# David-OConnor/molchanica

Measured on AMD Instinct MI355X. Metric: MD atom-updates/sec (and steps/sec), 1M-atom solvated box, higher is better.
Workload: dtype f32

## Files before the change

include/mdx.h:

```cpp
#ifndef MDX_H
#define MDX_H

#include <stddef.h>
#include <stdint.h>

#ifdef __cplusplus
extern "C" {
#endif

#define MDX_OK       0
#define MDX_EPARAM  (-1)
#define MDX_EDEVICE (-2)
#define MDX_ENAN    (-3)
#define MDX_EOOM    (-4)

#define MDX_OVR_BONDED_DISABLED           0x1u
#define MDX_OVR_COULOMB_DISABLED          0x2u
#define MDX_OVR_LJ_DISABLED               0x4u
#define MDX_OVR_LONG_RANGE_RECIP_DISABLED 0x8u

#define MDX_ATOM_STATIC      0x1u
#define MDX_ATOM_BONDED_ONLY 0x2u
#define MDX_ATOM_GHOST       0x4u

// ... 111 lines not shown
    uint64_t prune_passes;
    uint32_t n_owned, n_ghost;
    uint64_t repartitions;
    uint64_t local_rebuilds;
    double   repartition_ms_sum;
    double   fused_ms_sum;  uint64_t fused_launches;
    uint64_t energy_evaluations, energies_from_step_loop;
    uint64_t rebuild_fallbacks;
} mdx_stats;

typedef struct mdx_handle mdx_handle;

int mdx_device_count(void);

const char* mdx_last_error(void);

void mdx_config_default(mdx_config* cfg);

int mdx_create(const mdx_system* sys, const mdx_config* cfg, int device, mdx_handle** out);
void mdx_destroy(mdx_handle* h);

int mdx_step(mdx_handle* h, float dt, const float* ext_forces, uint32_t n_steps);

int      mdx_set_position_restraints(mdx_handle* h, uint32_t n, const uint32_t* idx, const float* ref, const float* k,
                                     const float* flat_bottom);
uint32_t mdx_position_restraints_read(mdx_handle* h, uint32_t capacity, uint32_t* idx, float* ref, float* k, float* flat_bottom);
int      mdx_restraint_energy(mdx_handle* h, double* energy, double* virial);

int mdx_energy(mdx_handle* h, mdx_energies* out);

int mdx_single_point(const mdx_system* sys, const mdx_config* cfg, int device,
                     mdx_energies* out, float* forces_or_null);
void mdx_single_point_release(void);

int mdx_download(mdx_handle* h, int which, float* dst );
int mdx_upload(mdx_handle* h, int which, const float* src );
int mdx_upload_range(mdx_handle* h, int which, uint32_t first, uint32_t count, const float* src );

int mdx_set_box(mdx_handle* h, const float lo[3], const float hi[3]);
int mdx_rebuild_spatial_caches(mdx_handle* h);

uint64_t mdx_step_count(const mdx_handle* h);

int mdx_neighbor_list(mdx_handle* h, uint32_t* offsets , uint32_t* idx );

enum { MDX_HC_FLEXIBLE = 0, MDX_HC_SHAKE = 1, MDX_HC_LINEAR = 2 };
int mdx_set_hydrogen_constraint(mdx_handle* h, int kind, uint32_t lincs_order, uint32_t lincs_iter, float shake_tolerance);
const char* mdx_constraint_description(mdx_handle* h);

int mdx_profile(mdx_handle* h, int enable);
int mdx_get_stats(mdx_handle* h, mdx_stats* out);
int mdx_pair_launch_info(const mdx_handle* h, uint32_t out[24]);
int mdx_pair_body_info(const mdx_handle* h, uint32_t out[4]);
int mdx_get_skin(const mdx_handle* h, float* skin, int* tuning);

#define MDX_THERMOSTAT_NONE      0
#define MDX_THERMOSTAT_BERENDSEN 1
#define MDX_THERMOSTAT_CSVR      2

#define MDX_INTEGRATOR_VERLET_VELOCITY 0
#define MDX_INTEGRATOR_LEAPFROG        1
#define MDX_INTEGRATOR_LANGEVIN_MIDDLE 2
int mdx_set_integrator(mdx_handle* h, int kind, float gamma_per_ps, float temperature, uint64_t seed);

int mdx_set_alchemical_softcore(mdx_handle* h, float alpha, float sigma_min);
int mdx_configure_alchemical_window(mdx_handle* h, uint32_t mol_index, double lambda);

#define MDX_MAX_FOREIGN_LAMBDAS 32
int      mdx_set_foreign_lambdas(mdx_handle* h, uint32_t n, const double* lambdas);
int      mdx_foreign_energies(mdx_handle* h, double* du , uint32_t n);
uint32_t mdx_snapshot_foreign_count(const mdx_handle* h, uint32_t k);
int      mdx_snapshot_read_foreign(mdx_handle* h, uint32_t k, double* du, uint32_t n);

#define MDX_BAROSTAT_NONE      0
#define MDX_BAROSTAT_BERENDSEN 1
#define MDX_BAR_PER_KCAL_MOL_A3 69476.95

int mdx_minimize_energy(mdx_handle* h, uint32_t max_iters, const float* ext_forces_or_null, float f_tol,
                        mdx_energies* final_or_null, uint32_t* iters_done_or_null);
int mdx_initialize_velocities(mdx_handle* h, float temperature, int zero_com_drift, uint64_t seed);
int mdx_shrink_cell_towards(mdx_handle* h, const float target_lo[3], const float target_hi[3], float shrink_per_step,
                            int* shrank_out);
int mdx_get_box(const mdx_handle* h, float lo[3], float hi[3]);
int mdx_set_barostat(mdx_handle* h, int kind, float pressure_target_bar, float tau_ps, float compressibility_per_bar,
                     uint32_t every_n_steps);
int mdx_set_thermostat(mdx_handle* h, int kind, float temp_target, float tau_ps, uint32_t every_n_steps,
                       uint64_t seed);
int mdx_set_zero_com_drift(mdx_handle* h, int enable);
int mdx_set_energy_cadence(mdx_handle* h, uint32_t every_n_steps);
int      mdx_set_snapshot_cadence(mdx_handle* h, uint32_t every_n, int with_velocities);
uint32_t mdx_snapshot_count(const mdx_handle* h);
int      mdx_snapshot_read(mdx_handle* h, uint32_t k, double* time_ps, uint64_t* step, mdx_energies* e,
                           float* pos , float* vel_or_null );
int      mdx_flush_snapshot_queues(mdx_handle* h);
#define MDX_SNAP_HANDLERS 8
enum { MDX_SNAP_MEMORY = 0, MDX_SNAP_DCD = 1, MDX_SNAP_NSTXOUT = 2, MDX_SNAP_NSTVOUT = 3, MDX_SNAP_NSTFOUT = 4, MDX_SNAP_NSTENERGY = 5,
       MDX_SNAP_NSTCALCENERGY = 6, MDX_SNAP_NSTXOUT_COMPRESSED = 7 };
int      mdx_set_snapshot_handlers(mdx_handle* h, const uint32_t every_n[MDX_SNAP_HANDLERS] );
uint32_t mdx_snapshot_handler_mask(const mdx_handle* h, uint32_t k);
int      mdx_snapshot_read_forces(mdx_handle* h, uint32_t k, float* frc );

#define MDX_HB_STANDARD 0
#define MDX_HB_WATER_O  1
#define MDX_HB_WATER_H0 2
#define MDX_HB_WATER_H1 3
typedef struct mdx_hbond {
// ... 132 lines not shown
```

molchanica_amd/csrc/mdx_api.hip:

```cpp
#include "mdx_comm.h"
#include <algorithm>
#include <atomic>
#include <chrono>
#include <cfloat>
#include <cmath>
#include <cstring>
#include <dlfcn.h>
#include <mutex>
#include <unordered_map>

static thread_local std::string g_last_error;
void mdx_set_error(const std::string& s) { g_last_error = s; }

static inline unsigned div_up(unsigned a, unsigned b) { return (a + b - 1) / b; }
static bool cut_on(float rc) { return rc > 0.f && std::isfinite(rc); }
static uint32_t f2u(float f) { uint32_t u; std::memcpy(&u, &f, 4); return u; }
static float u2f(uint32_t u) { float f; std::memcpy(&f, &u, 4); return f; }

#define FAIL(code, msg) do { mdx_set_error(msg); return (code); } while (0)

template <typename T>
static int upload_vec(T** dptr, const std::vector<T>& v, hipStream_t st) {
    if (*dptr) { (void)hipFree(*dptr); *dptr = nullptr; }
    HIP_TRY(hipMalloc((void**)dptr, std::max<size_t>(sizeof(T) * v.size(), 16)));
// ... 57 lines not shown
    MDX_TRY(chk(s->pairs14_idx, s->n_pairs14, 2, "pairs14"));
    if (s->n_bonds && (!s->bond_k || !s->bond_r0)) FAIL(MDX_EPARAM, "missing bond parameters");
    if (s->n_angles && (!s->angle_k || !s->angle_theta0)) FAIL(MDX_EPARAM, "missing angle parameters");
    if (s->n_dihedrals && (!s->dihedral_v || !s->dihedral_phase || !s->dihedral_n))
        FAIL(MDX_EPARAM, "missing dihedral parameters");
    if (s->excl_offsets) {
        if (s->excl_offsets[0] != 0) FAIL(MDX_EPARAM, "excl_offsets[0] must be 0");
        for (uint32_t i = 0; i < N; ++i)
            if (s->excl_offsets[i + 1] < s->excl_offsets[i]) FAIL(MDX_EPARAM, "excl_offsets not monotone");
        if (s->excl_offsets[N] && !s->excl_idx) FAIL(MDX_EPARAM, "missing excl_idx");
        for (uint32_t k = 0; k < s->excl_offsets[N]; ++k)
            if (s->excl_idx[k] >= N) FAIL(MDX_EPARAM, "exclusion index out of range");
    }
    if (!(c->skin >= 0.f) || !std::isfinite(c->skin)) FAIL(MDX_EPARAM, "skin must be finite and >= 0");
    if (!(c->coulomb_k >= 0.f)) FAIL(MDX_EPARAM, "coulomb_k must be >= 0");
    if (c->coulomb_mode < 0 || c->coulomb_mode > 2) FAIL(MDX_EPARAM, "unknown coulomb_mode");
    if (c->combining_rule < 0 || c->combining_rule > 1) FAIL(MDX_EPARAM, "unknown combining_rule");
    if (c->coulomb_mode == MDX_COULOMB_EWALD && !(c->ewald_alpha > 0.f))
        FAIL(MDX_EPARAM, "ewald_alpha must be > 0 for MDX_COULOMB_EWALD");
    return MDX_OK;
}

static void decode_periodic(int32_t v, int per[3]) {
    if (v & 0x10) { per[0] = v & 1; per[1] = (v >> 1) & 1; per[2] = (v >> 2) & 1; }
    else per[0] = per[1] = per[2] = (v != 0);
}

static int check_box(const int per[3], const float* lo, const float* hi, const mdx_config* c) {
    if (!(per[0] || per[1] || per[2])) return MDX_OK;
    if (!cut_on(c->lj_cutoff) || !cut_on(c->coulomb_cutoff))
        FAIL(MDX_EPARAM, "a periodic system needs finite LJ and Coulomb cut-offs");
    const float rl = std::max(c->lj_cutoff, c->coulomb_cutoff) + c->skin;
    for (int d = 0; d < 3; ++d) {
        if (!per[d]) continue;
        const float L = hi[d] - lo[d];
        if (!(L > 0.f) || !std::isfinite(L)) FAIL(MDX_EPARAM, "box extent must be positive");
        if (L < 2.0f * rl)
            FAIL(MDX_EPARAM, "box edge shorter than 2*(cutoff+skin): minimum image is not unique");
    }
    return MDX_OK;
}

int mdx_check_box(const mdx_handle* h, const float* lo, const float* hi) { return check_box(h->per, lo, hi, &h->cfg); }

static void free_device(mdx_handle* h) {
    DeviceState& d = h->d;
    void* ptrs[] = {d.o_qs, d.o_lj, d.o_invm, d.o_mass, d.o_q, d.o_lj_raw, d.excl_off, d.excl_idx, d.pos_orig,
                    d.vel_orig, d.ext_orig, d.posq, d.posq_alt, d.lj, d.vel, d.force, d.ref, d.orig_of, d.slot_of, d.gid, d.lflag,
                    d.slot_flags, d.cell_of,
                    d.cell_count, d.cell_start, d.cell_cursor, d.sorted_orig, d.sorted_tmp, d.col_tiles, d.tile_start,
                    d.tile_col, d.scan_tmp, d.cl_lo, d.cl_hi, d.cl_kind, d.list_counts, d.entry_cnt, d.entry_off,
                    d.mchunk_cnt, d.mchunk_off, d.entries, d.entries_in, d.inner_nch, d.list_cursors, d.masks, d.role_off_o, d.role_rec_o, d.role_cnt_s,
                    d.role_off_s, d.role_rec_s, d.role_prm, d.ctl, d.energy,
                    d.flags_dev, d.bonded_part, d.bbox_red, d.pair_count, d.inner_count, d.pme_force, d.wstep_s, d.path, d.dprune, d.force_b, d.force_c, d.cons_o, d.cons_s, d.cons_tmp, d.cons_mask, d.cons_cnt, d.cons_off, d.cons_vir, d.vsite_o, d.vsite_s, d.gsite_o, d.gsite_s, d.gsite_tmp, d.pme_q, d.pme_f,
                    d.pme_theta, d.pme_q2, d.pme_f2, d.scratch4, d.tile_bnd, d.tile_scan, d.tile_order, d.tile_lpt, d.rb_ctl, d.scan_chain, d.grp, d.grp_mat, d.fl_hot, d.fl_slab, d.star_o, d.star_s, d.ewald_tab,
                    d.ps_cls, d.ps_p14, d.ps_stage, d.ps_slab, d.ps_rows, d.ps_fslab, d.ps_fout, d.ps_rigid, d.ps_flex, d.ps_flex_tab, d.ps_search};
    for (void* p : ptrs) if (p) (void)hipFree(p);
    d = DeviceState{};
}

extern "C" void mdx_destroy(mdx_handle* h) {
    if (!h) return;
    (void)hipSetDevice(h->device);
    if (h->stream) (void)hipStreamSynchronize(h->stream);
    mdx_dd_destroy(h);
    for (auto& e : h->ev_pending) { (void)hipEventDestroy(e.a); (void)hipEventDestroy(e.b); }
    for (auto& e : h->ev_pool) (void)hipEventDestroy(e);
    mdx_pme_destroy(h);
    free_device(h);
    if (h->h_ctl) (void)hipHostFree(h->h_ctl);
    if (h->h_rb) (void)hipHostFree(h->h_rb);
    if (h->stream) (void)hipStreamDestroy(h->stream);
    delete h;
}

static int create_impl(const mdx_system* s, const mdx_config* c, int device, mdx_handle* h) {
    const uint32_t N = s->n_atoms;
    h->N = N; h->cfg = *c; h->device = device;
    if (h->cfg.chunk_steps == 0) h->cfg.chunk_steps = N < 131072u ? 48u : 16u;
    if (h->cfg.chunk_steps > MDX_MAX_CHUNK) h->cfg.chunk_steps = MDX_MAX_CHUNK;
    decode_periodic(s->periodic, h->per);
    h->periodic = h->per[0] || h->per[1] || h->per[2];
    for (int d = 0; d < 3; ++d) h->posre_per[d] = h->per[d];
    for (int d = 0; d < 3; ++d) { h->box_lo[d] = s->box_lo[d]; h->box_hi[d] = s->box_hi[d]; }
    MDX_TRY(check_box(h->per, h->box_lo, h->box_hi, c));
    h->n_local = N; h->cap_local = N;
    const bool all_cut = cut_on(c->lj_cutoff) && cut_on(c->coulomb_cutoff);
    if (c->skin == 0.f && all_cut && h->periodic) {
        float s0 = 2.0f;
        for (int d = 0; d < 3; ++d)
            if (h->per[d]) s0 = std::min(s0, 0.5f * (h->box_hi[d] - h->box_lo[d]) - std::max(c->lj_cutoff, c->coulomb_cutoff) - 0.01f);
        if (s0 >= 0.5f) { h->cfg.skin = s0; h->skin_tune.on = true; h->skin_tune.base_skin = s0; MDX_TRY(check_box(h->per, h->box_lo, h->box_hi, &h->cfg)); }
    }
    h->r_list = all_cut ? std::max(c->lj_cutoff, c->coulomb_cutoff) + h->cfg.skin : INFINITY;

    int ndev = 0;
    if (hipGetDeviceCount(&ndev) != hipSuccess || ndev == 0) FAIL(MDX_EDEVICE, "no HIP device available");
    if (device < 0 || device >= ndev) FAIL(MDX_EDEVICE, "device index out of range");
    HIP_TRY(hipSetDevice(device));
    h->pme_cus_per_xcd = mdx_pme_cu_split(h, c);
    if (h->pme_cus_per_xcd) MDX_TRY(mdx_stream_create_masked(&h->stream, h->pme_cus_per_xcd, true));
    else HIP_TRY(hipStreamCreateWithFlags(&h->stream, hipStreamNonBlocking));
    hipStream_t st = h->stream;
    DeviceState& d = h->d;

    const bool lj_off = (c->overrides & MDX_OVR_LJ_DISABLED) != 0;
    const bool coul_off = (c->overrides & MDX_OVR_COULOMB_DISABLED) != 0;
    const bool geom = c->combining_rule == MDX_COMBINE_GEOMETRIC;
    const float sqrt_ke = std::sqrt(c->coulomb_k);
    std::vector<float> qs(N), invm(N), mass(N), q(N);
    std::vector<float2> lj(N), ljraw(N);
    h->flags.assign(N, 0);
    h->n_mobile = 0; h->total_mass = 0.0;
    for (uint32_t i = 0; i < N; ++i) {
        const uint8_t fl = s->flags ? s->flags[i] : 0;
        h->flags[i] = fl;
        const bool nb_off = (fl & MDX_ATOM_BONDED_ONLY) != 0;
        const bool fixed = (fl & (MDX_ATOM_STATIC | MDX_ATOM_GHOST)) != 0;
        const float sg = s->lj_sigma[s->lj_type[i]], ep = s->lj_eps[s->lj_type[i]];
        q[i] = (nb_off || coul_off) ? 0.f : s->charge[i];
        qs[i] = q[i] * sqrt_ke;
        const float ep_eff = (nb_off || lj_off) ? 0.f : ep;
        lj[i] = make_float2(geom ? std::sqrt(sg) : 0.5f * sg, std::sqrt(24.0f * ep_eff));
        ljraw[i] = make_float2(sg, ep_eff);
        mass[i] = s->mass[i];
        invm[i] = fixed ? 0.f : MDX_ACC_CONV / s->mass[i];
        if (!fixed) { h->n_mobile++; }
        if (!(fl & MDX_ATOM_GHOST)) h->total_mass += s->mass[i];
    }
    h->h_mass = mass; h->h_lj = lj;
    {
        uint32_t n_lj_only = 0, n_q_only = 0;
        for (uint32_t i = 0; i < N; ++i) {
            const bool has_lj = lj[i].y != 0.f, has_q = qs[i] != 0.f;
            n_lj_only += has_lj && !has_q; n_q_only += has_q && !has_lj;
        }
        const char* const e = std::getenv("MDX_KIND_CLUSTERS");
        h->kind_split = e ? e[0] != '0' : (n_lj_only >= N / 20u && n_q_only >= N / 20u && N >= 200000u);
    }
    mdx_refresh_uni_lj(h);
    h->mol_start.assign(s->mol_start ? s->mol_start : nullptr, s->mol_start ? s->mol_start + s->n_mols : nullptr);
    h->total_charge = 0.0; h->sum_q2 = 0.0;
    h->q_abs_max = 0.0;
    for (uint32_t i = 0; i < N; ++i) { h->total_charge += q[i]; h->sum_q2 += (double)q[i] * q[i]; h->q_abs_max = std::max(h->q_abs_max, (double)std::fabs(q[i])); }
    const bool pme_on = c->coulomb_mode == MDX_COULOMB_EWALD && !(c->overrides & MDX_OVR_LONG_RANGE_RECIP_DISABLED) &&
                        !coul_off;
    MDX_TRY(upload_vec(&d.o_qs, qs, st)); MDX_TRY(upload_vec(&d.o_lj, lj, st));
    MDX_TRY(upload_vec(&d.o_invm, invm, st)); MDX_TRY(upload_vec(&d.o_mass, mass, st));
    MDX_TRY(upload_vec(&d.o_q, q, st)); MDX_TRY(upload_vec(&d.o_lj_raw, ljraw, st));

    std::vector<std::vector<uint32_t>> ex(N);
    {
        if (s->excl_offsets)
            for (uint32_t i = 0; i < N; ++i)
                for (uint32_t k = s->excl_offsets[i]; k < s->excl_offsets[i + 1]; ++k) {
                    const uint32_t j = s->excl_idx[k];
                    if (j == i) continue;
                    ex[i].push_back(j); ex[j].push_back(i);
                }
        for (uint32_t p = 0; p < s->n_pairs14; ++p) {
            const uint32_t a = s->pairs14_idx[2 * p], b = s->pairs14_idx[2 * p + 1];
            if (a == b) FAIL(MDX_EPARAM, "1-4 pair of an atom with itself");
            ex[a].push_back(b); ex[b].push_back(a);
        }
        std::vector<uint32_t> off(N + 1, 0), idx;
        for (uint32_t i = 0; i < N; ++i) {
            std::sort(ex[i].begin(), ex[i].end());
            ex[i].erase(std::unique(ex[i].begin(), ex[i].end()), ex[i].end());
            if (ex[i].size() > 255) FAIL(MDX_EPARAM, "more than 255 exclusions on one atom");
            off[i + 1] = off[i] + (uint32_t)ex[i].size();
            idx.insert(idx.end(), ex[i].begin(), ex[i].end());
        }
        MDX_TRY(upload_vec(&d.excl_off, off, st)); MDX_TRY(upload_vec(&d.excl_idx, idx, st));
    }

    h->n_bonds = s->n_bonds; h->n_angles = s->n_angles; h->n_dih = s->n_dihedrals; h->n_p14 = s->n_pairs14;
    {
        std::vector<uint32_t> cnt(N + 1, 0);
        auto count_term = [&](const uint32_t* idx, uint32_t n, int w) {
            for (size_t k = 0; k < (size_t)n * w; ++k) cnt[idx[k] + 1]++;
        };
        count_term(s->bond_idx, s->n_bonds, 2); count_term(s->angle_idx, s->n_angles, 3);
        count_term(s->dihedral_idx, s->n_dihedrals, 4); count_term(s->pairs14_idx, s->n_pairs14, 2);
        auto recip_excluded = [&](uint32_t i, uint32_t j) { return q[i] != 0.f && q[j] != 0.f; };
        if (pme_on)
            for (uint32_t i = 0; i < N; ++i)
                for (uint32_t j : ex[i]) cnt[i + 1] += recip_excluded(i, j) ? 1u : 0u;
        for (uint32_t i = 0; i < N; ++i) cnt[i + 1] += cnt[i];
        const uint32_t R = cnt[N];
        std::vector<RoleRec> recs(R);
        std::vector<uint32_t> cur(cnt.begin(), cnt.end() - 1);
        std::vector<float4> prm_tab;
// ... 1017 lines not shown

extern "C" int mdx_rebuild_spatial_caches(mdx_handle* h) {
    if (!h) FAIL(MDX_EPARAM, "null handle");
    HIP_TRY(hipSetDevice(h->device));
    h->list_valid = false;
    MDX_TRY(mdx_rebuild(h));
    return MDX_OK;
}

extern "C" int mdx_neighbor_list(mdx_handle* h, uint32_t* offsets, uint32_t* idx) {
    if (!h || !offsets) FAIL(MDX_EPARAM, "null argument");
    HIP_TRY(hipSetDevice(h->device));
    if (!h->list_valid) MDX_TRY(mdx_rebuild(h));
    return mdx_extract_neighbors(h, offsets, idx);
}

extern "C" int mdx_profile(mdx_handle* h, int enable) {
    if (!h) FAIL(MDX_EPARAM, "null handle");
    HIP_TRY(hipSetDevice(h->device));
    HIP_TRY(hipStreamSynchronize(h->stream));
    mdx_prof_collect(h);
    h->profile = enable != 0; h->profile_level = enable;
    if (enable) {
        h->stats.nb_ms_sum = h->stats.bonded_ms_sum = h->stats.integ_ms_sum = 0.0;
        h->stats.rebuild_ms_sum = h->stats.wall_ms_sum = 0.0;
        h->stats.nb_launches = h->stats.bonded_launches = h->stats.integ_launches = 0;
        if (h->dd) for (int k = 0; k < MDX_DIAG_PHASES; ++k) { h->dd->phase_ms[k] = 0.0; h->dd->phase_n[k] = 0; }
    }
    return MDX_OK;
}

extern "C" int mdx_get_skin(const mdx_handle* h, float* skin, int* tuning) {
    if (!h) FAIL(MDX_EPARAM, "null handle");
    if (skin) *skin = h->cfg.skin;
    if (tuning) *tuning = (h->skin_tune.on && h->skin_tune.phase < 4) ? 1 : 0;
    return MDX_OK;
}

extern "C" int mdx_pair_launch_info(const mdx_handle* h, uint32_t out[24]) {
    if (!h || !out) FAIL(MDX_EPARAM, "null argument");
    for (int k = 0; k < 8; ++k) { out[k] = h->pair_info_step[k]; out[8 + k] = h->pair_info_any[k]; }
    out[16] = h->inner_rebuilds; out[17] = h->inner_from_rebuild ? 1u : 0u; out[18] = h->water_step_launches; out[19] = h->water_step_mixed_launches;
    out[20] = (uint32_t)h->onepass_launches; out[21] = (uint32_t)h->onepass_violations; out[22] = h->pair_info_tail[0]; out[23] = h->pair_info_tail[1];
    return MDX_OK;
}

extern "C" int mdx_pair_body_info(const mdx_handle* h, uint32_t out[4]) {
    if (!h || !out) FAIL(MDX_EPARAM, "null argument");
    out[0] = h->uni_lj ? 1u : 0u; out[1] = h->pair_body_step; out[2] = h->pair_body_any;
    std::memcpy(&out[3], &h->uni_c, 4);
    return MDX_OK;
}

extern "C" int mdx_get_stats(mdx_handle* h, mdx_stats* out) {
    if (!h || !out) FAIL(MDX_EPARAM, "null argument");
    HIP_TRY(hipSetDevice(h->device));
    HIP_TRY(hipStreamSynchronize(h->stream));
    mdx_prof_collect(h);
    h->stats.step_count = h->step_count; h->stats.rebuild_count = h->rebuild_count;
    h->stats.n_inner_cluster_pairs = 0; h->stats.prune_passes = 0;
    if (h->d.inner_count) {
        unsigned long long c[MDX_EPART + 1];
        HIP_TRY(hipSetDevice(h->device));
        HIP_TRY(hipMemcpyAsync(c, h->d.inner_count, sizeof(c), hipMemcpyDeviceToHost, h->stream));
        HIP_TRY(hipStreamSynchronize(h->stream));
        unsigned long long tot = 0;
        for (int k = 0; k < MDX_EPART; ++k) tot += c[k];
        h->stats.prune_passes = c[MDX_EPART];
        h->stats.n_inner_cluster_pairs = c[MDX_EPART] ? tot / c[MDX_EPART] : 0;
    }
    h->stats.n_owned = h->dd ? h->dd->n_owned : h->n_local;
    h->stats.n_ghost = h->dd ? h->dd->n_local - h->dd->n_owned : 0;
    h->stats.repartitions = h->dd ? h->dd->repartitions : 0;
    h->stats.local_rebuilds = h->dd ? h->dd->local_rebuilds : 0;
    h->stats.repartition_ms_sum = h->dd ? h->dd->repartition_ms : 0.0;
    *out = h->stats;
    return MDX_OK;
}

__global__ void pack_pos_kernel(uint32_t n, const uint32_t* __restrict__ atom_idx, const uint32_t* __restrict__ slot_of,
                                const float4* __restrict__ posq, float4* __restrict__ out,
                                const uint32_t* __restrict__ flag_word) {
    uint32_t i = blockIdx.x * blockDim.x + threadIdx.x;
    if (i >= n) return;
    const uint32_t g = atom_idx[i];
    if (g == MDX_INVALID) {
        out[i] = make_float4(flag_word ? __uint_as_float(*flag_word) : 0.f, 0.f, 0.f, 0.f);
        return;
    }
    const uint32_t s = slot_of[g];
    out[i] = (s == MDX_INVALID) ? make_float4(0.f, 0.f, 0.f, 0.f) : posq[s];
}
__global__ void unpack_pos_kernel(uint32_t n, const uint32_t* __restrict__ atom_idx, const uint32_t* __restrict__ slot_of,
                                  float4* __restrict__ posq, const float4* __restrict__ in,
                                  const float4* __restrict__ shift, uint32_t* __restrict__ flag_word,
                                  float4* __restrict__ ref, uint32_t* __restrict__ prune_out, float path_thr,
                                  float gx, float gy, float gz, float* __restrict__ path_arr) {
    uint32_t i = blockIdx.x * blockDim.x + threadIdx.x;
    if (i >= n) return;
    const uint32_t g = atom_idx[i];
    if (g == MDX_INVALID) {
        if (flag_word) atomicMax(flag_word, __float_as_uint(in[i].x));
        return;
    }
    const uint32_t s = slot_of[g];
    if (s == MDX_INVALID) return;
// ... 267 lines not shown
```

molchanica_amd/csrc/mdx_extras.hip:

```cpp
#include "mdx_comm.h"
#include <algorithm>
#include <cmath>
#include <cstring>

#define FAIL(code, msg) do { mdx_set_error(msg); return (code); } while (0)
static inline unsigned div_up(unsigned a, unsigned b) { return (a + b - 1) / b; }

static double rng_u01(uint64_t* s) { return ((double)(mdx_splitmix64(s) >> 11) + 0.5) * (1.0 / 9007199254740992.0); }
static double rng_gauss(uint64_t* s) {
#pragma clang fp contract(off)
    const double u1 = rng_u01(s), u2 = rng_u01(s);
    return std::sqrt(-2.0 * std::log(u1)) * std::cos(6.283185307179586 * u2);
}
static double rng_gamma_int(uint64_t* s, long ia) {
    const double d = (double)ia - 1.0 / 3.0, c = 1.0 / std::sqrt(9.0 * d);
    for (;;) {
        const double x = rng_gauss(s), t = 1.0 + c * x;
        if (t <= 0.0) continue;
        const double v = t * t * t, u = rng_u01(s);
        if (std::log(u) < 0.5 * x * x + d - d * v + d * std::log(v)) return d * v;
    }
}
static double rng_sum_noises(uint64_t* s, long nn) {
    if (nn <= 0) return 0.0;
// ... 374 lines not shown
    h->e_cache_valid = false;
    return MDX_OK;
}

extern "C" int mdx_set_thermostat(mdx_handle* h, int kind, float temp_target, float tau_ps, uint32_t every_n_steps,
                                  uint64_t seed) {
    if (!h) FAIL(MDX_EPARAM, "null handle");
    if (kind < 0 || kind > 2) FAIL(MDX_EPARAM, "unknown thermostat kind");
    if (kind && (!(temp_target >= 0.f) || !(tau_ps > 0.f) || every_n_steps == 0))
        FAIL(MDX_EPARAM, "thermostat needs temp_target >= 0, tau > 0 and a coupling interval >= 1 step");
    h->tstat_kind = kind; h->tstat_temp = temp_target; h->tstat_tau = tau_ps;
    h->tstat_every = every_n_steps ? every_n_steps : 10; h->rng_state = seed;
    return MDX_OK;
}

extern "C" int mdx_set_integrator(mdx_handle* h, int kind, float gamma_per_ps, float temperature, uint64_t seed) {
    if (!h) FAIL(MDX_EPARAM, "null handle");
    if (kind < 0 || kind > 2) FAIL(MDX_EPARAM, "unknown integrator kind");
    if (kind == MDX_INTEGRATOR_LANGEVIN_MIDDLE && (!(gamma_per_ps >= 0.f) || !(temperature >= 0.f) || !std::isfinite(gamma_per_ps)))
        FAIL(MDX_EPARAM, "Langevin middle needs gamma >= 0 and temperature >= 0");
    if (kind && h->n_local != h->N && !h->dd) FAIL(MDX_EPARAM, "only velocity Verlet is supported on a decomposed handle");
    h->integrator = kind; h->lang_gamma = gamma_per_ps; h->lang_temp = temperature; h->lang_seed = seed;
    return MDX_OK;
}

extern "C" int mdx_set_alchemical_softcore(mdx_handle* h, float alpha, float sigma_min) {
    if (!h) FAIL(MDX_EPARAM, "null handle");
    if (!(alpha >= 0.f) || !std::isfinite(alpha)) FAIL(MDX_EPARAM, "soft-core alpha must be >= 0 (0 = linear coupling)");
    if (!(sigma_min > 0.f) || !std::isfinite(sigma_min)) FAIL(MDX_EPARAM, "soft-core sigma_min must be > 0");
    h->sc_alpha = alpha; h->sc_sigma_min = sigma_min;
    h->forces_valid = false;
    return MDX_OK;
}

extern "C" int mdx_configure_alchemical_window(mdx_handle* h, uint32_t mol_index, double lambda) {
    if (!h) FAIL(MDX_EPARAM, "null handle");
    HIP_TRY(hipSetDevice(h->device));
    const bool on = lambda >= 0.0;
    if (on) {
        if (!(lambda <= 1.0)) FAIL(MDX_EPARAM, "lambda must lie in [0, 1] (negative switches the window off)");
        if (h->mol_start.empty() || mol_index >= h->mol_start.size()) FAIL(MDX_EPARAM, "molecule index out of range (mol_start missing?)");
        if (!h->dd && h->n_local != h->N) FAIL(MDX_EPARAM, "alchemical windows need the library's own decomposition (mdx_comm_init) on a narrowed handle");
    }
    const uint32_t lo = on ? h->mol_start[mol_index] : 0;
    const uint32_t hi = on ? (mol_index + 1 < h->mol_start.size() ? h->mol_start[mol_index + 1] : h->N) : 0;
    for (uint32_t i = 0; i < h->N; ++i) {
        const float m = std::fabs(h->h_lj[i].y);
        h->h_lj[i].y = (i >= lo && i < hi) ? -m : m;
    }
    HIP_TRY(hipMemcpyAsync(h->d.o_lj, h->h_lj.data(), sizeof(float2) * h->N, hipMemcpyHostToDevice, h->stream));
    HIP_TRY(hipStreamSynchronize(h->stream));
    MDX_TRY(mdx_unsort_state(h));
    h->alch_on = on; h->alch_lambda = on ? lambda : 0.0; h->alch_lo = lo; h->alch_hi = hi;
    mdx_refresh_uni_lj(h);
    h->pme_canvas_clean = false; h->pme_canvas2_clean = false;
    h->list_valid = false; h->forces_valid = false;
    return MDX_OK;
}

extern "C" int mdx_get_box(const mdx_handle* h, float lo[3], float hi[3]) {
    if (!h || !lo || !hi) FAIL(MDX_EPARAM, "null argument");
    for (int d = 0; d < 3; ++d) { lo[d] = h->box_lo[d]; hi[d] = h->box_hi[d]; }
    return MDX_OK;
}

extern "C" int mdx_set_barostat(mdx_handle* h, int kind, float pressure_target_bar, float tau_ps,
                                float compressibility_per_bar, uint32_t every_n_steps) {
    if (!h) FAIL(MDX_EPARAM, "null handle");
    if (kind < 0 || kind > 1) FAIL(MDX_EPARAM, "unknown barostat kind");
    if (kind) {
        if (!h->dd && (!h->periodic || !(h->per[0] && h->per[1] && h->per[2]))) FAIL(MDX_EPARAM, "the barostat needs a fully periodic box");
        if (!h->dd && h->n_local != h->N) FAIL(MDX_EPARAM, "the barostat needs the library's own decomposition (mdx_comm_init) on a narrowed handle");
        if (!(tau_ps > 0.f) || every_n_steps == 0 || !std::isfinite(pressure_target_bar))
            FAIL(MDX_EPARAM, "barostat needs a finite target, tau > 0 and a coupling interval >= 1 step");
    }
    h->baro_kind = kind; h->baro_p0 = pressure_target_bar; h->baro_tau = tau_ps;
    h->baro_beta = compressibility_per_bar > 0.f ? compressibility_per_bar : 4.5e-5f;
    h->baro_every = every_n_steps ? every_n_steps : 25;
    return MDX_OK;
}

extern "C" int mdx_set_zero_com_drift(mdx_handle* h, int enable) {
    if (!h) FAIL(MDX_EPARAM, "null handle");
    h->zero_com = enable != 0;
    return MDX_OK;
}

extern "C" int mdx_set_snapshot_cadence(mdx_handle* h, uint32_t every_n, int with_velocities) {
    if (!h) FAIL(MDX_EPARAM, "null handle");
    h->snap_every = every_n; h->snap_vel = with_velocities != 0;
    return MDX_OK;
}

extern "C" uint32_t mdx_snapshot_count(const mdx_handle* h) { return h ? (uint32_t)h->snapshots.size() : 0u; }
extern "C" int mdx_snapshot_read_between_mols(mdx_handle* h, uint32_t k, float* out, uint32_t n) {
    if (!h || !out) FAIL(MDX_EPARAM, "null argument");
    if (k >= h->snapshots.size()) FAIL(MDX_EPARAM, "snapshot index out of range");
    const auto& sn = h->snapshots[k];
    if (sn.between.empty()) FAIL(MDX_EPARAM, "the snapshot was taken without energy groups (mdx_set_energy_groups)");
    if ((size_t)n * n != sn.between.size()) FAIL(MDX_EPARAM, "n must be the number of groups the snapshot was taken with");
    std::memcpy(out, sn.between.data(), sizeof(float) * sn.between.size());
    return MDX_OK;
}
extern "C" double mdx_time_ps(const mdx_handle* h) { return h ? h->time_ps : 0.0; }

extern "C" int mdx_set_snapshot_handlers(mdx_handle* h, const uint32_t every_n[MDX_SNAP_HANDLERS]) {
// ... 248 lines not shown
```

molchanica_amd/csrc/mdx_grid.hip:

```cpp
#include "mdx_internal.h"
#include <atomic>
#include <chrono>
#include <algorithm>
#include <cfloat>
#include <cmath>

#define WAVE_LDS_SYNC()                                      \
    do {                                                     \
        __builtin_amdgcn_fence(__ATOMIC_SEQ_CST, "workgroup"); \
        __builtin_amdgcn_wave_barrier();                     \
    } while (0)

static inline unsigned div_up(unsigned a, unsigned b) { return (a + b - 1) / b; }

constexpr int SCAN_THREADS = 256;
constexpr int SCAN_ITEMS = 8;
constexpr int SCAN_TILE = SCAN_THREADS * SCAN_ITEMS;

__device__ __forceinline__ uint32_t block_exclusive_scan_256(uint32_t v, uint32_t* s_wave, uint32_t* total) {
    const int lane = threadIdx.x & 63, wave = threadIdx.x >> 6;
    uint32_t inc = v;
#pragma unroll
    for (int d = 1; d < 64; d <<= 1) {
        uint32_t t = __shfl_up(inc, d);
// ... 836 lines not shown
        unsigned long long m = 0ull;
        uint32_t jcs[8], codes13 = 0;
#pragma unroll
        for (int e = 0; e < 8; ++e) {
            uint32_t idx = c * 8 + e;
            jcs[e] = (idx < nmc) ? (fl[idx] & 0x7FFFFFFu) : MDX_INVALID;
            if (a.half && idx < nmc && (fl[idx] >> 27) == 13u) codes13 |= 1u << e;
            if (idx < nmc) m |= 0xFFull << (8 * e);
        }
        if (myo == MDX_INVALID) {
            m = 0ull;
        } else {
#pragma unroll
            for (int e = 0; e < 8; ++e)
                if (jcs[e] == (myslot >> 3)) {
                    const unsigned long long gone = ((codes13 >> e) & 1u) ? ((2ull << (myslot & 7)) - 1ull)
                                                                          : (1ull << (myslot & 7));
                    m &= ~(gone << (8 * e));
                }
#pragma unroll
            for (int q = 0; q < LB_SPC; ++q) {
                const uint32_t sp = spc[q];
                if (sp == MDX_INVALID) continue;
#pragma unroll
                for (int e = 0; e < 8; ++e)
                    if (jcs[e] == (sp >> 3)) m &= ~(1ull << (8 * e + (sp & 7)));
            }
            for (uint32_t k = eb + LB_SPC; k < ee; ++k) {
                uint32_t sp = a.slot_of[a.excl_idx[k]];
                if (sp == MDX_INVALID) continue;
#pragma unroll
                for (int e = 0; e < 8; ++e)
                    if (jcs[e] == (sp >> 3)) m &= ~(1ull << (8 * e + (sp & 7)));
            }
        }
        if (a.mask_layout == 2) {
            const int ii = lane & 7, jj = lane >> 3;
            unsigned long long mq = 0ull;
#pragma unroll
            for (int ci = 0; ci < 8; ++ci) {
                const unsigned long long mp = __shfl(m, ci * 8 + ii);
#pragma unroll
                for (int e = 0; e < 8; ++e) mq |= ((mp >> (8 * e + jj)) & 1ull) << (8 * e + ci);
            }
            m = mq;
        }
        a.masks[(size_t)(mbase + c) * 64 + lane] = m;
    }
}

#ifndef PRUNE_TRIES
#define PRUNE_TRIES 1
#endif
struct PruneInner { uint2* entries_in; uint32_t* inner_nch; float rin2; WptRule rule; };
template <bool INNER>
__global__ __launch_bounds__(256) void prune_list_kernel(uint32_t T, float r2, float shx, float shy, float shz,
                                                         const float4* __restrict__ posq, ListCounts* __restrict__ counts,
                                                         const uint32_t* __restrict__ entry_off, uint2* __restrict__ entries,
                                                         uint32_t null_cluster, unsigned long long* __restrict__ pair_count,
                                                         const uint32_t* __restrict__ rb_ctl, uint32_t* __restrict__ tile_int,
                                                         const uint8_t* __restrict__ cl_kind, PruneInner pin) {
    __shared__ float4 s_j[4][64];
    const int lane = threadIdx.x & 63, wave = __builtin_amdgcn_readfirstlane(threadIdx.x >> 6);
    uint32_t first_ghost_cluster = 0xFFFFFFFFu;
    if (rb_ctl) {
        T = __builtin_amdgcn_readfirstlane(rb_ctl[0]); null_cluster = T * MDX_CL_PER_TILE;
        first_ghost_cluster = __builtin_amdgcn_readfirstlane(rb_ctl[1]) * MDX_CL_PER_TILE;
    }
    const bool inner_on = INNER && mdx_wpt_rule(pin.rule, T) == 1;
    bool ghost_hit = false;
    const uint32_t per_xcd = gridDim.x >> 3;
    const uint32_t t = MDX_XCD_SWIZZLE ? ((blockIdx.x & 7u) * per_xcd + (blockIdx.x >> 3)) * 4 + wave : blockIdx.x * 4 + wave;
    if (t >= T) return;
    const int ii = lane & 7, jj = lane >> 3;
    float xi[8], yi[8], zi[8];
#pragma unroll
    for (int ci = 0; ci < 8; ++ci) {
        const float4 p = posq[(size_t)t * MDX_TILE + ci * MDX_CLUSTER + ii];
        xi[ci] = p.x; yi[ci] = p.y; zi[ci] = p.z;
    }
    constexpr int NTRY = INNER ? 0 : PRUNE_TRIES;
    constexpr int TI[6] = {0, 7, 3, 0, 7, 4}, TJ[6] = {0, 7, 4, 7, 0, 3};
    float4 rep[NTRY ? NTRY : 1];
#pragma unroll
    for (int k = 0; k < NTRY; ++k) rep[k] = posq[(size_t)t * MDX_TILE + (lane & 7) * MDX_CLUSTER + TI[k]];
    uint32_t ilj = 0xFFu, iq = 0xFFu;
    if (cl_kind) {
        const uint32_t k = lane < MDX_CL_PER_TILE ? cl_kind[(size_t)t * MDX_CL_PER_TILE + lane] : 0u;
        ilj = (uint32_t)__ballot((k & 1u) != 0u) & 0xFFu; iq = (uint32_t)__ballot((k & 2u) != 0u) & 0xFFu;
    }
    const ListCounts cnt = counts[t];
    const uint32_t e0 = entry_off[t], nmc = cnt.n_masked >> 3, nchunks = (cnt.n_masked + cnt.n_plain) >> 3;
    uint32_t kept = 0, wcur = 0;
    uint32_t wcur_in = 0;
    uint2 ent_n = make_uint2(null_cluster, 13u), ent_nn = make_uint2(null_cluster, 13u);
    float4 pj_n = make_float4(0.f, 0.f, 0.f, 0.f);
    if (nchunks) { ent_n = entries[e0 + (lane >> 3)]; pj_n = posq[(size_t)ent_n.x * MDX_CLUSTER + (lane & 7)]; }
    if (nchunks > 1) ent_nn = entries[e0 + 8 + (lane >> 3)];
    for (uint32_t c = 0; c < nchunks; ++c) {
        const uint2 ent = ent_n;
        float4 pj = pj_n;
        if (c + 1 < nchunks) {
            ent_n = ent_nn;
            pj_n = posq[(size_t)ent_n.x * MDX_CLUSTER + (lane & 7)];
            if (c + 2 < nchunks) ent_nn = entries[e0 + (c + 2) * 8 + (lane >> 3)];
        }
        const uint32_t code = ent.y & 31u;
        pj.x += (float)((int)(code % 3u) - 1) * shx;
        pj.y += (float)((int)((code / 3u) % 3u) - 1) * shy;
        pj.z += (float)((int)(code / 9u) - 1) * shz;
        s_j[wave][lane] = pj;
        __builtin_amdgcn_fence(__ATOMIC_SEQ_CST, "workgroup"); __builtin_amdgcn_wave_barrier();
        uint32_t newy = ent.y;
        if (cl_kind) {
            const uint32_t kj = ent.x < null_cluster ? cl_kind[ent.x] : 0u;
            newy = (ent.y & 0xFFu) | (ent.y & ((((kj & 1u) ? ilj : 0u) | ((kj & 2u) ? iq : 0u)) << 8));
        }
        const uint32_t y_in = newy;
        uint32_t newy_in = newy & 0xFFu;
        unsigned long long acc = 0ull;
#pragma unroll
        for (int k = 0; k < NTRY; ++k) {
            const float4 q = s_j[wave][(lane & ~7) + TJ[k]];
            const float dx = rep[k].x - q.x, dy = rep[k].y - q.y, dz = rep[k].z - q.z;
            acc |= __ballot(dx * dx + dy * dy + dz * dz < r2);
        }
#pragma unroll 2
        for (int e = 0; e < 8; ++e) {
            const float4 q = s_j[wave][e * 8 + jj];
            const uint32_t y = __builtin_amdgcn_readlane(y_in, e * 8);
            const uint32_t sure = (uint32_t)(acc >> (e * 8)) & 0xFFu;
            uint32_t any = sure, anyin = 0u;
#pragma unroll
            for (int ci = 0; ci < 8; ++ci) {
                if (!(((y >> 8) & ~sure) & (1u << ci))) continue;
                const float dx = xi[ci] - q.x, dy = yi[ci] - q.y, dz = zi[ci] - q.z;
                const float d2 = dx * dx + dy * dy + dz * dz;
                const bool hit = __ballot(d2 < r2) != 0ull;
                any |= (hit ? 1u : 0u) << ci;
                if (INNER && hit) anyin |= (__ballot(d2 < pin.rin2) != 0ull ? 1u : 0u) << ci;
            }
            const uint32_t im = (y >> 8) & any;
            kept += __popc(im & 0xFFu);
            if ((lane >> 3) == e) newy = (y & 0xFFu) | ((im & 0xFFu) << 8);
            if (INNER && (lane >> 3) == e) newy_in = (y & 0xFFu) | ((((y >> 8) & anyin) & 0xFFu) << 8);
        }
        __builtin_amdgcn_fence(__ATOMIC_SEQ_CST, "workgroup"); __builtin_amdgcn_wave_barrier();
        ghost_hit |= ((newy >> 8) & 0xFFu) != 0u && ent.x >= first_ghost_cluster && ent.x < null_cluster;
        if (c < nmc) {
            if ((lane & 7) == 0 && newy != ent.y) entries[e0 + c * 8 + (lane >> 3)].y = newy;
            if (inner_on && (lane & 7) == 0) pin.entries_in[e0 + c * 8 + (lane >> 3)] = make_uint2(ent.x, newy_in);
        } else {
            const bool alive = (lane & 7) == 0 && ((newy >> 8) & 0xFFu) != 0u;
            const unsigned long long bal = __ballot(alive);
            if (alive) {
                const uint32_t rank = __popcll(bal & ((1ull << lane) - 1ull));
                entries[e0 + cnt.n_masked + wcur + rank] = make_uint2(ent.x, newy);
            }
            wcur += __popcll(bal);
            if (inner_on) {
                const bool alive_in = (lane & 7) == 0 && ((newy_in >> 8) & 0xFFu) != 0u;
                const unsigned long long bin = __ballot(alive_in);
                if (alive_in) pin.entries_in[e0 + cnt.n_masked + wcur_in + __popcll(bin & ((1ull << lane) - 1ull))] = make_uint2(ent.x, newy_in);
                wcur_in += __popcll(bin);
            }
        }
    }
    const uint32_t np_pad = (wcur + 7u) & ~7u;
    if (lane < (int)(np_pad - wcur)) entries[e0 + cnt.n_masked + wcur + lane] = make_uint2(null_cluster, 13u);
    if (inner_on) {
        const uint32_t nin_pad = (wcur_in + 7u) & ~7u;
        if (lane < (int)(nin_pad - wcur_in)) pin.entries_in[e0 + cnt.n_masked + wcur_in + lane] = make_uint2(null_cluster, 13u);
        if (lane < 8) pin.inner_nch[(size_t)t * 8 + lane] = nmc + (nin_pad >> 3);
    }
    const bool any_ghost = __any(ghost_hit);
    if (lane == 0) {
        counts[t].n_plain = np_pad;
        if (kept) atomicAdd(pc_slot(pair_count, t, 1), (unsigned long long)kept);
        if (tile_int) tile_int[t] = (!any_ghost && t * MDX_CL_PER_TILE < first_ghost_cluster) ? 1u : 0u;
    }
}

template <int W>
__global__ __launch_bounds__(W * 64) void prune_list_mw_kernel(uint32_t T, float r2, float shx, float shy, float shz,
                                                               const float4* __restrict__ posq, ListCounts* __restrict__ counts,
                                                               const uint32_t* __restrict__ entry_off, uint2* __restrict__ entries,
                                                               uint32_t null_cluster, unsigned long long* __restrict__ pair_count,
                                                               const uint32_t* __restrict__ rb_ctl, uint32_t* __restrict__ tile_int,
                                                               const uint8_t* __restrict__ cl_kind) {
    __shared__ float4 s_j[W][64];
    __shared__ uint32_t s_ghost;
    const int lane = threadIdx.x & 63, wave = __builtin_amdgcn_readfirstlane(threadIdx.x >> 6);
    uint32_t first_ghost_cluster = 0xFFFFFFFFu;
    if (rb_ctl) {
        T = __builtin_amdgcn_readfirstlane(rb_ctl[0]); null_cluster = T * MDX_CL_PER_TILE;
        first_ghost_cluster = __builtin_amdgcn_readfirstlane(rb_ctl[1]) * MDX_CL_PER_TILE;
    }
    const uint32_t t = blockIdx.x;
    if (t >= T) return;
    if (threadIdx.x == 0) s_ghost = 0u;
    if (tile_int) __syncthreads();
    bool ghost_hit = false;
    const int ii = lane & 7, jj = lane >> 3;
    float xi[8], yi[8], zi[8];
#pragma unroll
    for (int ci = 0; ci < 8; ++ci) {
        const float4 p = posq[(size_t)t * MDX_TILE + ci * MDX_CLUSTER + ii];
        xi[ci] = p.x; yi[ci] = p.y; zi[ci] = p.z;
    }
    const float4 rep = posq[(size_t)t * MDX_TILE + (lane & 7) * MDX_CLUSTER];
    uint32_t ilj = 0xFFu, iq = 0xFFu;
    if (cl_kind) {
        const uint32_t k = lane < MDX_CL_PER_TILE ? cl_kind[(size_t)t * MDX_CL_PER_TILE + lane] : 0u;
        ilj = (uint32_t)__ballot((k & 1u) != 0u) & 0xFFu; iq = (uint32_t)__ballot((k & 2u) != 0u) & 0xFFu;
    }
    const ListCounts cnt = counts[t];
    const uint32_t e0 = entry_off[t], nchunks = (cnt.n_masked + cnt.n_plain) >> 3;
    uint32_t kept = 0;
    uint2 ent_n = make_uint2(null_cluster, 13u);
    float4 pj_n = make_float4(0.f, 0.f, 0.f, 0.f);
    if ((uint32_t)wave < nchunks) { ent_n = entries[e0 + wave * 8 + (lane >> 3)]; pj_n = posq[(size_t)ent_n.x * MDX_CLUSTER + (lane & 7)]; }
    for (uint32_t c = wave; c < nchunks; c += W) {
        const uint2 ent = ent_n;
        float4 pj = pj_n;
        if (c + W < nchunks) {
            ent_n = entries[e0 + (c + W) * 8 + (lane >> 3)];
// ... 483 lines not shown
            return major * LPT_BUCKETS + LPT_BUCKETS - 1u - min(nch, LPT_BUCKETS - 1u);
        };
        for (uint32_t t = threadIdx.x; t < T; t += blockDim.x) atomicAdd(&s_hist[bucket(t)], 1u);
        __syncthreads();
        {
            const uint32_t b0 = 2u * threadIdx.x, h0 = b0 < NB ? s_hist[b0] : 0u, h1 = b0 + 1u < NB ? s_hist[b0 + 1u] : 0u;
            uint32_t tot;
            const uint32_t ex = block_exclusive_scan_1024(h0 + h1, s_scan, &tot);
            if (b0 < NB) s_cur[b0] = ex;
            if (b0 + 1u < NB) s_cur[b0 + 1u] = ex + h0;
            __syncthreads();
            if (pass == 1 && threadIdx.x == 0) s_nint = s_cur[LPT_BUCKETS];
        }
        __syncthreads();
        for (uint32_t t = threadIdx.x; t < T; t += blockDim.x) order[atomicAdd(&s_cur[bucket(t)], 1u)] = t;
        __syncthreads();
    }
    if (threadIdx.x < 64) {
        const unsigned long long c = a.cursors[(size_t)threadIdx.x * 16];
        uint32_t e = (uint32_t)c, m = (uint32_t)(c >> 32);
        unsigned long long pa = a.pair_count[(size_t)threadIdx.x * PC_STRIDE], pb = a.pair_count[(size_t)threadIdx.x * PC_STRIDE + 1];
#pragma unroll
        for (int k = 32; k > 0; k >>= 1) { e += __shfl_xor(e, k); m += __shfl_xor(m, k); pa += __shfl_xor(pa, k); pb += __shfl_xor(pb, k); }
        if (threadIdx.x == 0) {
            a.pair_count[PC_TOTAL] = pa; a.pair_count[PC_TOTAL + 1] = pb;
            a.rb_ctl[RB_N_INT] = s_nint;
            a.host[0] = T; a.host[1] = a.rb_ctl[RB_T_OWN]; a.host[2] = a.rb_ctl[RB_NONFINITE]; a.host[3] = s_nint;
            for (int k = 0; k < 4; ++k) a.host[4 + k] = a.flags[k];
            a.host[8] = e; a.host[9] = m;
            a.host[10] = (uint32_t)pa; a.host[11] = (uint32_t)(pa >> 32); a.host[12] = (uint32_t)pb; a.host[13] = (uint32_t)(pb >> 32);
            a.rb_ctl[RB_NONFINITE] = 0u;
            __threadfence_system();
            a.host[31] = a.seq;
        }
    }
}


static int spin_on_readback(mdx_handle* h, uint32_t seq) {
    static const bool spin_ok = [] { const char* e = std::getenv("MDX_CHUNK_SPIN"); return !(e && e[0] == '0'); }();
    if (!spin_ok) { HIP_TRY(hipStreamSynchronize(h->stream)); return MDX_OK; }
    volatile uint32_t* seq_word = (volatile uint32_t*)h->h_rb + 31;
    const auto t0 = std::chrono::steady_clock::now();
    for (uint32_t spins = 0; *seq_word != seq; ++spins) {
        if ((spins & 0xFFFu) == 0xFFFu && std::chrono::steady_clock::now() - t0 > std::chrono::milliseconds(50)) {
            HIP_TRY(hipStreamSynchronize(h->stream));
            break;
        }
    }
    std::atomic_thread_fence(std::memory_order_acquire);
    return MDX_OK;
}

struct RebuildResult { uint32_t T = 0, E = 0, MC = 0, n_interior = 0; unsigned long long npairs = 0; bool ordered = false, classified = false, inner_built = false; };

struct TileOrderPlan { bool lpt, grouped, split; };
static TileOrderPlan tile_order_plan(const mdx_handle* h, uint32_t T) {
    static const int lpt_env = [] { const char* e = std::getenv("MDX_TILE_LPT"); return e ? (e[0] == '0' ? 0 : (e[0] == '2' ? 2 : 1)) : -1; }();
    const bool decomposed = h->dd || h->n_local != h->N;
    TileOrderPlan p;
    p.lpt = (lpt_env >= 0 ? lpt_env >= 1 : (decomposed || T >= 512u)) && mdx_nb_variant(h) >= 2;
    p.grouped = lpt_env >= 0 ? lpt_env == 2 : !decomposed;
    p.split = h->want_tile_split && mdx_nb_variant(h) >= 2;
    return p;
}

static int rebuild_fast(mdx_handle* h, RebuildResult* res, bool* fell_back) {
    DeviceState& d = h->d;
    hipStream_t st = h->stream;
    const uint32_t N = h->n_local;
    const GridParams g = h->grid;
    *fell_back = false;
    if (!d.rb_ctl) { ALLOC(d.rb_ctl, RB_WORDS); HIP_TRY(hipMemsetAsync(d.rb_ctl, 0, sizeof(uint32_t) * RB_WORDS, st)); }
    if (!d.pair_count) ALLOC(d.pair_count, PC_TOTAL + 2);
    if (!d.list_cursors) ALLOC(d.list_cursors, LB_REGIONS * 32 + 2);
    if (!h->h_rb) { HIP_TRY(hipHostMalloc((void**)&h->h_rb, sizeof(uint32_t) * 32, hipHostMallocDefault)); h->h_rb[31] = 0u; }
    if (!h->cell_count_clean) { HIP_TRY(hipMemsetAsync(d.cell_count, 0, sizeof(uint32_t) * ((size_t)h->ncells + 1), st)); h->cell_count_clean = true; }
    if (!h->slot_of_clean) { HIP_TRY(hipMemsetAsync(d.slot_of, 0xFF, sizeof(uint32_t) * (size_t)h->N, st)); h->slot_of_clean = true; }
    const uint32_t T_bound = N / MDX_TILE + h->ncol + 1;
    if (T_bound + 1 > h->cap_tiles) { *fell_back = true; return MDX_OK; }
    const TileOrderPlan plan = tile_order_plan(h, T_bound);
    const bool prune = !std::isinf(h->r_list) && mdx_nb_variant(h) >= 2;
    static const bool exact_prune = [] { const char* e = std::getenv("MDX_EXACT_PRUNE"); return !(e && e[0] == '0'); }();
    const bool classify_here = plan.split && plan.lpt && g.npop > 1 && prune && exact_prune;
    if (plan.lpt && (!d.tile_lpt || d.cap_tile_lpt < T_bound)) { d.cap_tile_lpt = h->cap_tiles + 1; ALLOC(d.tile_lpt, d.cap_tile_lpt); }
    if (classify_here && (!d.tile_bnd || h->cap_tile_split < T_bound + 1)) {
        h->cap_tile_split = h->cap_tiles + 1;
        ALLOC(d.tile_bnd, h->cap_tile_split); ALLOC(d.tile_scan, h->cap_tile_split); ALLOC(d.tile_order, h->cap_tile_split);
    }

    if (h->in_slot_space)
        hipLaunchKernelGGL(rb_prep_kernel<true>, dim3(div_up(N, 256)), dim3(256), 0, st, N, g, d.gid, d.slot_of, d.posq, d.vel, d.pos_orig,
                           d.vel_orig, d.lflag, d.cell_of, d.sorted_orig, d.cell_count, d.rb_ctl);
    else
        hipLaunchKernelGGL(rb_prep_kernel<false>, dim3(div_up(N, 256)), dim3(256), 0, st, N, g, d.gid, d.slot_of, d.posq, d.vel, d.pos_orig,
                           d.vel_orig, d.lflag, d.cell_of, d.sorted_orig, d.cell_count, d.rb_ctl);
    h->in_slot_space = false;
    {
        GridScanArgs ga{};
        ga.ncells = h->ncells; ga.ncol = h->ncol; ga.nzb = g.nzb;
        ga.first_ghost_col = g.npop > 1 ? (uint32_t)(g.ncx * g.ncy) : 0xFFFFFFFFu;
        ga.cell_count = d.cell_count; ga.cell_start = d.cell_start; ga.tile_start = d.tile_start; ga.tile_col = d.tile_col;
        ga.rb_ctl = d.rb_ctl; ga.flags = d.flags_dev; ga.pair_count = d.pair_count; ga.list_cursors = d.list_cursors;
        MDX_TRY(scan_chain_of(h, &ga.chain));
        hipLaunchKernelGGL(rb_gridscan_kernel, dim3(div_up(h->ncells + 1, SCAN1_WINDOW)), dim3(SCAN1_THREADS), 0, st, ga);
    }
    hipLaunchKernelGGL(rb_scatter_kernel, dim3(div_up(N, 256)), dim3(256), 0, st, N, d.cell_of, d.sorted_orig, d.cell_start, d.sorted_tmp);
    hipLaunchKernelGGL(cell_rank_kernel, dim3(div_up(N, 256)), dim3(256), 0, st, N, d.cell_of, d.cell_start, d.pos_orig, d.sorted_tmp, d.sorted_orig);
    {
        AssignArgs aa{};
        aa.rb_ctl = d.rb_ctl; aa.nzb = g.nzb; aa.tile_col = d.tile_col; aa.tile_start = d.tile_start; aa.cell_start = d.cell_start;
        aa.sorted_orig = d.sorted_orig; aa.pos_orig = d.pos_orig; aa.vel_orig = d.vel_orig; aa.gid = d.gid; aa.lflag = d.lflag;
        aa.o_qs = d.o_qs; aa.o_lj = d.o_lj; aa.o_invm = d.o_invm; aa.orig_of = d.orig_of; aa.slot_of = d.slot_of;
        aa.cl_kind = d.cl_kind; aa.kind_split = h->kind_split ? 1 : 0;
        aa.posq = d.posq; aa.lj = d.lj; aa.vel = d.vel; aa.ref = d.ref; aa.force = d.force; aa.slot_flags = d.slot_flags; aa.path = d.path; aa.dprune = d.dprune;
        aa.cl_lo = d.cl_lo; aa.cl_hi = d.cl_hi;
        aa.role_off_o = h->n_roles ? d.role_off_o : nullptr; aa.role_cnt_s = h->n_roles ? d.role_cnt_s : nullptr;
        hipLaunchKernelGGL(rb_assign_kernel, dim3(div_up(T_bound + 1, 4)), dim3(256), 0, st, aa);
    }
    h->in_slot_space = true;
    const uint32_t S_bound = (T_bound + 1) * MDX_TILE;
    if (h->n_roles) MDX_TRY(scan_u32_dev_n(h, d.role_cnt_s, d.role_off_s, S_bound + 1, d.scan_tmp, d.rb_ctl + RB_SCAN_N));

    ListArgs a{};
    a.T = T_bound; a.T_dev = d.rb_ctl + RB_T; a.g = g;
    a.r_build = std::isinf(h->r_list) ? h->r_list : h->r_list * (1.0f + 1e-5f) + 1e-4f;
    a.tile_col = d.tile_col; a.tile_start = d.tile_start; a.cl_lo = d.cl_lo; a.cl_hi = d.cl_hi;
    a.orig_of = d.orig_of; a.slot_of = d.slot_of; a.gid = d.gid; a.slot_flags = d.slot_flags;
    a.excl_off = d.excl_off; a.excl_idx = d.excl_idx;
    a.counts = d.list_counts; a.entry_cnt = d.entry_cnt; a.mchunk_cnt = d.mchunk_cnt;
    a.entry_off = d.entry_off; a.mchunk_off = d.mchunk_off; a.entries = d.entries; a.masks = d.masks;
    a.err = d.flags_dev; a.null_cluster = T_bound * MDX_CL_PER_TILE;
    a.mask_layout = mdx_nb_variant(h) >= 2 ? 2 : 1;
    a.half = mdx_nb_half(h) ? 1 : 0;
    a.cell_start = d.cell_start; a.posq = d.posq; a.pair_count = d.pair_count;
    a.cursors = reinterpret_cast<unsigned long long*>(d.list_cursors);
    a.n_regions = 1;
    while (a.n_regions < (uint32_t)LB_REGIONS && a.n_regions * 128u <= T_bound) a.n_regions <<= 1;
    a.region_cap_e = (uint32_t)(std::min<uint64_t>(h->cap_entries, 0xFFFFFFFFull) / a.n_regions) & ~7u;
    a.region_cap_m = h->cap_mchunks / a.n_regions;
    a.list_grid = (div_up(T_bound, LB_WAVES) + 7u) & ~7u;
    uint32_t rf_blocks = 0;
    if (h->n_roles) {
        a.rf_S = S_bound; a.rf_role_off_o = d.role_off_o; a.rf_rec_o = d.role_rec_o; a.rf_role_off_s = d.role_off_s;
        a.rf_rec_s = d.role_rec_s; a.rf_lflag = d.lflag;
        rf_blocks = div_up(S_bound, LB_WAVES * 64);
    }
    if (g.npop > 1) hipLaunchKernelGGL((build_list_kernel<LB_SINGLE, LB_PLAIN_DD>), dim3(a.list_grid + rf_blocks), dim3(LB_WAVES * 64), 0, st, a);
    else hipLaunchKernelGGL(build_list_kernel<LB_SINGLE>, dim3(a.list_grid + rf_blocks), dim3(LB_WAVES * 64), 0, st, a);
    static const int inner_mode = [] { const char* e = std::getenv("MDX_REBUILD_INNER"); return e ? (e[0] == '0' ? 0 : (e[0] == '2' ? 2 : 1)) : 1; }();
    const bool inner_env = inner_mode == 2 || (inner_mode == 1 && !mdx_has_constraints(h) && h->n_vsites == 0);
    const float inner_skin_next = h->inner_skin_auto > 0.f ? h->inner_skin_auto : c_inner_skin(h->cfg);
    const bool dual_next = !h->dual_auto_off && mdx_nb_half(h) && prune && inner_skin_next > 0.f && inner_skin_next < h->cfg.skin &&
                           (h->n_vsites == 0 || h->vsites_convex);
    const bool inner_here = inner_env && dual_next && exact_prune && !h->dd && h->n_local == h->N && g.npop == 1 && !h->alch_on &&
                            d.entries_in && d.inner_nch;
    bool inner_launched = false;
    if (prune && exact_prune) {
        const float rb = a.r_build;
        const float shx = h->per[0] ? h->box_hi[0] - h->box_lo[0] : 0.f, shy = h->per[1] ? h->box_hi[1] - h->box_lo[1] : 0.f,
                    shz = h->per[2] ? h->box_hi[2] - h->box_lo[2] : 0.f;
        uint32_t* const tint = classify_here ? d.tile_bnd : nullptr;
        const uint8_t* const kinds = h->kind_split ? d.cl_kind : nullptr;
        static const uint32_t mw_below = [] { const char* e = std::getenv("MDX_PRUNE_MW_BELOW"); return e ? (uint32_t)std::atoi(e) : 12000u; }();
        if (T_bound < mw_below)
            hipLaunchKernelGGL(prune_list_mw_kernel<8>, dim3(T_bound), dim3(512), 0, st, T_bound, rb * rb, shx, shy, shz, d.posq, d.list_counts,
                               d.entry_off, d.entries, a.null_cluster, d.pair_count, (const uint32_t*)d.rb_ctl, tint, kinds);
        else if (inner_here) {
            PruneInner pin{};
            pin.entries_in = d.entries_in; pin.inner_nch = d.inner_nch; pin.rule = mdx_wpt_rule_of(h);
            const float rin = std::max(std::isfinite(h->cfg.lj_cutoff) && h->cfg.lj_cutoff > 0.f ? h->cfg.lj_cutoff : 0.f,
                                       std::isfinite(h->cfg.coulomb_cutoff) && h->cfg.coulomb_cutoff > 0.f ? h->cfg.coulomb_cutoff : 0.f) + inner_skin_next;
            pin.rin2 = rin * rin;
            hipLaunchKernelGGL(prune_list_kernel<true>, dim3((div_up(T_bound, 4) + 7u) & ~7u), dim3(256), 0, st, T_bound, rb * rb, shx, shy, shz,
                               d.posq, d.list_counts, d.entry_off, d.entries, a.null_cluster, d.pair_count, (const uint32_t*)d.rb_ctl, tint, kinds, pin);
            inner_launched = true;
        } else
            hipLaunchKernelGGL(prune_list_kernel<false>, dim3((div_up(T_bound, 4) + 7u) & ~7u), dim3(256), 0, st, T_bound, rb * rb, shx, shy, shz,
                               d.posq, d.list_counts, d.entry_off, d.entries, a.null_cluster, d.pair_count, (const uint32_t*)d.rb_ctl, tint, kinds,
                               PruneInner{});
    }
    MDX_TRY(mdx_remap_constraints(h));
    const uint32_t seq = ++h->rb_seq;
    {
        FinishArgs fa{};
        fa.rb_ctl = d.rb_ctl; fa.counts = d.list_counts;
        fa.tile_lpt = plan.lpt ? d.tile_lpt : nullptr; fa.lpt_grouped = plan.grouped ? 1u : 0u; fa.rule = mdx_wpt_rule_of(h);
        fa.tile_int = classify_here ? d.tile_bnd : nullptr; fa.tile_order = classify_here ? d.tile_order : nullptr;
        fa.cursors = reinterpret_cast<const unsigned long long*>(d.list_cursors); fa.pair_count = d.pair_count; fa.flags = d.flags_dev;
        fa.host = (volatile uint32_t*)h->h_rb; fa.seq = seq;
        hipLaunchKernelGGL(rb_finish_kernel, dim3(1), dim3(1024), 0, st, fa);
    }
    HIP_TRY(hipGetLastError());
    MDX_TRY(spin_on_readback(h, seq));
    const uint32_t T = h->h_rb[0];
    uint32_t flags[4];
    for (int k = 0; k < 4; ++k) flags[k] = h->h_rb[4 + k];
    if (h->h_rb[2]) { h->cell_count_clean = false; mdx_set_error("non-finite position at neighbour rebuild"); return MDX_ENAN; }
    if (T > T_bound) { mdx_set_error("internal: tile count beyond its bound"); return MDX_EDEVICE; }
    h->T = T; h->S = (T + 1) * MDX_TILE;
    if (flags[0] & 1u) { mdx_set_error("exclusion table overflow while building the pair list"); return MDX_EPARAM; }
    if (flags[0] & (16u | 32u)) {
        if (std::getenv("MDX_LIST_DEBUG")) fprintf(stderr, "[mdx] fused list rebuild fell back: flags %u, T %u, cap_e %llu cap_m %u regions %u\n",
                                                   flags[0], T, (unsigned long long)h->cap_entries, h->cap_mchunks, a.n_regions);
        *fell_back = true;
        return MDX_OK;
    }
    if (flags[0] & 8u) { mdx_set_error("a constrained / virtual-site atom is missing from the local atom set"); return MDX_EPARAM; }
    if (flags[0] & 2u) { mdx_set_error("exclusion table overflow while building the pair list"); return MDX_EPARAM; }
    if (flags[0] & 4u) { mdx_set_error("a bonded partner of an owned atom is missing from the local atom set (halo too thin)"); return MDX_EPARAM; }
    res->T = T; res->E = h->h_rb[8]; res->MC = h->h_rb[9];
    const unsigned long long built = (unsigned long long)h->h_rb[10] | ((unsigned long long)h->h_rb[11] << 32);
    const unsigned long long kept = (unsigned long long)h->h_rb[12] | ((unsigned long long)h->h_rb[13] << 32);
    res->npairs = (prune && exact_prune) ? kept : built;
    h->E = res->E; h->MC = res->MC;
    res->ordered = true;
    res->inner_built = inner_launched && mdx_wpt_rule(mdx_wpt_rule_of(h), T) == 1;
    h->force_zeroed = true;
    h->tile_lpt_on = plan.lpt; h->tile_lpt_grouped = plan.grouped;
    h->tile_split = false; h->n_interior = 0;
    if (classify_here) { h->tile_split = true; h->n_interior = h->h_rb[3]; res->classified = true; }
    return MDX_OK;
}


int mdx_rebuild(mdx_handle* h) {
    MdxRange range_rebuild("mdx list rebuild");
    h->vsites_fresh = false;
    hipEvent_t e0 = nullptr, e1 = nullptr;
    if (h->profile) {
        for (hipEvent_t* e : {&e0, &e1}) {
            if (!h->ev_pool.empty()) { *e = h->ev_pool.back(); h->ev_pool.pop_back(); }
            else HIP_TRY(hipEventCreate(e));
        }
        HIP_TRY(hipEventRecord(e0, h->stream));
    }
    DeviceState& d = h->d;
    static const bool fused_env = [] { const char* e = std::getenv("MDX_REBUILD_FUSED"); return !(e && e[0] == '0'); }();
    static const bool two_pass_env0 = [] { const char* e = std::getenv("MDX_LIST_TWO_PASS"); return e && e[0] == '1'; }();
    bool fast = fused_env && !two_pass_env0 && d.entries && d.masks && h->cap_entries && h->cap_mchunks && h->T > 0 && h->n_local > 0;
    for (int k = 0; k < 3; ++k) if (!h->per[k] && !h->have_local_bounds) fast = false;
    if (!fast) MDX_TRY(mdx_unsort_state(h));
    const bool was_in_slot_space = h->in_slot_space;
    MDX_TRY(setup_grid(h));
    if (fast && (size_t)h->ncells + 1 > ((size_t)1 << 21)) { fast = false; MDX_TRY(mdx_unsort_state(h)); }
    if (fast && was_in_slot_space && !h->in_slot_space) fast = false;
    const uint32_t N = h->n_local;
    const GridParams g = h->grid;
    hipStream_t st = h->stream;
    RebuildResult res;
    bool fast_done = false;
    if (fast) {
        bool fell_back = false;
        MDX_TRY(rebuild_fast(h, &res, &fell_back));
        fast_done = !fell_back;
        if (fell_back) { MDX_TRY(mdx_unsort_state(h)); h->stats.rebuild_fallbacks++; }
    }
    uint32_t E = res.E, MC = res.MC;
    unsigned long long npairs = res.npairs;
    const bool prune = !std::isinf(h->r_list) && mdx_nb_variant(h) >= 2;
    if (!fast_done) {
    h->cell_count_clean = false;
    {
        const uint32_t n_max = std::max<uint32_t>(h->N, h->ncells + 1);
        hipLaunchKernelGGL(rebuild_clear_kernel, dim3(div_up(n_max, 256)), dim3(256), 0, st, d.slot_of, h->N, d.cell_count,
                           d.cell_cursor, h->ncells + 1, d.flags_dev);
    }
    hipLaunchKernelGGL(bin_atoms_kernel, dim3(div_up(N, 256)), dim3(256), 0, st, d.pos_orig, N, g, d.lflag, d.cell_of,
                       d.cell_count, d.flags_dev + 1);
// ... 143 lines not shown
    };
    MDX_TRY(read_counts());
    if (speculative) {
        if (flags[0] & 1u) { mdx_set_error("exclusion table overflow while building the pair list"); return MDX_EPARAM; }
        if (flags[0] & (16u | 32u)) {
            const uint32_t keep = flags[0] & ~(16u | 32u);
            HIP_TRY(hipMemcpyAsync(d.flags_dev, &keep, sizeof(uint32_t), hipMemcpyHostToDevice, st));
            HIP_TRY(hipStreamSynchronize(st));
            speculative = false;
            grow_for_regions = (flags[0] & 32u) != 0;
            if (std::getenv("MDX_LIST_DEBUG")) fprintf(stderr, "[mdx] single-pass list build fell back: flags %u, T %u, E %u MC %u, cap_e %llu cap_m %u regions %u\n",
                                                       flags[0], T, E, MC, (unsigned long long)h->cap_entries, h->cap_mchunks, a.n_regions);
            MDX_TRY(two_pass());
            launch_prune();
            MDX_TRY(read_counts());
        } else {
            h->E = E; h->MC = MC;
        }
    }
    if (prune && exact_prune) npairs = npairs_pruned;
    if (flags[0] & 8u) { mdx_set_error("a constrained / virtual-site atom is missing from the local atom set"); return MDX_EPARAM; }
    if (flags[0] & 3u) { mdx_set_error("exclusion table overflow while building the pair list"); return MDX_EPARAM; }
    if (flags[0] & 4u) {
        mdx_set_error("a bonded partner of an owned atom is missing from the local atom set (halo too thin)");
        return MDX_EPARAM;
    }

    res.T = T;
    }
    const uint32_t T = h->T, S = h->S, NC = (T + 1) * MDX_CL_PER_TILE;
    {
        const TileOrderPlan plan = tile_order_plan(h, T);
        if (!res.classified) {
            h->tile_split = false; h->n_interior = 0;
            if (plan.split) MDX_TRY(mdx_classify_tiles(h, plan.lpt));
        }
        if (!res.ordered) {
            h->tile_lpt_on = false;
            if (plan.lpt) MDX_TRY(mdx_order_tiles_by_length(h, plan.grouped));
        }
    }
    h->list_valid = true;
    h->forces_valid = false;
    h->rebuild_count++; h->steps_since_rebuild = 0;
    mdx_dd_note_rebuild(h);
    h->inner_skin = h->inner_skin_auto > 0.f ? h->inner_skin_auto : c_inner_skin(h->cfg);
    h->dual_on = !h->dual_auto_off && mdx_nb_half(h) && prune && h->inner_skin > 0.f && h->inner_skin < h->cfg.skin &&
                 (h->n_vsites == 0 || h->vsites_convex);
    h->prune_pending = !(res.inner_built && h->dual_on);
    h->inner_from_rebuild = !h->prune_pending;
    if (h->inner_from_rebuild) ++h->inner_rebuilds;
    h->tail_w = 0; h->tail_tiles = 0;
    if (h->dual_on && h->tile_lpt_on && h->tile_lpt_grouped && !h->alch_on) mdx_tail_plan(h, T, &h->tail_w, &h->tail_tiles);
    if (!d.inner_count) { ALLOC(d.inner_count, MDX_EPART + 8); HIP_TRY(hipMemsetAsync(d.inner_count, 0, sizeof(unsigned long long) * (MDX_EPART + 8), st)); }
    uint64_t nmask = (uint64_t)MC * 8;
    h->stats.n_atoms = N; h->stats.n_slots = S; h->stats.n_tiles = T; h->stats.n_clusters = NC;
    h->stats.n_list_entries = E; h->stats.n_masked_entries = nmask;
    h->stats.n_cluster_pairs = (mdx_nb_variant(h) >= 2) ? npairs : (uint64_t)E * 8;
    if (h->profile) {
        float ms = 0.f;
        HIP_TRY(hipEventRecord(e1, st)); HIP_TRY(hipEventSynchronize(e1));
        HIP_TRY(hipEventElapsedTime(&ms, e0, e1));
        h->stats.rebuild_ms_sum += ms;
        h->ev_pool.push_back(e0); h->ev_pool.push_back(e1);
    }
    return MDX_OK;
}

__global__ __launch_bounds__(1024) void lpt_order_kernel(uint32_t T, const ListCounts* __restrict__ counts, const uint32_t* __restrict__ is_int,
                                                         uint32_t* __restrict__ order, uint32_t group_tiles) {
    constexpr uint32_t NB = 8 * LPT_BUCKETS;
    __shared__ uint32_t s_hist[NB], s_cur[NB];
    for (uint32_t b = threadIdx.x; b < NB; b += blockDim.x) s_hist[b] = 0;
    __syncthreads();
    auto bucket = [&](uint32_t t) {
        const uint32_t nch = (counts[t].n_masked + counts[t].n_plain) >> 3;
        const uint32_t major = group_tiles ? min(t / group_tiles, 7u) : ((is_int && !is_int[t]) ? 1u : 0u);
        return major * LPT_BUCKETS + LPT_BUCKETS - 1u - min(nch, LPT_BUCKETS - 1u);
    };
    for (uint32_t t = threadIdx.x; t < T; t += blockDim.x) atomicAdd(&s_hist[bucket(t)], 1u);
    __syncthreads();
    if (threadIdx.x == 0) {
        uint32_t run = 0;
        for (uint32_t b = 0; b < NB; ++b) { s_cur[b] = run; run += s_hist[b]; }
    }
    __syncthreads();
    for (uint32_t t = threadIdx.x; t < T; t += blockDim.x) order[atomicAdd(&s_cur[bucket(t)], 1u)] = t;
}

__global__ __launch_bounds__(256) void tile_class_kernel(uint32_t T, const uint8_t* __restrict__ slot_flags,
                                                         const ListCounts* __restrict__ counts, const uint32_t* __restrict__ entry_off,
                                                         const uint2* __restrict__ entries, uint32_t* __restrict__ tile_bnd) {
    const uint32_t t = blockIdx.x * 4 + (threadIdx.x >> 6);
    const int lane = threadIdx.x & 63;
    if (t >= T) return;
    const uint8_t f = slot_flags[t * MDX_TILE + lane];
    bool ghost = (f & 1u) && !(f & 2u);
    const ListCounts c = counts[t];
    const uint32_t e0 = entry_off[t], n = c.n_masked + c.n_plain;
    for (uint32_t k = lane; k < n; k += 64) {
        const uint2 e = entries[e0 + k];
        if (((e.y >> 8) & 0xFFu) == 0u) continue;
        const unsigned long long fl = *reinterpret_cast<const unsigned long long*>(slot_flags + (size_t)e.x * MDX_CLUSTER);
        ghost |= ((fl & 0x0101010101010101ull) & ~((fl >> 1) & 0x0101010101010101ull)) != 0ull;
    }
    const bool any = __any(ghost);
// ... 113 lines not shown
```

molchanica_amd/csrc/mdx_hostutil.cpp:

```cpp
#include <cstdint>
#include <cstddef>
#include <cstring>
#if defined(__x86_64__) || defined(__i386__)
#define MDX_HOST_X86 1
#include <immintrin.h>
#endif

static uint64_t fp_mix_scalar(uint64_t h, const void* p, size_t bytes) {
    const unsigned char* b = (const unsigned char*)p;
    const uint64_t K = 0x9E3779B97F4A7C15ull;
    uint64_t x0 = h ^ 0x243F6A8885A308D3ull, x1 = h ^ 0x13198A2E03707344ull, x2 = h ^ 0xA4093822299F31D0ull, x3 = h ^ 0x082EFA98EC4E6C89ull;
    auto rotl = [](uint64_t v, int r) { return (v << r) | (v >> (64 - r)); };
    size_t k = 0;
    for (; k + 32 <= bytes; k += 32) {
        uint64_t w[4]; std::memcpy(w, b + k, 32);
        x0 = rotl(x0 ^ w[0], 29) * K; x1 = rotl(x1 ^ w[1], 31) * K; x2 = rotl(x2 ^ w[2], 33) * K; x3 = rotl(x3 ^ w[3], 37) * K;
    }
    for (; k + 8 <= bytes; k += 8) { uint64_t w; std::memcpy(&w, b + k, 8); x0 = rotl(x0 ^ w, 29) * K; }
    uint64_t w = 0; std::memcpy(&w, b + k, bytes - k);
    x1 = rotl(x1 ^ w ^ (uint64_t)bytes, 31) * K;
    h = (x0 ^ rotl(x1, 17) ^ rotl(x2, 31) ^ rotl(x3, 47)) * 0xBF58476D1CE4E5B9ull;
    return h ^ (h >> 31);
}
#ifdef MDX_HOST_X86
__attribute__((target("avx2"))) static uint64_t fp_mix_avx2(uint64_t h, const void* p, size_t bytes) {
    const unsigned char* b = (const unsigned char*)p;
    const __m256i key[4] = {_mm256_set_epi64x(0x243F6A8885A308D3ll, 0x13198A2E03707344ll, (long long)0xA4093822299F31D0ull, 0x082EFA98EC4E6C89ll),
                            _mm256_set_epi64x(0x452821E638D01377ll, (long long)0xBE5466CF34E90C6Cull, (long long)0xC0AC29B7C97C50DDull, 0x3F84D5B5B5470917ll),
                            _mm256_set_epi64x((long long)0x9216D5D98979FB1Bull, (long long)0xD1310BA698DFB5ACull, 0x2FFD72DBD01ADFB7ll, (long long)0xB8E1AFED6A267E96ull),
                            _mm256_set_epi64x((long long)0xBA7C9045F12C7F99ull, 0x24A19947B3916CF7ll, 0x0801F2E2858EFC16ll, 0x636920D871574E69ll)};
    __m256i acc[4];
    for (int i = 0; i < 4; ++i) acc[i] = _mm256_xor_si256(key[i], _mm256_set1_epi64x((long long)h));
    size_t k = 0;
    __m256i walk = _mm256_setzero_si256();
    const __m256i stride = _mm256_set_epi64x((long long)0x9E3779B97F4A7C15ull, (long long)0xC2B2AE3D27D4EB4Full, 0x165667B19E3779F9ll, (long long)0x85EBCA77C2B2AE63ull);
    for (; k + 128 <= bytes; k += 128) {
        walk = _mm256_add_epi64(walk, stride);
        for (int i = 0; i < 4; ++i) {
            const __m256i d = _mm256_loadu_si256((const __m256i*)(b + k + 32 * i));
            const __m256i dk = _mm256_xor_si256(d, _mm256_add_epi64(key[i], walk));
            acc[i] = _mm256_add_epi64(acc[i], _mm256_mul_epu32(dk, _mm256_shuffle_epi32(dk, 0x31)));
            acc[i] = _mm256_add_epi64(acc[i], _mm256_shuffle_epi32(d, 0x4E));
        }
    }
    uint64_t lanes[16];
    for (int i = 0; i < 4; ++i) _mm256_storeu_si256((__m256i*)(lanes + 4 * i), acc[i]);
    uint64_t x = h ^ (uint64_t)bytes;
    for (int i = 0; i < 16; ++i) { x = (x ^ lanes[i]) * 0x9E3779B97F4A7C15ull; x ^= x >> 29; }
    return fp_mix_scalar(x, b + k, bytes - k);
}
#endif
bool mdx_uniform_lj(const float* lj, size_t n, bool geometric, bool alch_on, float* c_out) {
    if (c_out) *c_out = 0.f;
    if (!lj || geometric || alch_on) return false;
    bool have = false;
    uint32_t hbits = 0;
    for (size_t i = 0; i < n; ++i) {
        if (lj[2 * i + 1] == 0.f) continue;
        uint32_t b; std::memcpy(&b, &lj[2 * i], 4);
        if (!have) { have = true; hbits = b; }
        else if (b != hbits) return false;
    }
    if (!have) return false;
    float h; std::memcpy(&h, &hbits, 4);
    volatile float sig = h + h;
    const float s = sig;
    volatile float c = s * s;
    if (c_out) *c_out = c;
    return true;
}

uint64_t mdx_fp_mix(uint64_t h, const void* p, size_t bytes) {
    if (!p) return (h ^ 0x9E3779B97F4A7C15ull) * 0xBF58476D1CE4E5B9ull;
#ifdef MDX_HOST_X86
    static const bool avx2 = __builtin_cpu_supports("avx2");
    if (avx2 && bytes >= 512) return fp_mix_avx2(h, p, bytes);
#endif
    return fp_mix_scalar(h, p, bytes);
}
```

molchanica_amd/csrc/mdx_internal.h:

```cpp
#pragma once
#include <hip/hip_runtime.h>
#include <stdint.h>
#include <chrono>
#include <cstdlib>
#include <cstring>
#include <string>
#include <vector>
#include "../../include/mdx.h"

#define MDX_TILE 64
#define MDX_CLUSTER 8
#define MDX_CL_PER_TILE 8
#define MDX_ACC_CONV 418.4f
#define MDX_KB 0.0019872041
#define MDX_INVALID 0xFFFFFFFFu
#define MDX_DUMMY_BASE 1.0e6f
#define MDX_DUMMY_STEP 64.0f
#define MDX_MAX_CHUNK 64
#define MDX_MAX_GROUPS 255

#define MDX_ESTRIDE 5
#define MDX_EPART 256
enum { EN_BOND = 0, EN_ANGLE, EN_DIHEDRAL, EN_LJ, EN_COUL, EN_LJ14, EN_COUL14, EN_KIN, EN_RECIP, EN_VIRIAL, EN_POSRE, EN_POSRE_VIR, EN_COUNT };

// ... 113 lines not shown
    float4* ref = nullptr;
    float* path = nullptr; float* dprune = nullptr;
    float4* force_b = nullptr;
    float4* force_c = nullptr;
    float4* posq_alt = nullptr;
    uint32_t* orig_of = nullptr;
    uint32_t* slot_of = nullptr;
    uint32_t* gid = nullptr;
    uint8_t*  lflag = nullptr;
    uint8_t*  slot_flags = nullptr;
    uint32_t* cell_of = nullptr;
    uint32_t* cell_count = nullptr;
    uint32_t* cell_start = nullptr;
    uint32_t* cell_cursor = nullptr;
    uint32_t* sorted_orig = nullptr;
    uint32_t* sorted_tmp = nullptr;
    uint32_t* col_tiles = nullptr;
    uint32_t* tile_start = nullptr;
    uint32_t* tile_col = nullptr;
    uint32_t* scan_tmp = nullptr;
    float4* cl_lo = nullptr; float4* cl_hi = nullptr;
    uint8_t* cl_kind = nullptr;
    ListCounts* list_counts = nullptr;
    uint32_t* entry_cnt = nullptr;
    uint32_t* entry_off = nullptr;
    uint32_t* mchunk_cnt = nullptr;
    uint32_t* mchunk_off = nullptr;
    uint2*    entries = nullptr;
    uint2*    entries_in = nullptr;
    uint32_t* list_cursors = nullptr;
    uint32_t* inner_nch = nullptr;
    unsigned long long* masks = nullptr;
    uint32_t* role_off_o = nullptr; RoleRec* role_rec_o = nullptr;
    uint32_t* role_cnt_s = nullptr; uint32_t* role_off_s = nullptr;
    RoleRec*  role_rec_s = nullptr;
    float4*   role_prm = nullptr;
    float* pme_q = nullptr; float2* pme_f = nullptr; float* pme_theta = nullptr;
    float* pme_q2 = nullptr; float2* pme_f2 = nullptr;
    float4* pme_force = nullptr;
    ConsGroup* cons_o = nullptr; ConsGroup* cons_s = nullptr;
    ConsGroup* cons_tmp = nullptr; unsigned long long* cons_mask = nullptr; uint32_t* cons_cnt = nullptr; uint32_t* cons_off = nullptr;
    uint32_t cons_cap_tiles = 0; const uint32_t* cons_n_dev = nullptr;
    float* cons_vir = nullptr;
    ConsStar5* star_o = nullptr; ConsStar5* star_s = nullptr;
    VSite* vsite_o = nullptr; VSite* vsite_s = nullptr;
    uint8_t* wstep_s = nullptr; uint32_t cap_wstep = 0;
    GroupSite* gsite_o = nullptr; GroupSite* gsite_s = nullptr; GroupSite* gsite_tmp = nullptr;
    StepCtl* ctl = nullptr;
    double*  energy = nullptr;
    uint32_t* flags_dev = nullptr;
    double*  bonded_part = nullptr; size_t cap_bonded_part = 0;
    unsigned long long* pair_count = nullptr;
    unsigned long long* inner_count = nullptr;
    float*   bbox_red = nullptr;
    uint32_t* tile_bnd = nullptr;
    uint32_t* tile_scan = nullptr;
    uint32_t* tile_order = nullptr;
    uint32_t* tile_lpt = nullptr;
    uint32_t cap_tile_lpt = 0;
    float4*  scratch4 = nullptr;
    uint32_t* rb_ctl = nullptr;
    unsigned long long* scan_chain = nullptr;
    uint8_t* grp = nullptr; double* grp_mat = nullptr;
    uint8_t* fl_hot = nullptr; uint32_t fl_hot_cap = 0; double* fl_slab = nullptr;
    float4* ewald_tab = nullptr;
    uint8_t* ps_cls = nullptr; void* ps_p14 = nullptr; float* ps_stage = nullptr; double* ps_slab = nullptr; double* ps_rows = nullptr;
    double* ps_fslab = nullptr; float* ps_fout = nullptr; float* ps_rigid = nullptr;
    void* ps_flex = nullptr; void* ps_flex_tab = nullptr;
    void* ps_search = nullptr;
};

struct MdxDecomp;
struct mdx_handle;
bool mdx_dd_brick_bounds(const mdx_handle* h, int d, float* lo, float* hi);
bool mdx_dd_half_shell(const mdx_handle* h);

struct mdx_handle {
    int device = 0;
    MdxDecomp* dd = nullptr;
    hipStream_t stream = nullptr;
    uint32_t N = 0;
    mdx_config cfg{};
    bool periodic = false;
    int per[3] = {0, 0, 0};
    uint32_t n_local = 0, cap_local = 0;
    uint32_t cap_scratch4 = 0;
    float local_lo[3]{}, local_hi[3]{};
    bool have_local_bounds = false;
    float box_lo[3]{}, box_hi[3]{};
    uint32_t n_bonds = 0, n_angles = 0, n_dih = 0, n_p14 = 0;
    uint32_t n_roles = 0;
    uint32_t n_roles_excl = 0;
    uint32_t n_roles_dih = 0;
    uint32_t n_posre = 0, n_prm_base = 0;
    int posre_per[3] = {0, 0, 0};
    std::vector<uint32_t> posre_idx; std::vector<float> posre_ref, posre_k, posre_b;
    double posre_e = 0.0, posre_w = 0.0;
    bool excl_inside_rigid = false;
    uint32_t n_groups = 0, n_cons = 0, n_vsites = 0;
    uint32_t n_star5 = 0; std::vector<ConsStar5> h_star5;
    bool cons_all_rigid3 = false;
    bool vsites_in_groups = false;
    uint32_t water_step_launches = 0, water_step_mixed_launches = 0;
    uint32_t n_wstep_groups = 0;
    bool wstep_all = false;
    bool wstep_sites_all = false;
// ... 41 lines not shown
    float inner_skin_auto = 0.f; bool dual_auto_off = false; uint32_t dual_win_steps = 0, dual_win_prunes = 0;
    bool prune_pending = true;
    uint32_t inner_rebuilds = 0;
    bool inner_from_rebuild = false;
    bool path_split = false;
    OnePassNow onepass;
    bool onepass_refused = false;
    uint64_t onepass_launches = 0, onepass_violations = 0;
    bool prune_latch = false;
    bool moved_outside = true;
    void (*wait_hook)(void*) = nullptr; void* wait_hook_arg = nullptr;
    bool kind_split = false;
    uint32_t n_interior = 0;
    bool tile_split = false;
    bool tile_lpt_on = false;
    bool tile_lpt_grouped = false;
    bool want_tile_split = false; uint32_t cap_tile_split = 0;
    int nb_step = -1;
    uint32_t energy_every = 0; bool e_pending = false, e_cache_valid = false; uint64_t e_cache_step = 0; mdx_energies e_cache{};
    bool nb_post_rebuild = false;
    uint32_t steps_since_rebuild = 0, stretch_samples = 0; float stretch_mean = 0.f, stretch_dev = 0.f;
    struct SkinTune {
        bool on = false; int phase = 0;
        float base_skin = 2.f, best_skin = 2.f, trial = 2.f; double base_rate = 0.0, best_rate = 0.0;
        uint32_t win_steps = 0, win_rebuilds = 0, skip_rebuilds = 0, warm_steps = 0;
        float dt_tuned = 0.f;
        std::chrono::steady_clock::time_point t0;
    } skin_tune;
    int chunk_s = -1;
    bool list_valid = false;
    bool forces_valid = false;
    bool in_slot_space = false;
    bool have_ext = false;
    uint64_t step_count = 0, rebuild_count = 0;
    bool profile = false; int profile_level = 0; bool prof_open = false;
    struct EvPair { hipEvent_t a, b; int kind; int tag; hipStream_t st; };
    int prof_tag = -1;
    uint32_t prof_seq = 0; bool prof_sampled = false;
    std::vector<EvPair> ev_pending;
    std::vector<hipEvent_t> ev_pool;
    mdx_stats stats{};
    int tstat_kind = 0; float tstat_temp = 300.f, tstat_tau = 1.f; uint32_t tstat_every = 10;
    int integrator = 0; float lang_gamma = 1.f, lang_temp = 300.f; uint64_t lang_seed = 0, lang_step = 0;
    int baro_kind = 0; float baro_p0 = 1.f, baro_tau = 5.f, baro_beta = 4.5e-5f; uint32_t baro_every = 25;
    double last_pressure = 0.0, last_mu = 1.0;
    bool force_zeroed = false;
    bool cons_full_kick = false;
    bool bonded_fused = false;
    uint32_t tail_w = 0, tail_tiles = 0;
    uint32_t pair_info_tail[2] = {};
    uint32_t pair_info_step[8] = {}, pair_info_any[8] = {};
    bool uni_lj = false; float uni_c = 0.f;
    uint32_t pair_body_step = 0, pair_body_any = 0;
    bool bonded_deferred = false;
    uint64_t rng_state = 0;
    bool zero_com = false;
    uint32_t snap_every = 0; bool snap_vel = false;
    uint32_t snap_handlers[MDX_SNAP_HANDLERS] = {};
    double time_ps = 0.0;
    struct Snapshot { double time; uint64_t step; mdx_energies e; std::vector<float> pos, vel, frc; std::vector<mdx_hbond> hbonds; std::vector<float> between; uint32_t handler_mask = 0;
                      std::vector<double> foreign; };
    uint32_t water_first = 0, n_waters = 0, water_sites = 0;
    std::vector<uint8_t> hb_heavy; float hb_dmax = 2.5f, hb_angle_min = 120.f;
    std::vector<uint32_t> hb_donor_of;
    std::vector<uint32_t> h_bond_pairs;
    std::vector<uint32_t> h_dih_idx; std::vector<float> h_dih_v, h_dih_phase; std::vector<int32_t> h_dih_n;
    std::vector<Snapshot> snapshots;
    DeviceState d;
    StepCtl* h_ctl = nullptr;
    uint32_t ctl_seq = 0;
    uint32_t* h_rb = nullptr;
    uint32_t rb_seq = 0;
    uint32_t scan_gen = 0;
    bool cell_count_clean = false;
    bool slot_of_clean = false;
};

struct FusedArgs {
    uint32_t S; float dt;
    const float4* posq_in; float4* posq_out; float4* vel; float4* force; float4* ref;
    float* path; const float* dprune;
    const uint32_t* role_off; const RoleRec* roles; const float4* prm; BondedParams p; uint32_t R;
    const uint32_t* gate_in; uint32_t* disp_out; uint32_t thr_bits; uint32_t* prune_out; float path_thr;
    uint32_t pipe_flags;
    const uint32_t* send_cnt; const uint32_t* send_rows;
    const float4* frc_in; float4* send_buf;
    uint32_t n_flag; uint32_t flag_rows[32];
    PipeCtl* pc;
    uint32_t* gate_word;
};
bool mdx_dd_pipe_fill(mdx_handle* h, FusedArgs& a, uint32_t* gate_word);
void mdx_dd_note_rebuild(mdx_handle* h);

void mdx_set_error(const std::string& s);
#define HIP_TRY(expr)                                                                      \
    do {                                                                                   \
        hipError_t _e = (expr);                                                            \
        if (_e != hipSuccess) {                                                            \
            mdx_set_error(std::string(#expr) + ": " + hipGetErrorString(_e));              \
            return (_e == hipErrorOutOfMemory) ? MDX_EOOM : MDX_EDEVICE;                   \
        }                                                                                  \
    } while (0)
#define MDX_TRY(expr) do { int _r = (expr); if (_r != MDX_OK) return _r; } while (0)

int mdx_rebuild(mdx_handle* h);
int mdx_unsort_state(mdx_handle* h);
// ... 37 lines not shown
#ifndef MDX_NB_WAVES
#define MDX_NB_WAVES 1
#endif
struct WptRule { int env; uint32_t wpt8_below; int decomposed; };
__host__ __device__ static inline int mdx_wpt_rule(const WptRule& r, uint32_t T) {
    if (r.env) return r.env;
    if (T >= 12000u) return r.decomposed ? 2 : 1;
    if (T >= (r.decomposed ? 8000u : 3000u)) return 2;
    return T < r.wpt8_below ? 8 : 4;
}
static inline WptRule mdx_wpt_rule_of(const mdx_handle* h) {
    static const int env = [] { const char* e = std::getenv("MDX_WPT"); return (e && (e[0] == '1' || e[0] == '2' || e[0] == '4' || e[0] == '8')) ? e[0] - '0' : 0; }();
    WptRule r; r.env = env; r.wpt8_below = mdx_wpt8_below(h); r.decomposed = (h->dd || h->n_local != h->N) ? 1 : 0;
    return r;
}
static inline int mdx_nb_wpt_half(const mdx_handle* h, uint32_t T) { return mdx_wpt_rule(mdx_wpt_rule_of(h), T); }
#define MDX_WPT_TAIL_DEFAULT_W 4u
#define MDX_WPT_TAIL_DEFAULT_DEN 8u
static inline void mdx_tail_plan(const mdx_handle* h, uint32_t T, uint32_t* w_out, uint32_t* tiles_out) {
    struct TailEnv { int set; uint32_t w, den; };
    static const TailEnv env = [] {
        TailEnv r{0, 0u, 0u};
        const char* e = std::getenv("MDX_WPT_TAIL");
        if (!e || !e[0]) return r;
        r.set = 1;
        const uint32_t w = (uint32_t)std::atoi(e);
        const char* s = std::strchr(e, '/');
        const uint32_t den = s ? (uint32_t)std::atoi(s + 1) : 8u;
        if ((w == 2u || w == 4u) && den >= 1u) { r.w = w; r.den = den; }
        return r;
    }();
    *w_out = 0; *tiles_out = 0;
    if (h->dd || h->n_local != h->N || mdx_nb_wpt_half(h, T) != 1) return;
    if (const char* e = std::getenv("MDX_ONEPASS")) { if (e[0] == '2') return; }
    uint32_t w = 0, den = 0;
    if (env.set) { w = env.w; den = env.den; }
    else if (T >= 12000u && !h->pme_on) { w = MDX_WPT_TAIL_DEFAULT_W; den = MDX_WPT_TAIL_DEFAULT_DEN; }
    if (w < 2u) return;
    const uint32_t group = (T + 7u) >> 3;
    const uint32_t tiles = den == 1u ? group : group / den;
    if (!tiles) return;
    *w_out = w; *tiles_out = tiles;
}

bool mdx_uniform_lj(const float* lj, size_t n, bool geometric, bool alch_on, float* c_out);
static inline void mdx_refresh_uni_lj(mdx_handle* h) {
    static const bool off = [] { const char* e = std::getenv("MDX_UNI_LJ"); return e && e[0] == '0'; }();
    float c = 0.f;
    const bool ok = !off && mdx_uniform_lj(reinterpret_cast<const float*>(h->h_lj.data()), h->h_lj.size(),
                                           h->cfg.combining_rule == MDX_COMBINE_GEOMETRIC, h->alch_on, &c);
    h->uni_lj = ok; h->uni_c = ok ? c : 0.f;
}

int mdx_build_constraints(mdx_handle* h, const mdx_system* s);
int mdx_remap_constraints(mdx_handle* h);
int mdx_launch_constrain_positions(mdx_handle* h, float dt, const uint32_t* d_gate, uint32_t* d_disp_out, uint32_t thr,
                                   uint32_t* d_prune_out = nullptr, bool skip_wstep = false);
int mdx_launch_constrain_velocities(mdx_handle* h, const uint32_t* d_gate, uint32_t thr);
bool mdx_water_step_ok(const mdx_handle* h);
bool mdx_water_step_mixed(const mdx_handle* h);
int mdx_launch_water_step(mdx_handle* h, int mode, float dt, const uint32_t* d_gate, uint32_t* d_disp_out, uint32_t thr, uint32_t* d_prune_out);
int mdx_launch_vsite_construct(mdx_handle* h, const uint32_t* d_gate, uint32_t thr);
int mdx_launch_constraint_virial(mdx_handle* h);
int mdx_check_box(const mdx_handle* h, const float* lo, const float* hi);
int mdx_launch_vsite_spread(mdx_handle* h, const uint32_t* d_gate, uint32_t thr);

int mdx_pme_setup(mdx_handle* h);
int mdx_pme_cu_split(const mdx_handle* h, const mdx_config* c);
int mdx_stream_create_masked(hipStream_t* s, int cus_per_xcd, bool complement);
int mdx_stream_unmask(mdx_handle* h);
void mdx_pme_destroy(mdx_handle* h);
int mdx_launch_pme(mdx_handle* h, bool energy, const uint32_t* d_gate, uint32_t thr);
int mdx_pme_fork(mdx_handle* h);
int mdx_pme_join(mdx_handle* h, const uint32_t* d_gate, uint32_t thr);

int mdx_compute_forces(mdx_handle* h, bool energy, const uint32_t* gate, uint32_t thr);
int mdx_ensure_ready(mdx_handle* h);
int mdx_energy_impl(mdx_handle* h, mdx_energies* out);
int mdx_after_steps(mdx_handle* h, float dt, uint32_t done);
uint32_t mdx_steps_to_next_event(const mdx_handle* h);
bool mdx_energy_wanted_at(const mdx_handle* h, uint64_t step);
int mdx_finalize_energy_cache(mdx_handle* h);
int mdx_groups_evaluate(mdx_handle* h, float* out );
int mdx_foreign_evaluate(mdx_handle* h, double* du );
int mdx_launch_scale_velocities(mdx_handle* h, float lambda, const double* com_v_or_null);
int mdx_launch_momentum(mdx_handle* h);

static inline bool mdx_has_constraints(const mdx_handle* h) { return h->n_groups != 0 || h->n_star5 != 0; }
static inline double mdx_dof(const mdx_handle* h) {
    const double d = 3.0 * (double)h->n_mobile - (double)h->n_cons - 3.0;
    return d < 1.0 ? 1.0 : d;
}

#include "mdx_splitmix64.h"

void mdx_range_push(const char* name);
void mdx_range_pop();
struct MdxRange {
    explicit MdxRange(const char* name) { mdx_range_push(name); }
    ~MdxRange() { mdx_range_pop(); }
    MdxRange(const MdxRange&) = delete; MdxRange& operator=(const MdxRange&) = delete;
};

void mdx_prof_begin(mdx_handle* h, int kind, hipStream_t st = nullptr);
void mdx_prof_end(mdx_handle* h);
void mdx_prof_collect(mdx_handle* h, int first_stale_step = 1 << 30);
// ... 1 lines not shown
```

molchanica_amd/csrc/mdx_nonbonded.hip:

```cpp
#include "mdx_internal.h"
#include "mdx_bonded_dev.h"
#include "mdx_pair_dev.h"
#include <algorithm>
#include <cfloat>
#include <cstdlib>
#include <cstring>
#include <vector>

template <bool ENERGY, int COUL>
void launch_variant(mdx_handle* h, const NbArgs& a, bool geom, bool samecut);
#define NB_EXTERN(E, C) extern template void launch_variant<E, C>(mdx_handle*, const NbArgs&, bool, bool);
NB_EXTERN(false, CM_SHIFTED) NB_EXTERN(false, CM_RF) NB_EXTERN(false, CM_EWALD) NB_EXTERN(false, CM_SOFT)
NB_EXTERN(false, CM_EWALD_TAB)
NB_EXTERN(true, CM_SHIFTED) NB_EXTERN(true, CM_RF) NB_EXTERN(true, CM_EWALD) NB_EXTERN(true, CM_SOFT)
#undef NB_EXTERN

#ifdef NB_DRAIN_TRACE
uint4* g_mdx_drain = nullptr; size_t g_mdx_drain_cap = 0; uint32_t g_mdx_drain_n = 0; int g_mdx_drain_on = 0;
extern "C" int mdx_debug_drain_trace(mdx_handle* h, int on, uint32_t* out, uint32_t cap_waves) {
    HIP_TRY(hipStreamSynchronize(h->stream));
    g_mdx_drain_on = on;
    if (!out || !g_mdx_drain) return 0;
    const uint32_t n = std::min(g_mdx_drain_n, cap_waves);
    HIP_TRY(hipMemcpy(out, g_mdx_drain, sizeof(uint4) * 2 * (size_t)n, hipMemcpyDeviceToHost));
// ... 64 lines not shown
    HIP_TRY(hipMalloc((void**)&h->d.ewald_tab, sizeof(float4) * tab.size()));
    HIP_TRY(hipMemcpy(h->d.ewald_tab, tab.data(), sizeof(float4) * tab.size(), hipMemcpyHostToDevice));
    h->ewald_tab_n = (uint32_t)tab.size(); h->ewald_tab_scale = (float)scale; h->ewald_tab_shift = sh;
    return MDX_OK;
}

bool mdx_onepass_ok(const mdx_handle* h) {
    const char* e = std::getenv("MDX_ONEPASS");
    if (e && e[0] == '0') return false;
    const int wpt = mdx_nb_wpt_half(h, h->T);
    if (!(wpt == 8 || (wpt == 1 && e && e[0] == '2'))) return false;
    static const bool dbg = [] { const char* x = std::getenv("MDX_DEBUG_ONEPASS"); return x && x[0] == '1'; }();
    if (dbg) std::fprintf(stderr, "[mdx onepass] refused %d dd %d dual %d path_split %d force_b %d fuse_ok %d variant %d wpt %d (T %u)\n", (int)h->onepass_refused, h->dd != nullptr,
                          (int)h->dual_on, (int)h->path_split, h->d.force_b != nullptr, (int)mdx_bonded_integrate_ok(h), mdx_nb_variant(h), mdx_nb_wpt_half(h, h->T), h->T);
    if (h->onepass_refused || h->dd || !h->dual_on || !h->path_split || !h->d.force_b) return false;
    if (mdx_nb_variant(h) != 5 || h->integrator != MDX_INTEGRATOR_VERLET_VELOCITY || mdx_has_constraints(h) || h->n_vsites != 0 || h->pme_on ||
        h->have_ext || h->n_posre || h->n_local != h->N || h->alch_on || h->d.posq_alt == nullptr) return false;
    if (wpt == 1 && !mdx_bonded_integrate_ok(h)) return false;
    if (h->profile && h->profile_level < 2) return false;
    NbParams p; int mode = CM_SHIFTED; bool geom = false, samecut = false;
    mdx_fill_nb_params(h, p, &mode, &geom, &samecut);
    return !geom && mode != CM_SOFT;
}

int mdx_launch_nonbonded(mdx_handle* h, bool energy, const uint32_t* d_gate, uint32_t thr_bits, int part) {
    const mdx_config& c = h->cfg;
    NbArgs a{};
    a.T = h->T;
    if (part != 0) {
        if (!h->tile_split) FAIL_NB("internal: split pair-kernel launch without a tile classification");
        a.tile_order = h->d.tile_order;
        a.t_first = part == 1 ? 0u : h->n_interior;
        a.t_count = part == 1 ? h->n_interior : h->T - h->n_interior;
    }
    if (part == 0 && h->tile_lpt_on) { a.tile_order = h->d.tile_lpt; a.t_first = 0; a.t_count = h->T; }
    a.posq = h->d.posq; a.lj = h->d.lj; a.counts = h->d.list_counts; a.entry_off = h->d.entry_off;
    a.mchunk_off = h->d.mchunk_off; a.entries = h->d.entries; a.masks = h->d.masks;
    a.force = h->d.force; a.energy = h->d.energy; a.slot_flags = h->d.slot_flags; a.gate = d_gate; a.thr_bits = thr_bits;
    a.energy_all = mdx_dd_half_shell(h) ? 1u : 0u;
    {
        static const int xcd_env = [] { const char* e = std::getenv("MDX_XCD_INTERLEAVE"); return e ? (e[0] == '1' ? 1 : 0) : -1; }();
        a.xcd_interleave = xcd_env >= 0 ? (uint32_t)xcd_env : ((h->have_local_bounds && h->n_local != h->N) ? 1u : 0u);
        if (part == 0 && h->tile_lpt_on && !h->tile_lpt_grouped) a.xcd_interleave = 1u;
    }
    const bool step_call = h->nb_step >= 0 && d_gate != nullptr;
    a.inner = (h->dual_on && !h->alch_on && !energy && (step_call || (h->nb_post_rebuild && (h->prune_pending || h->inner_from_rebuild)))) ? 1u : 0u;
    if (a.inner) {
        if (part != 2) { h->prune_latch = h->prune_pending; h->prune_pending = false; }
        a.force_prune = h->prune_latch ? 1u : 0u;
        a.prune_flag = &h->d.ctl->prune[step_call ? h->nb_step + 1 : 0];
        a.prune_flag2 = (part == 2 && step_call) ? &h->d.ctl->prune_ghost[h->nb_step + 1] : nullptr;
        const float rin = std::max(cut_on(c.lj_cutoff) ? c.lj_cutoff : 0.f, cut_on(c.coulomb_cutoff) ? c.coulomb_cutoff : 0.f) + h->inner_skin;
        a.rin2 = rin * rin;
        a.entries_in = h->d.entries_in; a.inner_nch = h->d.inner_nch; a.ref = h->d.ref; a.inner_count = h->d.inner_count;
        a.path = h->path_split ? h->d.path : nullptr; a.dprune = h->path_split ? h->d.dprune : nullptr;
    }
    static const bool fuse_bonded = [] { const char* e = std::getenv("MDX_FUSE_BONDED"); return !(e && e[0] == '0'); }();
    h->bonded_fused = false;
    if (fuse_bonded && a.inner && part == 0 && mdx_bonded_wanted(h) && !h->n_posre && !h->bonded_deferred && (!h->profile || h->profile_level >= 2)) {
        a.b_S = h->S; a.b_role_off = h->d.role_off_s; a.b_roles = h->d.role_rec_s; a.b_prm = h->d.role_prm;
        mdx_fill_bonded_params(h, a.b_p);
    }
    if (h->onepass.fprev && a.inner && part == 0 && !energy) {
        const OnePassNow& o = h->onepass;
        a.posq = o.yin; a.force = o.fcur;
        a.st_fprev = o.fprev; a.st_yout = o.yout; a.st_fnext = o.fnext; a.st_vel = h->d.vel; a.st_dt = o.dt; a.st_last = o.last ? 1u : 0u; a.st_kick = o.first ? 0.5f : 1.0f;
        {
            static const float grant = [] { const char* e = std::getenv("MDX_ONEPASS_GRANT"); return e ? (float)std::atof(e) : 1.0f; }();
            a.st_grant = grant;
        }
        a.st_disp_out = o.disp_out; a.st_prune_out = o.prune_out; a.st_viol = o.viol;
        a.st_path_thr = 0.5f * h->inner_skin * (1.0f - 1.0e-4f);
        a.b_S = 0; a.b_role_off = nullptr;
        if (mdx_bonded_wanted(h)) {
            a.b_role_off = h->d.role_off_s; a.b_roles = h->d.role_rec_s; a.b_prm = h->d.role_prm;
            mdx_fill_bonded_params(h, a.b_p);
            if (mdx_nb_wpt_half(h, a.T) != 1) a.b_S = h->S;
        }
        h->force_zeroed = true;
        ++h->onepass_launches;
    }
    int mode = CM_SHIFTED; bool geom = false, samecut = false;
    mdx_fill_nb_params(h, a.p, &mode, &geom, &samecut);
    mdx_prof_begin(h, energy ? 3 : (part == 2 ? 4 : 0));
    if (part != 2) {
        if (mdx_nb_half(h) && !h->force_zeroed) HIP_TRY(hipMemsetAsync(h->d.force, 0, sizeof(float4) * (size_t)h->S, h->stream));
        h->force_zeroed = false;
    }
#define NB_DISPATCH(E)                                                              \
    switch (mode) {                                                                 \
    case CM_SHIFTED: launch_variant<E, CM_SHIFTED>(h, a, geom, samecut); break;     \
    case CM_SOFT: launch_variant<E, CM_SOFT>(h, a, geom, samecut); break;           \
    case CM_RF: launch_variant<E, CM_RF>(h, a, geom, samecut); break;               \
    default: launch_variant<E, CM_EWALD>(h, a, geom, samecut); break;               \
    }
    if (!energy && mode == CM_EWALD && a.p.etab && !h->alch_on && mdx_nb_variant(h) != 1) launch_variant<false, CM_EWALD_TAB>(h, a, geom, samecut);
    else if (energy) { NB_DISPATCH(true) } else { NB_DISPATCH(false) }
#undef NB_DISPATCH
    mdx_prof_end(h);
    HIP_TRY(hipGetLastError());
    return MDX_OK;
}
```

molchanica_amd/csrc/mdx_nonbonded_impl.h:

```cpp
#pragma once
#include "mdx_internal.h"
#include "mdx_bonded_dev.h"
#include "mdx_pair_dev.h"
#include <algorithm>
#include <cfloat>
#include <cstdlib>
#include <type_traits>

constexpr int NB_WAVES = MDX_NB_WAVES;
#ifdef NB_DRAIN_TRACE
extern uint4* g_mdx_drain; extern size_t g_mdx_drain_cap; extern uint32_t g_mdx_drain_n; extern int g_mdx_drain_on;
#endif
#ifndef NB_ASM_PAIR
#define NB_ASM_PAIR 0
#endif
#ifndef NB_HALF_FLUSH
#define NB_HALF_FLUSH 0
#endif

template <bool BIAS, bool R2OUT>
__device__ __forceinline__ void pair_eval_asm(float xi, float yi, float zi, float qi, float sgi, float epi, const float4 pj,
                                              const float2 lj, float rc2, float bias, float& fx, float& fy, float& fz,
                                              float& g0, float& g1, float& g2, float& r2_out) {
    float dx, dy, dz, r2, t1, t2, t3, t4;
// ... 90 lines not shown
    float fx = 0.f, fy = 0.f, fz = 0.f;
    double elj = 0.0, ecoul = 0.0, evir = 0.0;

    float4 nj = make_float4(0.f, 0.f, 0.f, 0.f);
    float2 nl = make_float2(0.f, 0.f);
    uint32_t ncode = 13;
    if (nchunks) {
        const uint2 ent = a.entries[e0 + (lane >> 3)];
        const uint32_t js = ent.x * MDX_CLUSTER + (lane & 7);
        nj = a.posq[js]; nl = a.lj[js]; ncode = ent.y & 31u;
    }
    for (uint32_t c = 0; c < nchunks; ++c) {
        {
            const int kx = (int)(ncode % 3u) - 1, ky = (int)((ncode / 3u) % 3u) - 1, kz = (int)(ncode / 9u) - 1;
            nj.x += (float)kx * a.p.shift[0];
            nj.y += (float)ky * a.p.shift[1];
            nj.z += (float)kz * a.p.shift[2];
            sx[lane] = nj;
            sl[lane] = nl;
        }
        WAVE_LDS_SYNC();
        if (c + 1 < nchunks) {
            const uint2 ent = a.entries[e0 + (c + 1) * 8 + (lane >> 3)];
            const uint32_t js = ent.x * MDX_CLUSTER + (lane & 7);
            nj = a.posq[js]; nl = a.lj[js]; ncode = ent.y & 31u;
        }
        if (c < nmc) {
            const unsigned long long m = a.masks[(size_t)(mbase + c) * 64 + lane];
            chunk_pairs<ENERGY, COUL, GEOM, SAMECUT, true>(sx, sl, m, pi.x, pi.y, pi.z, pi.w, li.x, li.y, a.p,
                                                           fx, fy, fz, elj, ecoul, evir);
        } else {
            chunk_pairs<ENERGY, COUL, GEOM, SAMECUT, false>(sx, sl, ~0ull, pi.x, pi.y, pi.z, pi.w, li.x, li.y,
                                                            a.p, fx, fy, fz, elj, ecoul, evir);
        }
        WAVE_LDS_SYNC();
    }
    a.force[islot] = make_float4(fx, fy, fz, 0.f);
    if (ENERGY) {
        if (!(a.slot_flags[islot] & 2u)) { elj = 0.0; ecoul = 0.0; evir = 0.0; }
#pragma unroll
        for (int m = 32; m > 0; m >>= 1) {
            elj += __shfl_xor(elj, m);
            ecoul += __shfl_xor(ecoul, m);
            evir += __shfl_xor(evir, m);
        }
        if (lane == 0) {
            double* q = a.energy + EN_COUNT + 8 + MDX_ESTRIDE * (blk & (MDX_EPART - 1));
            atomicAdd(q, 0.5 * elj); atomicAdd(q + 1, 0.5 * ecoul); atomicAdd(q + 2, 0.5 * evir);
        }
    }
}


template <bool ENERGY, int COUL, bool GEOM, bool SAMECUT, int WPT, bool HALF, bool ALCH, int DUAL, int BW, bool STEP = false, bool UNI = false>
__device__ __forceinline__ void nb_cluster_body(const NbArgs& a, const bool owned_prune, float4 (*s_xyzq)[64], float4 (*s_lj)[64],
                                                float (*s_red)[3][64], float (*s_ownj)[64], float4 (*s_g)[64],
                                                unsigned long long (*s_mask)[64], const float4* __restrict__ etab = nullptr) {
    const int lane = threadIdx.x & 63, wave = __builtin_amdgcn_readfirstlane(threadIdx.x >> 6);
    constexpr int SPLIT = BW < WPT ? WPT / BW : 1;
    static_assert(!UNI || (!ENERGY && !GEOM && !ALCH && !STEP), "the constant-sigma^2 body: force-only, Lorentz-Berthelot, no alchemical window");
    static_assert(SPLIT == 1 || HALF, "a tile split over workgroups returns its i-forces through atomics");
    constexpr int TPB = SPLIT > 1 ? 1 : BW / WPT;
    const uint32_t ntiles = a.tile_order ? a.t_count : a.T;
    const uint32_t nblocks = SPLIT > 1 ? ntiles * SPLIT : (ntiles + TPB - 1) / TPB;
    const uint32_t per_xcd = (nblocks + 7) >> 3;
    constexpr bool TAIL = WPT == 1 && HALF && DUAL != 0 && !STEP && BW == 1;
    const bool tail_on = TAIL && a.tail_w > 1u;
    const uint32_t blk = (a.xcd_interleave || tail_on) ? blockIdx.x : (blockIdx.x & 7u) * per_xcd + (blockIdx.x >> 3);
    if (!tail_on && blk >= nblocks) return;
    const int tib = SPLIT > 1 ? 0 : wave / WPT;
    int part = SPLIT > 1 ? (int)(blk % SPLIT) * BW + wave : wave % WPT;
    uint32_t tidx = SPLIT > 1 ? blk / SPLIT : blk * TPB + tib;
    uint32_t wv = WPT;
    if (tail_on) {
        const uint32_t xcd = blockIdx.x & 7u, u = blockIdx.x >> 3;
        tidx = xcd * a.tail_group + u;
        if (u >= a.tail_head) {
            const uint32_t v = u - a.tail_head;
            wv = a.tail_w;
            part = (int)(v & (wv - 1u));
            tidx = xcd * a.tail_group + a.tail_head + (v >> (wv == 4u ? 2 : 1));
        }
    }
    const bool t_ok = tidx < ntiles;
    if (WPT == 1 && !t_ok) return;
    const uint32_t t = t_ok ? (a.tile_order ? __builtin_amdgcn_readfirstlane(a.tile_order[a.t_first + tidx]) : tidx) : a.T;
    const int ii = lane & 7, jj = lane >> 3;

    float xi[8], yi[8], zi[8], qi[8], sgi[8], epi[8], fx[8], fy[8], fz[8];
    if constexpr (STEP) {
        static_assert(HALF && !ENERGY && !ALCH && DUAL != 0, "one launch per step: half list, dual list");
        const uint32_t s = t * MDX_TILE + lane;
        const float4 Y = a.posq[s], Fp = a.st_fprev[s];
        const float4 x = step_pos(Y, Fp);
        if (part == 0 && t_ok) {
            float4 v = a.st_vel[s];
            float d2w = 0.f, pw = 0.f;
            bool viol = false;
            if (v.w != 0.f) {
                const float w = Fp.w, kdt = a.st_kick * a.st_dt * v.w;
                const float4 Fm = a.st_fnext[s];
                const float kx = w * Fp.x, ky = w * Fp.y, kz = w * Fp.z;
                const float sx_ = fmaf(a.st_dt, v.x, kx), sy_ = fmaf(a.st_dt, v.y, ky), sz_ = fmaf(a.st_dt, v.z, kz);
                v.x = fmaf(kdt, Fp.x, v.x); v.y = fmaf(kdt, Fp.y, v.y); v.z = fmaf(kdt, Fp.z, v.z);
                float path;
                const float4 r = a.ref[s];
                const float dpr = __builtin_sqrtf((x.x - r.x) * (x.x - r.x) + (x.y - r.y) * (x.y - r.y) + (x.z - r.z) * (x.z - r.z));
                if (DUAL == 2) {
                    path = 0.f;
                    a.dprune[s] = dpr;
                } else path = a.path[s] + __builtin_sqrtf(sx_ * sx_ + sy_ * sy_ + sz_ * sz_);
                a.path[s] = path;
                {
                    float dt2 = dpr * dpr;
// ... 45 lines not shown
            fx[ci] = 0.f; fy[ci] = 0.f; fz[ci] = 0.f;
        }
        WAVE_LDS_SYNC();
    } else {
#pragma unroll
    for (int ci = 0; ci < 8; ++ci) {
        const uint32_t s = t * MDX_TILE + ci * MDX_CLUSTER + ii;
        const float4 pi = a.posq[s];
        const float2 li = UNI ? make_float2(0.f, reinterpret_cast<const float*>(a.lj)[2 * s + 1]) : a.lj[s];
        xi[ci] = pi.x; yi[ci] = pi.y; zi[ci] = pi.z; qi[ci] = pi.w; sgi[ci] = li.x; epi[ci] = li.y;
        fx[ci] = 0.f; fy[ci] = 0.f; fz[ci] = 0.f;
    }
    }
    ListCounts cnt = a.counts[t_ok ? t : 0];
    if (!t_ok) { cnt.n_masked = 0; cnt.n_plain = 0; }
    const uint32_t e0 = a.entry_off[t_ok ? t : 0];
    const uint2* __restrict__ const entries = DUAL == 1 ? a.entries_in : a.entries;
    const uint32_t nmc = cnt.n_masked >> 3;
    const uint32_t nchunks = DUAL == 1 ? (t_ok ? a.inner_nch[t * 8 + part] : 0u) : (cnt.n_masked + cnt.n_plain) >> 3;
    const uint32_t mbase = a.mchunk_off[t_ok ? t : 0];
    float4* sx = s_xyzq[wave];
    float4* const sl = s_lj[wave];
    const float* __restrict__ const lj_eps = reinterpret_cast<const float*>(a.lj) + 1;
    double elj = 0.0, ecoul = 0.0, evir = 0.0, ecross = 0.0, edudl = 0.0;
    uint32_t own_bits = 0xFFu;
    if (ENERGY && !a.energy_all) {
        own_bits = 0;
#pragma unroll
        for (int ci = 0; ci < 8; ++ci)
            own_bits |= ((a.slot_flags[t * MDX_TILE + ci * MDX_CLUSTER + ii] >> 1) & 1u) << ci;
    }

    float4 nj = make_float4(0.f, 0.f, 0.f, 0.f), nf = nj;
    float2 nl = make_float2(0.f, 0.f);
    uint32_t ny = 13, njc = 0;
    float nown = 0.f;
    unsigned long long nmq = ~0ull;
    uint2 ent_n = make_uint2(0u, 13u);
    if ((uint32_t)part < nchunks) {
        const uint2 ent = entries[e0 + part * 8 + (lane >> 3)];
        if ((uint32_t)part < nmc) nmq = a.masks[(size_t)(mbase + part) * 64 + lane];
        if ((uint32_t)part + wv < nchunks) ent_n = entries[e0 + (part + wv) * 8 + (lane >> 3)];
        const uint32_t js = ent.x * MDX_CLUSTER + (lane & 7);
        nj = a.posq[js]; ny = ent.y; njc = ent.x;
        if (UNI) nl.y = lj_eps[2 * js]; else nl = a.lj[js];
        if (STEP) nf = a.st_fprev[js];
        if (ENERGY && HALF) nown = a.energy_all ? 1.0f : (float)((a.slot_flags[js] >> 1) & 1u);
    }
    float* const fbase = reinterpret_cast<float*>(a.force);
    const bool jsel_x = ii == 0 || ii == 7, jsel_y = ii == 1 || ii == 6;
    const uint32_t jlane_off = (uint32_t)(jj * 4 + ii) * 4u;
    float4* const sg = s_g[HALF ? wave : 0];
    constexpr bool prune = DUAL == 2;
    uint32_t kept = 0;
#ifdef NB_HALF_STATS
    uint32_t dbg_jh = 0, dbg_ih = 0, dbg_q = 0, dbg_pairs = 0;
#endif
    const uint32_t c_first = nmc + (TAIL ? (((uint32_t)part + wv - (nmc & (wv - 1u))) & (wv - 1u)) : ((uint32_t)part + WPT - nmc % WPT) % WPT);
    uint32_t wcur = 0;
    if (HALF && NB_HALF_FLUSH) __builtin_amdgcn_s_waitcnt(0x0F70);
    const float rc2_s = __builtin_bit_cast(float, __builtin_amdgcn_readfirstlane(__builtin_bit_cast(int, a.p.rc2_lj)));
    auto chunk_pass = [&](auto masked_tag, const uint32_t c_begin, const uint32_t c_end) __attribute__((always_inline)) {
    constexpr bool MASKED_CHUNK = decltype(masked_tag)::value;
    for (uint32_t c = c_begin; c < c_end; c += wv) {
        const uint32_t cur_y = ny, cur_jc = njc;
        constexpr bool masked = MASKED_CHUNK;
        if (masked) s_mask[wave][lane] = nmq;
        if (ENERGY && HALF) s_ownj[wave][lane] = nown;
        if (HALF && NB_HALF_FLUSH) {
            const bool live = ((ny >> 8) & 0xFFu) != 0u;
            sg[lane] = make_float4(0.f, 0.f, 0.f, __uint_as_float(live ? njc * MDX_CLUSTER + (uint32_t)ii : t * MDX_TILE + lane));
        }
        {
            const uint32_t code = ny & 31u;
            const int kx = (int)(code % 3u) - 1, ky = (int)((code / 3u) % 3u) - 1, kz = (int)(code / 9u) - 1;
            if (STEP) nj = step_pos(nj, nf);
            nj.x += (float)kx * a.p.shift[0];
            nj.y += (float)ky * a.p.shift[1];
            nj.z += (float)kz * a.p.shift[2];
            sx[lane] = nj;
            if (UNI) sl[lane].x = nl.y; else *reinterpret_cast<float2*>(&sl[lane]) = nl;
        }
        WAVE_LDS_SYNC();
        if (c + wv < nmc) nmq = a.masks[(size_t)(mbase + c + wv) * 64 + lane];
        if (c + wv < nchunks) {
            const uint32_t js = ent_n.x * MDX_CLUSTER + (lane & 7);
            nj = a.posq[js]; ny = ent_n.y; njc = ent_n.x;
            if (UNI) nl.y = lj_eps[2 * js]; else nl = a.lj[js];
            if (STEP) nf = a.st_fprev[js];
            if (ENERGY && HALF) nown = a.energy_all ? 1.0f : (float)((a.slot_flags[js] >> 1) & 1u);
            if (c + 2 * wv < nchunks) ent_n = entries[e0 + (c + 2 * wv) * 8 + (lane >> 3)];
        }
        float celj = 0.f, cecoul = 0.f, cevir = 0.f, cecross = 0.f, cedudl = 0.f;
        uint32_t newy = cur_y & 0xFFu;
#pragma unroll 1
        for (int e = 0; e < 8; ++e) {
            const float4 pj = sx[e * 8 + jj];
            const float2 lj = UNI ? make_float2(0.f, sl[e * 8 + jj].x) : *reinterpret_cast<const float2*>(&sl[e * 8 + jj]);
            const uint32_t im = (__builtin_amdgcn_readlane(cur_y, e * 8) >> 8) & 0xFFu;
            if (im == 0) continue;
            uint32_t newm = 0;
            const int x8 = MASKED_CHUNK ? (int)(~(uint32_t)reinterpret_cast<const uint8_t*>(&s_mask[wave][lane])[e]) : 0;
            float g[3] = {-0.f, -0.f, -0.f};
            float wj = 0.f;
            if (ENERGY && HALF) wj = 0.5f * s_ownj[wave][e * 8 + jj];
#pragma unroll
            for (int ci = 0; ci < 8; ++ci) {
                if (im & (1u << ci)) {
                    float e1 = 0.f, e2 = 0.f, e3 = 0.f, e4 = 0.f, e5 = 0.f;
                    const float bias = MASKED_CHUNK ? __int_as_float((x8 << (31 - ci)) >> 31) : 0.f;
                    float r2v = 0.f;
                    constexpr bool ASM_PAIR = NB_ASM_PAIR && !ENERGY && COUL == CM_SHIFTED && !GEOM && SAMECUT && HALF && !ALCH && !UNI;
                    if constexpr (ASM_PAIR)
                        pair_eval_asm<MASKED_CHUNK, prune>(xi[ci], yi[ci], zi[ci], qi[ci], sgi[ci], epi[ci], pj, lj, rc2_s, bias, fx[ci], fy[ci], fz[ci],
                                                           g[0], g[1], g[2], r2v);
                    else
                    pair_eval<ENERGY, COUL, GEOM, SAMECUT, true, HALF, ALCH, MASKED_CHUNK, UNI>(xi[ci], yi[ci], zi[ci], qi[ci], sgi[ci], epi[ci],
                                                                             pj, lj, true, a.p, fx[ci], fy[ci],
                                                                             fz[ci], e1, e2, g, ENERGY ? &e3 : nullptr,
                                                                             (ENERGY && ALCH) ? &e4 : nullptr, bias,
                                                                             prune ? &r2v : nullptr, (ENERGY && ALCH) ? &e5 : nullptr, etab);
                    if (prune) {
                        const unsigned long long bb = __ballot(r2v < a.rin2);
                        if (bb != 0ull) newm |= 1u << ci;
#ifdef NB_HALF_STATS
                        if (bb != 0ull) {
                            const unsigned long long ilo = 0x0F0F0F0F0F0F0F0Full;
                            dbg_jh += ((uint32_t)bb != 0u) + ((bb >> 32) != 0ull);
                            dbg_ih += ((bb & ilo) != 0ull) + ((bb & ~ilo) != 0ull);
                            dbg_q += (((uint32_t)bb & 0x0F0F0F0Fu) != 0u) + (((uint32_t)bb & 0xF0F0F0F0u) != 0u) +
                                     (((uint32_t)(bb >> 32) & 0x0F0F0F0Fu) != 0u) + (((uint32_t)(bb >> 32) & 0xF0F0F0F0u) != 0u);
                            dbg_pairs += __popcll(bb);
                        }
#endif
                    }
                    if (ENERGY && HALF) {
                        const float w = wj + (((own_bits >> ci) & 1u) ? 0.5f : 0.f);
                        celj += w * e1; cecoul += w * e2; cevir += w * e3; cecross += w * e4; cedudl += w * e5;
                    } else if (ENERGY && ((own_bits >> ci) & 1u)) { celj += e1; cecoul += e2; cevir += e3; cecross += e4; cedudl += e5; }
                }
            }
            if (prune) {
                kept += __popc(newm);
                if (jj == e) newy |= newm << 8;
            }
            if (HALF && NB_HALF_FLUSH) {
#pragma unroll
                for (int d = 0; d < 3; ++d) {
                    g[d] = dpp_xadd<0xB1>(g[d]);
                    g[d] = dpp_xadd<0x4E>(g[d]);
                    g[d] = dpp_xadd<0x141>(g[d]);
                }
                if (ii < 3) reinterpret_cast<float*>(sg)[(e * 8 + jj) * 4 + ii] = ii == 0 ? g[0] : (ii == 1 ? g[1] : g[2]);
            } else if (HALF) {
                const float v = jforce_reduce8(g, jsel_x, jsel_y);
                typedef __attribute__((address_space(1))) char gchar;
                gchar* frow = (gchar*)(fbase + (size_t)__builtin_amdgcn_readlane(cur_jc, e * 8) * (MDX_CLUSTER * 4));
                asm("" : "+s"(frow));
                if (ii < 3) {
                    uint32_t off = jlane_off;
                    asm("" : "+v"(off));
#ifdef NB_EXP_NOATOMIC
                    if (v == 1.2345e30f)
#endif
                    unsafeAtomicAdd((float*)(frow + off), v);
                }
            }
        }
        if (ENERGY) { elj += (double)celj; ecoul += (double)cecoul; evir += (double)cevir; ecross += (double)cecross; edudl += (double)cedudl; }
        if (prune) {
            if (masked) {
                if (ii == 0) a.entries_in[e0 + c * 8 + jj] = make_uint2(cur_jc, newy);
            } else {
                const bool alive = ii == 0 && (newy >> 8) != 0u;
                const unsigned long long bal = __ballot(alive);
                if (alive) {
                    const uint32_t k = wcur + (uint32_t)__popcll(bal & ((1ull << lane) - 1ull));
                    a.entries_in[e0 + (c_first + (k >> 3) * wv) * 8 + (k & 7u)] = make_uint2(cur_jc, newy);
                }
                wcur += (uint32_t)__popcll(bal);
            }
        }
        WAVE_LDS_SYNC();
        if (HALF && NB_HALF_FLUSH) {
            __builtin_amdgcn_s_waitcnt(0x0F70);
            const float* const sgf = reinterpret_cast<const float*>(sg);
#pragma unroll
            for (int k = 0; k < 3; ++k) {
                const uint32_t fidx = (uint32_t)(k * 64 + lane), atom = (fidx * 171u) >> 9, comp = fidx - 3u * atom;
                const uint32_t slot = __float_as_uint(sgf[atom * 4 + 3]);
                unsafeAtomicAdd(fbase + (size_t)slot * 4 + comp, sgf[atom * 4 + comp]);
            }
        }
    }
    };
#ifndef NB_SPLIT_MASKED
#define NB_SPLIT_MASKED 1
#endif
    if (NB_SPLIT_MASKED) {
        const uint32_t c_mid = c_first < nchunks ? c_first : nchunks;
        chunk_pass(std::true_type{}, (uint32_t)part, c_mid);
        chunk_pass(std::false_type{}, c_mid, nchunks);
    } else chunk_pass(std::true_type{}, (uint32_t)part, nchunks);
    float ox = 0.f, oy = 0.f, oz = 0.f;
#pragma unroll
    for (int ci = 0; ci < 8; ++ci) {
        float x = fx[ci], y = fy[ci], z = fz[ci];
#pragma unroll
        for (int m = 8; m < 64; m <<= 1) {
            x += __shfl_xor(x, m); y += __shfl_xor(y, m); z += __shfl_xor(z, m);
        }
        if (jj == ci) { ox = x; oy = y; oz = z; }
    }
    float* const fi = fbase + (size_t)(t * MDX_TILE + lane) * 4;
    constexpr bool IFORCE_ROWS = HALF && NB_IFORCE_ROWS && !STEP;
    if (prune && t_ok) {
        const uint32_t nfull = (wcur + 7u) >> 3;
        if ((uint32_t)lane < nfull * 8u - wcur) {
            const uint32_t k = wcur + (uint32_t)lane;
            a.entries_in[e0 + (c_first + (k >> 3) * wv) * 8 + (k & 7u)] = make_uint2(a.T * MDX_CL_PER_TILE, 13u);
        }
        if (lane == 0) a.inner_nch[t * 8 + part] = nfull ? c_first + (nfull - 1u) * wv + 1u : nmc;
    }
    if (prune) {
        if (!STEP && part == 0 && t_ok && (owned_prune || !(a.slot_flags[t * MDX_TILE + lane] & 2u))) {
            const uint32_t s = t * MDX_TILE + lane;
            if (a.path) {
                const float4 x = a.posq[s], r = a.ref[s];
                const float dx = x.x - r.x, dy = x.y - r.y, dz = x.z - r.z;
                a.path[s] = 0.f; a.dprune[s] = __builtin_sqrtf(dx * dx + dy * dy + dz * dz);
            } else a.ref[s].w = 0.f;
        }
        if (lane == 0 && kept) atomicAdd(a.inner_count + ((blk * BW + wave) & (MDX_EPART - 1)), (unsigned long long)kept);
        if (lane == 0 && blk == 0 && wave == 0) atomicAdd(a.inner_count + MDX_EPART, 1ull);
#ifdef NB_HALF_STATS
        if (lane == 0) {
            atomicAdd(a.inner_count + MDX_EPART + 1, (unsigned long long)dbg_jh); atomicAdd(a.inner_count + MDX_EPART + 2, (unsigned long long)dbg_ih);
            atomicAdd(a.inner_count + MDX_EPART + 3, (unsigned long long)dbg_q); atomicAdd(a.inner_count + MDX_EPART + 4, (unsigned long long)kept);
            atomicAdd(a.inner_count + MDX_EPART + 5, (unsigned long long)dbg_pairs);
        }
#endif
    }
    if (WPT > 1) {
        s_red[wave][0][lane] = ox; s_red[wave][1][lane] = oy; s_red[wave][2][lane] = oz;
        __syncthreads();
        if ((SPLIT > 1 ? wave == 0 : part == 0) && t_ok) {
            const int w0 = SPLIT > 1 ? 0 : tib * WPT;
            ox = s_red[w0][0][lane]; oy = s_red[w0][1][lane]; oz = s_red[w0][2][lane];
#pragma unroll
            for (int w = 1; w < (SPLIT > 1 ? BW : WPT); ++w) { ox += s_red[w0 + w][0][lane]; oy += s_red[w0 + w][1][lane]; oz += s_red[w0 + w][2][lane]; }
            if (IFORCE_ROWS) iforce_add_rows(fbase + (size_t)t * (MDX_TILE * 4), sx, lane, ox, oy, oz);
            else if (HALF) { unsafeAtomicAdd(fi, ox); unsafeAtomicAdd(fi + 1, oy); unsafeAtomicAdd(fi + 2, oz); }
            else a.force[t * MDX_TILE + lane] = make_float4(ox, oy, oz, 0.f);
        }
    } else {
        if (IFORCE_ROWS) iforce_add_rows(fbase + (size_t)t * (MDX_TILE * 4), sx, lane, ox, oy, oz);
        else if (HALF) { unsafeAtomicAdd(fi, ox); unsafeAtomicAdd(fi + 1, oy); unsafeAtomicAdd(fi + 2, oz); }
        else a.force[t * MDX_TILE + lane] = make_float4(ox, oy, oz, 0.f);
    }
    if (ENERGY) {
#pragma unroll
        for (int m = 32; m > 0; m >>= 1) {
            elj += __shfl_xor(elj, m);
            ecoul += __shfl_xor(ecoul, m);
            evir += __shfl_xor(evir, m);
            if (ALCH) { ecross += __shfl_xor(ecross, m); edudl += __shfl_xor(edudl, m); }
        }
        if (lane == 0) {
            double* q = a.energy + EN_COUNT + 8 + MDX_ESTRIDE * ((blk * BW + wave) & (MDX_EPART - 1));
            atomicAdd(q, HALF ? elj : 0.5 * elj);
            atomicAdd(q + 1, HALF ? ecoul : 0.5 * ecoul);
            atomicAdd(q + 2, HALF ? evir : 0.5 * evir);
            if (ALCH) { atomicAdd(q + 3, HALF ? ecross : 0.5 * ecross); atomicAdd(q + 4, HALF ? edudl : 0.5 * edudl); }
        }
    }
}

template <bool STEP = false>
__device__ __forceinline__ void bonded_workgroup(const NbArgs& a, uint32_t wg, uint32_t wg_threads) {
    const uint32_t tid = wg * wg_threads + threadIdx.x;
    const uint32_t s = tid >> 2, q4 = tid & 3u;
    if (s >= a.b_S) return;
    const uint32_t rb = a.b_role_off[s], re = a.b_role_off[s + 1];
    if (re <= rb) return;
    const float4 self = STEP ? step_pos(a.posq[s], a.st_fprev[s]) : a.posq[s];
    float fx = 0.f, fy = 0.f, fz = 0.f;
    RoleEnergies en;
    for (uint32_t k = rb + q4; k < re; k += 4) {
        const RoleRec r = a.b_roles[k];
        if (STEP) role_eval_step<false>(r, a.b_prm, self, a.posq, a.st_fprev, a.b_p, fx, fy, fz, en);
        else role_eval<false>(r, a.b_prm, self, a.posq, a.b_p, fx, fy, fz, en);
    }
    fx = dpp_xadd<0xB1>(fx); fy = dpp_xadd<0xB1>(fy); fz = dpp_xadd<0xB1>(fz);
    fx = dpp_xadd<0x4E>(fx); fy = dpp_xadd<0x4E>(fy); fz = dpp_xadd<0x4E>(fz);
    if (q4 < 3) {
        float* const f = reinterpret_cast<float*>(a.force) + (size_t)s * 4;
        unsafeAtomicAdd(f + q4, q4 == 0 ? fx : (q4 == 1 ? fy : fz));
    }
}

#ifndef NB_STEP_WAVES3
#define NB_STEP_WAVES3 0
#endif
#ifndef NB_MERGED_NOINLINE
#define NB_MERGED_NOINLINE 0
#endif
template <bool ENERGY, int COUL, bool GEOM, bool SAMECUT, int WPT, bool HALF, bool ALCH, int DUAL, int BW>
__device__ __attribute__((noinline)) void nb_cluster_body_call(const NbArgs& a, const bool owned_prune, float4 (*s_xyzq)[64], float4 (*s_lj)[64],
                                                               float (*s_red)[3][64], float (*s_ownj)[64], float4 (*s_g)[64],
                                                               unsigned long long (*s_mask)[64], const float4* __restrict__ etab = nullptr) {
    nb_cluster_body<ENERGY, COUL, GEOM, SAMECUT, WPT, HALF, ALCH, DUAL, BW>(a, owned_prune, s_xyzq, s_lj, s_red, s_ownj, s_g, s_mask, etab);
}

template <bool ENERGY, int COUL, bool GEOM, bool SAMECUT, int WPT, bool HALF, bool ALCH = false, int DUAL = 0, bool FB = false, int SPLIT = 1, bool UNI = false>
__global__ __launch_bounds__((SPLIT > 1 ? WPT / SPLIT : (WPT > NB_WAVES ? WPT : NB_WAVES)) * 64, ((HALF && NB_HALF_FLUSH) || ENERGY || (DUAL == 5 && NB_STEP_WAVES3)) ? 3 : 4) void nb_cluster_kernel(NbArgs a) {
    if (a.gate && *a.gate > a.thr_bits) {
        if ((DUAL == 5 || DUAL == 6) && a.st_disp_out && blockIdx.x == 0 && threadIdx.x == 0) atomicMax(a.st_disp_out, *a.gate);
        return;
    }
    static_assert(DUAL != 5 || (WPT == 1 && !FB && SPLIT == 1), "one launch per step: the one-wave-per-tile class");
    static_assert(DUAL != 6 || (WPT == 8 && !FB), "one launch per step: the eight-waves-per-tile class");
    constexpr bool STEP = DUAL == 5 || DUAL == 6;
    static_assert(!UNI || (!ENERGY && !GEOM && !ALCH && !STEP && !FB && SPLIT == 1 && DUAL <= 3), "the constant-sigma^2 bodies that exist (launch_cluster)");
    static_assert(DUAL == 0 || (HALF && !ENERGY), "the dual list exists for the half-list force kernel");
    static_assert(!FB || DUAL != 0, "the bonded workgroups ride with the dual-list launches");
    constexpr int BW = SPLIT > 1 ? WPT / SPLIT : (WPT > NB_WAVES ? WPT : NB_WAVES);
    if ((DUAL == 4 || DUAL == 6 || FB) && blockIdx.x >= a.pair_grid) {
        if (DUAL == 1 || DUAL == 2) {
            const bool want_prune = (a.force_prune | *a.prune_flag) != 0u || (a.prune_flag2 && *a.prune_flag2 != 0u);
            if (want_prune != (DUAL == 2)) return;
        }
        bonded_workgroup<STEP>(a, blockIdx.x - a.pair_grid, BW * 64);
        return;
    }
    __shared__ float4 s_xyzq[BW][64];
    __shared__ float4 s_lj[BW][64];
    __shared__ float s_red[WPT > 1 ? BW : 1][3][64];
    __shared__ float s_ownj[(ENERGY && HALF) ? BW : 1][64];
    __shared__ float4 s_g[HALF ? BW : 1][64];
    __shared__ unsigned long long s_mask[BW][64];
    extern __shared__ float4 s_dyn_etab[];
    const float4* etab = nullptr;
    if (COUL == CM_EWALD_TAB && !ENERGY && !ALCH) {
        for (uint32_t k = threadIdx.x; k < a.p.etab_n; k += BW * 64) s_dyn_etab[k] = a.p.etab[k];
        __syncthreads();
        etab = reinterpret_cast<const float4*>(reinterpret_cast<const char*>(s_dyn_etab) - ((EWALD_TAB_CBITS >> a.p.etab_shift) << 4));
    }
#ifdef NB_DRAIN_TRACE
    const unsigned long long drain_t0 = wall_clock64();
#endif
    if (DUAL == 0) {
        nb_cluster_body<ENERGY, COUL, GEOM, SAMECUT, WPT, HALF, ALCH, 0, BW, false, UNI>(a, true, s_xyzq, s_lj, s_red, s_ownj, s_g, s_mask, etab);
    } else {
        const bool owned_prune = (a.force_prune | *a.prune_flag) != 0u;
        const bool want_prune = owned_prune || (a.prune_flag2 && *a.prune_flag2 != 0u);
        if (DUAL >= 3) {
#if NB_MERGED_NOINLINE
            static_assert(!UNI, "the experiment has the general bodies only");
            if (want_prune) nb_cluster_body_call<ENERGY, COUL, GEOM, SAMECUT, WPT, HALF, ALCH, 2, BW>(a, owned_prune, s_xyzq, s_lj, s_red, s_ownj, s_g, s_mask, etab);
            else nb_cluster_body_call<ENERGY, COUL, GEOM, SAMECUT, WPT, HALF, ALCH, 1, BW>(a, owned_prune, s_xyzq, s_lj, s_red, s_ownj, s_g, s_mask, etab);
#else
            if (want_prune) nb_cluster_body<ENERGY, COUL, GEOM, SAMECUT, WPT, HALF, ALCH, 2, BW, STEP, UNI>(a, owned_prune, s_xyzq, s_lj, s_red, s_ownj, s_g, s_mask, etab);
            else nb_cluster_body<ENERGY, COUL, GEOM, SAMECUT, WPT, HALF, ALCH, 1, BW, STEP, UNI>(a, owned_prune, s_xyzq, s_lj, s_red, s_ownj, s_g, s_mask, etab);
#endif
        } else {
            if (want_prune != (DUAL == 2)) return;
            nb_cluster_body<ENERGY, COUL, GEOM, SAMECUT, WPT, HALF, ALCH, DUAL == 2 ? 2 : 1, BW, false, UNI>(a, owned_prune, s_xyzq, s_lj, s_red, s_ownj, s_g, s_mask, etab);
        }
#ifdef NB_DRAIN_TRACE
        if (DUAL == 3 && a.drain) {
            __builtin_amdgcn_s_waitcnt(0);
            const unsigned long long t1 = wall_clock64();
            if ((threadIdx.x & 63u) == 0u) {
                uint4* const o = a.drain + 2 * ((size_t)blockIdx.x * BW + (threadIdx.x >> 6));
                o[0] = make_uint4((uint32_t)drain_t0, (uint32_t)(drain_t0 >> 32), (uint32_t)t1, (uint32_t)(t1 >> 32));
                o[1] = make_uint4(__builtin_amdgcn_s_getreg(4 | (31 << 11)), __builtin_amdgcn_s_getreg(20 | (31 << 11)), want_prune ? 1u : 0u, 1u);
            }
        }
#endif
    }
}

template <bool ENERGY, int COUL, bool G, bool S, int WPT, bool HALF, int DUAL>
static bool launch_cluster(bool uni, dim3 g, dim3 b, uint32_t lds, hipStream_t st, const NbArgs& a) {
    if constexpr (!ENERGY && !G && COUL != CM_SOFT) {
        if (uni) {
            hipLaunchKernelGGL((nb_cluster_kernel<false, COUL, false, S, WPT, HALF, false, DUAL, false, 1, true>), g, b, lds, st, a);
            return true;
        }
    }
    hipLaunchKernelGGL((nb_cluster_kernel<ENERGY, COUL, G, S, WPT, HALF, false, DUAL>), g, b, lds, st, a);
    return false;
}

template <bool ENERGY, int COUL>
void launch_variant(mdx_handle* h, const NbArgs& a_in, bool geom, bool samecut) {
    NbArgs a = a_in;
    const bool uni = h->uni_lj && !h->alch_on && !geom && a.p.uni_c != 0.f;
    bool uni_used = false;
    const int var = mdx_nb_variant(h);
    int wpt = 1;
    const bool half = var == 5;
    if (var == 2) wpt = (a.T < mdx_wpt8_below(h)) ? 8 : 4;
    if (half) wpt = mdx_nb_wpt_half(h, a.T);
    if (var == 4) wpt = 4;
    const uint32_t bw = std::max(wpt, NB_WAVES);
    const uint32_t tpb = (var == 1) ? NB_WAVES : bw / wpt;
    const uint32_t nblocks = ((a.tile_order ? a.t_count : a.T) + tpb - 1) / tpb;
    const uint32_t grid = ((nblocks + 7) / 8) * 8;
    if (nblocks == 0) return;
    dim3 g(grid), b(bw * 64);
    if (half && wpt == 1 && a.inner && !ENERGY && !a.st_fprev && h->tail_w > 1u && h->tile_lpt_on && a.tile_order == h->d.tile_lpt && !a.xcd_interleave) {
        a.tail_group = (a.T + 7u) >> 3;
        const uint32_t tail = std::min(h->tail_tiles, a.tail_group);
        a.tail_w = h->tail_w; a.tail_head = a.tail_group - tail;
        g = dim3(8u * (a.tail_head + a.tail_w * tail));
    }
    if (a.inner) {
        uint32_t n_tail = 0;
        for (uint32_t x = 0; a.tail_w && x < 8u; ++x) {
            const uint32_t in_range = a.T > x * a.tail_group ? std::min(a.T - x * a.tail_group, a.tail_group) : 0u;
            n_tail += in_range > a.tail_head ? in_range - a.tail_head : 0u;
        }
        h->pair_info_tail[0] = a.tail_w; h->pair_info_tail[1] = n_tail;
    }
#ifdef NB_DRAIN_TRACE
    if (a.inner && g_mdx_drain_on) {
        const size_t want = (size_t)g.x * bw * 2;
        if (want > g_mdx_drain_cap) {
            if (g_mdx_drain) (void)hipFree(g_mdx_drain);
            (void)hipMalloc((void**)&g_mdx_drain, sizeof(uint4) * want);
            g_mdx_drain_cap = want;
        }
        (void)hipMemsetAsync(g_mdx_drain, 0, sizeof(uint4) * want, h->stream);
        a.drain = g_mdx_drain; g_mdx_drain_n = (uint32_t)(g.x * bw);
    }
#endif
    static const uint32_t lds_pad_env = [] { const char* e = std::getenv("MDX_NB_LDS_PAD"); return e ? (uint32_t)std::atoi(e) : 0u; }();
    const uint32_t lds_pad = ((h->pme_on && h->pme_overlap && !ENERGY) ? lds_pad_env : 0u) +
                             ((COUL == CM_EWALD_TAB && !ENERGY) ? a.p.etab_n * (uint32_t)sizeof(float4) : 0u);
    static const bool dual_merged = [] { const char* e = std::getenv("MDX_DUAL_MERGED"); return !(e && e[0] == '0'); }();
    static const bool merge_all = [] { const char* e = std::getenv("MDX_DUAL_MERGED"); return !(e && (e[0] == '0' || e[0] == '1')); }();
    static const int split_env = [] { const char* e = std::getenv("MDX_TILE_SPLIT"); return e ? (e[0] == '0' ? 0 : 1) : -1; }();
    const bool split2 = split_env >= 0 ? split_env == 1 : (a.tile_order ? a.t_count : a.T) < 1024u;
    static const bool fb_all = [] { const char* e = std::getenv("MDX_FUSE_BONDED"); return e && e[0] == '2'; }();
    auto note = [&](int dual, int w, int split, int fb) {
        uint32_t* const o = a.inner ? h->pair_info_step : h->pair_info_any;
        o[0] = (uint32_t)w; o[1] = (uint32_t)dual; o[2] = half ? 1u : 0u; o[3] = (uint32_t)COUL; o[4] = ENERGY ? 1u : 0u;
        o[5] = (uint32_t)split; o[6] = (uint32_t)fb; o[7] = a.tile_order ? a.t_count : a.T;
    };
#define NB_STEP(G, S)                                                                                                 \
    do {                                                                                                               \
        if constexpr (!ENERGY && !G && COUL != CM_SOFT) {                                                              \
            if (wpt == 1 && half && a.inner) {                                                                         \
                hipLaunchKernelGGL((nb_cluster_kernel<false, COUL, false, S, 1, true, false, 5>), g, b, lds_pad, h->stream, a); \
                note(5, 1, 1, 0);                                                                                      \
            } else if (wpt == 8 && half && a.inner && split2) {             \
                NbArgs af = a;                                                                                         \
                const uint32_t nb2 = (a.tile_order ? a.t_count : a.T) * 2u;                                            \
                af.pair_grid = ((nb2 + 7) / 8) * 8;                                                                    \
                const dim3 gf(af.pair_grid + (a.b_S ? (uint32_t)(((size_t)a.b_S * 4 + 255) / 256) : 0u)), bf(256);     \
                hipLaunchKernelGGL((nb_cluster_kernel<false, COUL, false, S, 8, true, false, 6, false, 2>), gf, bf, lds_pad, h->stream, af); \
                note(6, 8, 2, 0);                                                                                      \
            } else if (wpt == 8 && half && a.inner) {                                                                  \
                NbArgs af = a; af.pair_grid = grid;                                                                    \
                const dim3 gf(grid + (a.b_S ? (uint32_t)(((size_t)a.b_S * 4 + bw * 64 - 1) / (bw * 64)) : 0u));        \
                hipLaunchKernelGGL((nb_cluster_kernel<false, COUL, false, S, 8, true, false, 6>), gf, b, lds_pad, h->stream, af); \
                note(6, 8, 1, 0);                                                                                      \
            } else h->onepass_refused = true;                                                                          \
        } else h->onepass_refused = true;                                                                              \
    } while (0)
#define NB_DUAL(G, S, D)                                                                                              \
    do {                                                                                                               \
        if (ENERGY) break;                                                                                             \
        if (fb_all && a.b_S && (wpt == 2 || wpt == 4)) {     \
            NbArgs af = a; af.pair_grid = grid;                                                                        \
            const dim3 gf(grid + (uint32_t)(((size_t)a.b_S * 4 + bw * 64 - 1) / (bw * 64)));                           \
            if (wpt == 2) hipLaunchKernelGGL((nb_cluster_kernel<false, COUL, G, S, 2, true, false, D, true>), gf, b, lds_pad, h->stream, af); \
            else hipLaunchKernelGGL((nb_cluster_kernel<false, COUL, G, S, 4, true, false, D, true>), gf, b, lds_pad, h->stream, af);          \
            h->bonded_fused = true; note(D, wpt, 1, 1);                                                                \
            break;                                                                                                     \
        }                                                                                                              \
        note(D, wpt == 8 || wpt == 2 || wpt == 1 ? wpt : 4, 1, 0);                                                     \
        if (wpt == 8) hipLaunchKernelGGL((nb_cluster_kernel<false, COUL, G, S, 8, true, false, D>), g, b, lds_pad, h->stream, a); \
        else if (wpt == 2) hipLaunchKernelGGL((nb_cluster_kernel<false, COUL, G, S, 2, true, false, D>), g, b, lds_pad, h->stream, a); \
        else if (wpt == 1) uni_used = launch_cluster<false, COUL, G, S, 1, true, D>(uni, g, b, lds_pad, h->stream, a);                 \
        else hipLaunchKernelGGL((nb_cluster_kernel<false, COUL, G, S, 4, true, false, D>), g, b, lds_pad, h->stream, a);               \
    } while (0)
#define NB_LAUNCH(G, S)                                                                                    \
    do {                                                                                                   \
        note(0, var == 1 ? 0 : ((h->alch_on && wpt != 8) ? 4 : wpt), 1, 0);    \
        if (h->alch_on && wpt == 8) hipLaunchKernelGGL((nb_cluster_kernel<ENERGY, COUL, G, S, 8, true, COUL != CM_EWALD_TAB>), g, b, lds_pad, h->stream, a); \
        else if (h->alch_on) hipLaunchKernelGGL((nb_cluster_kernel<ENERGY, COUL, G, S, 4, true, COUL != CM_EWALD_TAB>), g, b, lds_pad, h->stream, a); \
        else if (a.st_fprev) { NB_STEP(G, S); }                                                                    \
        else if (var == 1) hipLaunchKernelGGL((nb_tile_kernel<ENERGY, COUL, G, S>), g, b, lds_pad, h->stream, a);     \
        else if (half && a.inner && dual_merged && wpt == 8 && split2 && !ENERGY) {    \
            NbArgs af = a;                                                                                         \
            const uint32_t nb2 = (a.tile_order ? a.t_count : a.T) * 2u;                                            \
            af.pair_grid = ((nb2 + 7) / 8) * 8;                                                                    \
            const dim3 gf(af.pair_grid + (a.b_S ? (uint32_t)(((size_t)a.b_S * 4 + 255) / 256) : 0u)), bf(256);     \
            if (a.b_S) { hipLaunchKernelGGL((nb_cluster_kernel<false, COUL, G, S, 8, true, false, 4, false, 2>), gf, bf, lds_pad, h->stream, af); h->bonded_fused = true; note(4, 8, 2, 0); } \
            else { hipLaunchKernelGGL((nb_cluster_kernel<false, COUL, G, S, 8, true, false, 3, false, 2>), gf, bf, lds_pad, h->stream, af); note(3, 8, 2, 0); } \
        }                                                                                                          \
        else if (half && a.inner && dual_merged && wpt == 8 && a.b_S && !ENERGY) {                                 \
            NbArgs af = a; af.pair_grid = grid;                                                                    \
            const dim3 gf(grid + (uint32_t)(((size_t)a.b_S * 4 + bw * 64 - 1) / (bw * 64)));                       \
            hipLaunchKernelGGL((nb_cluster_kernel<false, COUL, G, S, 8, true, false, 4>), gf, b, lds_pad, h->stream, af); \
            h->bonded_fused = true; note(4, 8, 1, 0);                                                              \
        }                                                                                                          \
        else if (half && a.inner && dual_merged && (wpt == 8 || merge_all)) { NB_DUAL(G, S, 3); }                  \
        else if (half && a.inner) { if (!a.force_prune) NB_DUAL(G, S, 1); NB_DUAL(G, S, 2); }    \
        else if (half && wpt == 8) hipLaunchKernelGGL((nb_cluster_kernel<ENERGY, COUL, G, S, 8, true>), g, b, lds_pad, h->stream, a); \
        else if (half && wpt == 2) hipLaunchKernelGGL((nb_cluster_kernel<ENERGY, COUL, G, S, 2, true>), g, b, lds_pad, h->stream, a); \
        else if (half && wpt == 1) uni_used = launch_cluster<ENERGY, COUL, G, S, 1, true, 0>(uni, g, b, lds_pad, h->stream, a);    \
        else if (half) hipLaunchKernelGGL((nb_cluster_kernel<ENERGY, COUL, G, S, 4, true>), g, b, lds_pad, h->stream, a); \
        else if (wpt == 8) uni_used = launch_cluster<ENERGY, COUL, G, S, 8, false, 0>(uni, g, b, lds_pad, h->stream, a);           \
        else if (wpt == 4) uni_used = launch_cluster<ENERGY, COUL, G, S, 4, false, 0>(uni, g, b, lds_pad, h->stream, a);           \
        else hipLaunchKernelGGL((nb_cluster_kernel<ENERGY, COUL, G, S, 1, false>), g, b, lds_pad, h->stream, a);        \
    } while (0)
    if (geom) { if (samecut) NB_LAUNCH(true, true); else NB_LAUNCH(true, false); }
    else      { if (samecut) NB_LAUNCH(false, true); else NB_LAUNCH(false, false); }
#undef NB_LAUNCH
#undef NB_DUAL
#undef NB_STEP
    if (a.inner || (h->nb_step >= 0 && a.gate)) h->pair_body_step = uni_used ? 1u : 0u;
    h->pair_body_any = uni_used ? 1u : 0u;
}
```

molchanica_amd/csrc/mdx_pair_dev.h:

```cpp
#pragma once
#include "mdx_internal.h"

struct NbParams;
void mdx_fill_nb_params(const mdx_handle* h, NbParams& p, int* mode_out, bool* geom_out, bool* samecut_out);

#define WAVE_LDS_SYNC()                                        \
    do {                                                       \
        __builtin_amdgcn_fence(__ATOMIC_SEQ_CST, "workgroup"); \
        __builtin_amdgcn_wave_barrier();                       \
    } while (0)

template <int CTRL>
__device__ __forceinline__ float dpp_xadd(float v) {
    return v + __int_as_float(__builtin_amdgcn_update_dpp(0, __float_as_int(v), CTRL, 0xF, 0xF, true));
}

__device__ __forceinline__ float jforce_reduce8(const float g[3], const bool sel_x, const bool sel_y) {
    float q[3];
#pragma unroll
    for (int d = 0; d < 3; ++d) q[d] = dpp_xadd<0x4E>(dpp_xadd<0xB1>(g[d]));
    float v = dpp_xadd<0x141>(sel_x ? q[0] : (sel_y ? q[1] : q[2]));
    asm volatile("" : "+v"(v));
    return v;
}

#ifndef NB_IFORCE_ROWS
#define NB_IFORCE_ROWS 1
#endif

__device__ __forceinline__ void iforce_add_rows(float* __restrict__ rows, float4* strip, const int lane, const float ox, const float oy, const float oz) {
    strip[lane] = make_float4(ox, oy, oz, 0.f);
    WAVE_LDS_SYNC();
    const float* const w = reinterpret_cast<const float*>(strip);
#pragma unroll
    for (int k = 0; k < 4; ++k) {
        const float v = w[k * 64 + lane];
        if ((lane & 3) != 3) unsafeAtomicAdd(rows + k * 64 + lane, v);
    }
}

struct NbArgs {
    uint32_t T;
    const float4* posq; const float2* lj;
    const ListCounts* counts; const uint32_t* entry_off; const uint32_t* mchunk_off;
    const uint2* entries; const unsigned long long* masks;
    float4* force; double* energy;
    const uint8_t* slot_flags;
    NbParams p;
    const uint32_t* gate; uint32_t thr_bits;
    uint32_t inner;
    uint32_t force_prune;
    const uint32_t* prune_flag;
    float rin2;
    uint2* entries_in;
    uint32_t* inner_nch;
    float4* ref; unsigned long long* inner_count;
    float* path; float* dprune;
    uint32_t xcd_interleave;
    const uint32_t* tile_order; uint32_t t_first, t_count;
    const uint32_t* prune_flag2;
    uint32_t energy_all;
    uint32_t pair_grid, b_S;
    const uint32_t* b_role_off; const RoleRec* b_roles; const float4* b_prm;
    BondedParams b_p;
    const float4* st_fprev; float4* st_yout; float4* st_fnext; float4* st_vel;
    float st_dt, st_path_thr;
    uint32_t st_last;
    float st_grant;
    float st_kick;
    uint32_t* st_disp_out;
    uint32_t* st_prune_out;
    uint32_t* st_viol;
    uint32_t tail_w, tail_head, tail_group;
#ifdef NB_DRAIN_TRACE
    uint4* drain;
#endif
};

enum { CM_SHIFTED = 0, CM_RF = 1, CM_EWALD = 2, CM_SOFT = 3,
       CM_EWALD_TAB = 4 };

#define EWALD_TAB_C 4.0f
#define EWALD_TAB_CBITS 0x40800000u
#define EWALD_TAB_MAX 1024u

template <bool ENERGY, int COUL, bool GEOM, bool SAMECUT, bool BRANCHY, bool HALF = false, bool ALCH = false, bool NANMASK = false, bool UNI = false>
__device__ __forceinline__ void pair_eval(float xi, float yi, float zi, float qi, float sgi, float epi,
                                          const float4 pj, const float2 lj, bool allowed, const NbParams& p,
                                          float& fx, float& fy, float& fz, float& elj, float& ecoul,
                                          float* g = nullptr, float* evir = nullptr, float* ecross = nullptr,
                                          float r2bias = 0.f, float* r2_out = nullptr, float* edudl = nullptr,
                                          const float4* __restrict__ etab = nullptr) {
    static_assert(!NANMASK || BRANCHY, "the NaN-coded exclusion needs the early-out");
    static_assert(!UNI || (!ENERGY && !GEOM && !ALCH), "the constant-sigma^2 body: force-only, Lorentz-Berthelot, no alchemical window");
    const float dx = xi - pj.x, dy = yi - pj.y, dz = zi - pj.z;
    const float r2 = NANMASK ? __builtin_fmaf(dz, dz, __builtin_fmaf(dx, dx, __builtin_fmaf(dy, dy, r2bias)))
                             : dx * dx + dy * dy + dz * dz;
    if (NANMASK) allowed = true;
    if (r2_out) *r2_out = r2;
    const bool in_lj = (r2 < p.rc2_lj) && allowed;
    const bool in_c = SAMECUT ? in_lj : ((r2 < p.rc2_coul) && allowed);
    if (BRANCHY && !(in_lj || in_c)) return;
    const float sig = UNI ? 0.f : (GEOM ? sgi * lj.x : sgi + lj.x);
    const float eps_s = epi * lj.y;
    const float eps = ALCH ? fabsf(eps_s) : eps_s;
    const bool cross = ALCH && __float_as_int(eps_s) < 0;
    const float ascale = cross ? p.alch_scale : 1.0f;
    float rinv, r2e = r2, sg6 = 0.f;
    float4 en = make_float4(0.f, 0.f, 0.f, 0.f); float dxt = 0.f;
    constexpr bool tab = COUL == CM_EWALD_TAB && !ENERGY && !ALCH;
    if (tab) {
        const float x = __builtin_fmaf(r2, p.etab_scale, EWALD_TAB_C);
        const uint32_t sh = p.etab_shift, xm = __float_as_uint(x) & (0xFFFFFFFFu << sh);
        en = *reinterpret_cast<const float4*>(reinterpret_cast<const char*>(etab) + (xm >> (sh - 4u)));
        dxt = x - __uint_as_float(xm);
    }
    if (ALCH) {
        const float sgsc = (sig > 0.f && eps != 0.f) ? sig : p.sc_sigmin;
        const float sg2 = sgsc * sgsc;
        sg6 = sg2 * sg2 * sg2;
        const float rsc6 = __builtin_fmaf(cross ? p.sc_al : 0.f, sg6, r2 * r2 * r2);
        rinv = (cross && p.sc_al != 0.f) ? __builtin_amdgcn_exp2f(__builtin_amdgcn_logf(rsc6) * (-1.0f / 6.0f)) : __builtin_amdgcn_rsqf(r2);
        if (cross && p.sc_al != 0.f) r2e = __builtin_amdgcn_rcpf(rinv * rinv);
    } else rinv = __builtin_amdgcn_rsqf(r2);
    const float rinv2 = rinv * rinv;
    const float s2 = (UNI ? p.uni_c : sig * sig) * rinv2;
    const float s6 = s2 * s2 * s2;
    const float es6 = eps * s6;
#ifdef NB_EXP_NOLJ
    const float flj_r2 = 0.f;
#else
    const float flj_r2 = es6 * (2.0f * s6 - 1.0f);
#endif
    const float qq = qi * pj.w;
    float fc_r2;
    if (COUL == CM_SHIFTED) fc_r2 = qq * rinv;
    else if (COUL == CM_SOFT) fc_r2 = qq * rinv * r2e * __frcp_rn(r2e + p.soft2);
    else if (COUL == CM_RF) fc_r2 = qq * (rinv - p.k_rf2 * r2e);
    float erfc_ar = 0.f;
    if (tab) {
        const float gsm = __builtin_fmaf(dxt, __builtin_fmaf(dxt, en.z, en.y), en.x);
        fc_r2 = qq * __builtin_fmaf(-gsm, r2e, rinv);
    } else if (COUL == CM_EWALD || COUL == CM_EWALD_TAB) {
        const float ar = p.alpha * r2e * rinv;
        const float ex = __expf(-ar * ar);
        const float t = __builtin_amdgcn_rcpf(1.0f + 0.3275911f * ar);
        erfc_ar = t * (0.254829592f + t * (-0.284496736f + t * (1.421413741f + t * (-1.453152027f + t * 1.061405429f)))) * ex;
        fc_r2 = qq * (erfc_ar * rinv + 1.1283791671f * p.alpha * ex);
    }
    float fs;
    if (SAMECUT) fs = (BRANCHY || in_lj) ? (flj_r2 + fc_r2) * rinv2 : 0.0f;
    else fs = (in_lj || in_c) ? ((in_lj ? flj_r2 : 0.0f) + (in_c ? fc_r2 : 0.0f)) * rinv2 : 0.0f;
    const float fsc = fs;
    if (ALCH) {
        const float w = r2 * rinv2;
        fs *= cross ? ascale * w * w : 1.0f;
    }
    fx += fs * dx; fy += fs * dy; fz += fs * dz;
    if (HALF) { g[0] = __builtin_fmaf(-fs, dx, g[0]); g[1] = __builtin_fmaf(-fs, dy, g[1]); g[2] = __builtin_fmaf(-fs, dz, g[2]); }
    if (ENERGY) {
        const float e_l = es6 * (s6 - 1.0f) * (1.0f / 6.0f);
        float e_c;
        if (COUL == CM_SHIFTED || COUL == CM_SOFT) e_c = qq * (rinv - p.coul_shift);
        else if (COUL == CM_RF) e_c = qq * (rinv + p.k_rf * r2e - p.coul_shift);
        else e_c = qq * erfc_ar * rinv;
        const float u_l = in_lj ? e_l : 0.f, u_c = in_c ? e_c : 0.f;
        elj += ALCH ? ascale * u_l : u_l;
        ecoul += ALCH ? ascale * u_c : u_c;
        if (ALCH && ecross && cross) {
            *ecross += u_l + u_c;
            if (edudl) *edudl += -(u_l + u_c) - ascale * fsc * p.sc_alpha * sg6 * rinv2 * rinv2 * (1.0f / 6.0f);
        }
        if (evir) *evir += fs * r2;
    }
}
```

molchanica_amd/md_state.py:

```python
from __future__ import annotations

import ctypes as C
import os

import numpy as np

from ._abi import (CCommDiag, CFlexOpts, CHBond, CConfig, CEnergies, CRefineOpts, CSearchOpts, CStats, CSystem, FLEX_DIHEDRALS, FORCE,
                   MDX_EDEVICE, MDX_ENAN, MDX_EOOM, MDX_EPARAM, MDX_OK, POS, POSE_MAX_ATOMS, POSE_MAX_TORSIONS, VEL, MdConfig, MdSystem)

_HERE = os.path.dirname(os.path.abspath(__file__))
LIB_PATH = os.environ.get("MDX_LIB") or os.path.join(_HERE, "libmdx.so")


class ParamError(ValueError):
    """The reference's `ParamError { descrip }` (src/md/mod.rs:967)."""


class DeviceError(RuntimeError):
    """HIP/device failure (MDX_EDEVICE / MDX_EOOM); the reference degrades to its CPU path here
    (src/util.rs:1072-1119) — this library has none and says so loudly."""


class BlowUpError(FloatingPointError):
    """Non-finite state (MDX_ENAN); cf. the stop criteria at sol_shrinking_box.rs:776-789."""


_lib = None
_fp = C.POINTER(C.c_float)
_u32p = C.POINTER(C.c_uint32)


def load_library():
    global _lib
    if _lib is not None:
        return _lib
    if not os.path.exists(LIB_PATH):
        raise ImportError(
            f"{LIB_PATH} not found: the HIP extension is not built. Run "
            f"`python -c 'import __graft_entry__ as g; g.build()'` (no CPU fallback exists).")
    try:
        import torch
    except ImportError:
        pass
    lib = C.CDLL(LIB_PATH)
    H = C.c_void_p
    lib.mdx_device_count.restype = C.c_int
    lib.mdx_last_error.restype = C.c_char_p
    lib.mdx_config_default.argtypes = [C.POINTER(CConfig)]
    lib.mdx_create.argtypes = [C.POINTER(CSystem), C.POINTER(CConfig), C.c_int, C.POINTER(H)]
    lib.mdx_destroy.argtypes = [H]
    lib.mdx_destroy.restype = None
    lib.mdx_step.argtypes = [H, C.c_float, _fp, C.c_uint32]
    lib.mdx_energy.argtypes = [H, C.POINTER(CEnergies)]
    lib.mdx_single_point.argtypes = [C.POINTER(CSystem), C.POINTER(CConfig), C.c_int,
                                     C.POINTER(CEnergies), _fp]
    lib.mdx_download.argtypes = [H, C.c_int, _fp]
    lib.mdx_upload.argtypes = [H, C.c_int, _fp]
    lib.mdx_upload_range.argtypes = [H, C.c_int, C.c_uint32, C.c_uint32, _fp]
    lib.mdx_set_box.argtypes = [H, C.c_float * 3, C.c_float * 3]
    lib.mdx_shrink_cell_towards.argtypes = [H, C.c_float * 3, C.c_float * 3, C.c_float, C.POINTER(C.c_int)]
    lib.mdx_rebuild_spatial_caches.argtypes = [H]
    lib.mdx_step_count.argtypes = [H]
    lib.mdx_step_count.restype = C.c_uint64
    lib.mdx_neighbor_list.argtypes = [H, _u32p, _u32p]
    lib.mdx_profile.argtypes = [H, C.c_int]
    lib.mdx_get_stats.argtypes = [H, C.POINTER(CStats)]
    lib.mdx_get_skin.argtypes = [H, _fp, C.POINTER(C.c_int)]
    lib.mdx_pair_launch_info.argtypes = [H, _u32p]
    lib.mdx_pair_body_info.argtypes = [H, _u32p]
    lib.mdx_minimize_energy.argtypes = [H, C.c_uint32, _fp, C.c_float, C.POINTER(CEnergies), _u32p]
    lib.mdx_initialize_velocities.argtypes = [H, C.c_float, C.c_int, C.c_uint64]
    lib.mdx_set_thermostat.argtypes = [H, C.c_int, C.c_float, C.c_float, C.c_uint32, C.c_uint64]
    lib.mdx_set_barostat.argtypes = [H, C.c_int, C.c_float, C.c_float, C.c_float, C.c_uint32]
    lib.mdx_set_integrator.argtypes = [H, C.c_int, C.c_float, C.c_float, C.c_uint64]
    lib.mdx_configure_alchemical_window.argtypes = [H, C.c_uint32, C.c_double]
    lib.mdx_set_alchemical_softcore.argtypes = [H, C.c_float, C.c_float]
    lib.mdx_get_box.argtypes = [H, C.POINTER(C.c_float), C.POINTER(C.c_float)]
    lib.mdx_set_zero_com_drift.argtypes = [H, C.c_int]
    lib.mdx_set_snapshot_cadence.argtypes = [H, C.c_uint32, C.c_int]
    lib.mdx_set_energy_cadence.argtypes = [H, C.c_uint32]
    lib.mdx_snapshot_count.argtypes = [H]
    lib.mdx_snapshot_count.restype = C.c_uint32
    lib.mdx_snapshot_read.argtypes = [H, C.c_uint32, C.POINTER(C.c_double), C.POINTER(C.c_uint64),
                                      C.POINTER(CEnergies), _fp, _fp]
    lib.mdx_flush_snapshot_queues.argtypes = [H]
    lib.mdx_set_snapshot_handlers.argtypes = [H, _u32p]
    lib.mdx_snapshot_handler_mask.argtypes = [H, C.c_uint32]
    lib.mdx_snapshot_handler_mask.restype = C.c_uint32
    lib.mdx_snapshot_read_forces.argtypes = [H, C.c_uint32, _fp]
    lib.mdx_set_water_layout.argtypes = [H, C.c_uint32, C.c_uint32, C.c_uint32]
    lib.mdx_water_download.argtypes = [H, C.c_int, _fp, _fp, _fp, _fp]
    lib.mdx_set_hbond_detection.argtypes = [H, C.c_void_p, C.c_float, C.c_float]
    lib.mdx_snapshot_read_water.argtypes = [H, C.c_uint32, _fp, _fp, _fp]
    lib.mdx_snapshot_hbond_count.argtypes = [H, C.c_uint32]
    lib.mdx_snapshot_hbond_count.restype = C.c_uint32
    lib.mdx_snapshot_read_hbonds.argtypes = [H, C.c_uint32, C.POINTER(CHBond), C.c_uint32]
    lib.mdx_time_ps.argtypes = [H]
    lib.mdx_time_ps.restype = C.c_double
    lib.mdx_set_local_atoms.argtypes = [H, C.c_uint32, C.c_void_p, C.c_void_p, C.c_void_p, C.c_void_p,
                                        C.c_float * 3, C.c_float * 3, C.c_int32]
    lib.mdx_local_state.argtypes = [H, C.c_void_p, C.c_void_p]
    lib.mdx_chunk_begin.argtypes = [H]
    lib.mdx_chunk_integrate.argtypes = [H, C.c_int, C.c_float, C.c_uint32]
    lib.mdx_chunk_forces.argtypes = [H, C.c_int32]
    lib.mdx_chunk_end.argtypes = [H, C.c_uint32, _u32p]
    lib.mdx_flag_words.argtypes = [H]
    lib.mdx_flag_words.restype = C.c_void_p
    lib.mdx_stale_threshold.argtypes = [H]
    lib.mdx_stale_threshold.restype = C.c_uint32
    lib.mdx_add_steps.argtypes = [H, C.c_uint32]
    lib.mdx_pack_positions.argtypes = [H, C.c_void_p, C.c_uint32, C.c_void_p, C.c_int32]
    lib.mdx_unpack_positions.argtypes = [H, C.c_void_p, C.c_uint32, C.c_void_p, C.c_void_p, C.c_int32]
    lib.mdx_stream.argtypes = [H]
    lib.mdx_stream.restype = C.c_void_p
    lib.mdx_comm_unique_id.argtypes = [C.c_char_p]
    lib.mdx_comm_init.argtypes = [H, C.c_char_p, C.c_int, C.c_int]
    lib.mdx_fabric_create.argtypes = [C.c_int]
    lib.mdx_fabric_create.restype = C.c_void_p
    lib.mdx_fabric_destroy.argtypes = [C.c_void_p]
    lib.mdx_fabric_destroy.restype = None
    lib.mdx_fabric_abort.argtypes = [C.c_void_p]
    lib.mdx_fabric_abort.restype = None
# ... 457 lines not shown
    _water_first = 0
    _water_sites = 0

    def set_water_layout(self, first_atom: int, n_waters: int, sites_per_water: int):
        _check(load_library().mdx_set_water_layout(self._h, int(first_atom), int(n_waters), int(sites_per_water)))
        self._water_first, self._n_waters, self._water_sites = int(first_atom), int(n_waters), int(sites_per_water)

    def water(self, which: str = "posit") -> dict:
        n = self._n_waters
        arr = {k: np.empty((n, 3), dtype=np.float32) for k in (("o", "h0", "h1", "m") if self._water_sites == 4 else ("o", "h0", "h1"))}
        _check(load_library().mdx_water_download(self._h, POS if which == "posit" else FORCE, arr["o"].ctypes.data_as(_fp),
                                                 arr["h0"].ctypes.data_as(_fp), arr["h1"].ctypes.data_as(_fp),
                                                 arr["m"].ctypes.data_as(_fp) if "m" in arr else None))
        return arr

    def set_hbond_detection(self, is_heavy_nosf, max_h_acc_dist: float = 2.5, min_angle_deg: float = 120.0):
        if is_heavy_nosf is None:
            _check(load_library().mdx_set_hbond_detection(self._h, None, 0.0, 0.0))
            return
        m = np.ascontiguousarray(is_heavy_nosf, dtype=np.uint8).reshape(self.n_atoms)
        _check(load_library().mdx_set_hbond_detection(self._h, m.ctypes.data, float(max_h_acc_dist), float(min_angle_deg)))

    def flush_snapshot_queues(self):
        _check(load_library().mdx_flush_snapshot_queues(self._h))

    @property
    def time_ps(self) -> float:
        return float(load_library().mdx_time_ps(self._h))

    def profile(self, enable=True):
        _check(load_library().mdx_profile(self._h, int(enable)))

    def stats(self) -> dict:
        s = CStats()
        _check(load_library().mdx_get_stats(self._h, C.byref(s)))
        return s.as_dict()

    def pair_launch_info(self) -> dict:
        out = (C.c_uint32 * 24)()
        _check(load_library().mdx_pair_launch_info(self._h, out))
        keys = ("waves_per_tile", "dual", "half", "coulomb", "energy", "workgroups_per_tile", "bonded_workgroups", "tiles")
        return {"step": dict(zip(keys, (int(v) for v in out[0:8]))), "any": dict(zip(keys, (int(v) for v in out[8:16]))),
                "inner_lists_from_rebuilds": int(out[16]), "last_rebuild_wrote_the_inner_list": bool(out[17]),
                "water_step_launches": int(out[18]), "water_step_mixed_launches": int(out[19]),
                "one_launch_steps": int(out[20]), "kicks_beyond_grant": int(out[21]),
                "tail": {"waves_per_tile": int(out[22]), "tiles": int(out[23])}}

    def pair_body_info(self) -> dict:
        out = (C.c_uint32 * 4)()
        _check(load_library().mdx_pair_body_info(self._h, out))
        return {"eligible": bool(out[0]), "step": bool(out[1]), "any": bool(out[2]), "c_bits": int(out[3]),
                "c": float(np.array([out[3]], np.uint32).view(np.float32)[0])}

    def skin(self):
        v, t = C.c_float(), C.c_int()
        _check(load_library().mdx_get_skin(self._h, C.byref(v), C.byref(t)))
        return float(v.value), bool(t.value)

    def computation_time(self) -> float:
        return float(self.stats()["wall_ms_sum"])

    def comm_init(self, unique_id: bytes, rank: int, world: int):
        assert len(unique_id) == 128
        _check(load_library().mdx_comm_init(self._h, bytes(unique_id), int(rank), int(world)))

    def comm_init_fabric(self, fabric: "Fabric", rank: int):
        self._fabric = fabric
        _check(load_library().mdx_comm_init_fabric(self._h, fabric.ptr, int(rank)))

    def comm_init_shm(self, name: str, rank: int, world: int):
        _check(load_library().mdx_comm_init_shm(self._h, name.encode(), int(rank), int(world)))

    def comm_init_null(self, rank: int, world: int):
        _check(load_library().mdx_comm_init_null(self._h, int(rank), int(world)))

    def comm_selftest(self):
        _check(load_library().mdx_comm_selftest(self._h))

    def comm_selftest_fault(self):
        _check(load_library().mdx_comm_selftest_fault(self._h))

    def comm_debug_partition(self, n_atoms: int) -> dict:
        cls = np.zeros(n_atoms, np.uint8); owner = np.zeros(n_atoms, np.uint8); code = np.zeros(n_atoms, np.uint8)
        mask = np.zeros(n_atoms, np.uint32)
        ns, nr = C.c_uint32(), C.c_uint32()
        lib = load_library()
        _check(lib.mdx_comm_debug_partition(self._h, cls.ctypes.data, owner.ctypes.data, code.ctypes.data, mask.ctypes.data,
                                            C.byref(ns), C.byref(nr), None, None, 0))
        sid = np.zeros(max(ns.value, 1), np.uint32); rid = np.zeros(max(nr.value, 1), np.uint32)
        _check(lib.mdx_comm_debug_partition(self._h, None, None, None, None, C.byref(ns), C.byref(nr), sid.ctypes.data, rid.ctypes.data,
                                            max(ns.value, nr.value, 1)))
        return dict(cls=cls, owner=owner, image_code=code, send_mask=mask, send_ids=sid[:ns.value], recv_ids=rid[:nr.value])

    def pme_info(self) -> dict:
        on, a, b, c = C.c_int(), C.c_uint64(), C.c_uint64(), C.c_uint64()
        _check(load_library().mdx_pme_info(self._h, C.byref(on), C.byref(a), C.byref(b), C.byref(c)))
        return dict(slab_on=bool(on.value), mesh_bytes_sent=a.value, transpose_bytes_sent=b.value, replicated_mesh_bytes=c.value)

    def pme_brick_overflows(self) -> int:
        n = C.c_uint64()
        _check(load_library().mdx_pme_brick_overflows(self._h, C.byref(n)))
        return int(n.value)

    def set_hydrogen_constraint(self, kind: str, order: int = 4, iters: int = 1, shake_tolerance: float = 0.0) -> str:
        k = {"flexible": 0, "shake": 1, "linear": 2}[kind.lower()]
        lib = load_library()
# ... 116 lines not shown
```

Baseline: 2.227 billion.

## Tag inner-list cluster pairs with an LJ bit and skip LJ math when absent

During inner-list pruning, the code now records a per-cluster-pair bit that says whether any atom pair within reach has nonzero LJ epsilon on both sides. A new force kernel variant (LJB) reads that bit and evaluates a Coulomb-only pair body for pairs without LJ wells, such as water hydrogens. The aim is to avoid the LJ arithmetic on most pairs in a solvated box. The cost is an extra LJ parameter load and ballots during prune, CAS-based atomic counters, and more kernel template instantiations.

```diff
diff --git a/include/mdx.h b/include/mdx.h
--- a/include/mdx.h
+++ b/include/mdx.h
@@ -187,6 +187,7 @@
 int mdx_get_stats(mdx_handle* h, mdx_stats* out);
 int mdx_pair_launch_info(const mdx_handle* h, uint32_t out[24]);
 int mdx_pair_body_info(const mdx_handle* h, uint32_t out[4]);
+int mdx_pair_lj_info(const mdx_handle* h, uint64_t out[4]);
 int mdx_get_skin(const mdx_handle* h, float* skin, int* tuning);
 
 #define MDX_THERMOSTAT_NONE      0
diff --git a/molchanica_amd/csrc/mdx_api.hip b/molchanica_amd/csrc/mdx_api.hip
--- a/molchanica_amd/csrc/mdx_api.hip
+++ b/molchanica_amd/csrc/mdx_api.hip
@@ -133,7 +133,7 @@
                     d.tile_col, d.scan_tmp, d.cl_lo, d.cl_hi, d.cl_kind, d.list_counts, d.entry_cnt, d.entry_off,
                     d.mchunk_cnt, d.mchunk_off, d.entries, d.entries_in, d.inner_nch, d.list_cursors, d.masks, d.role_off_o, d.role_rec_o, d.role_cnt_s,
                     d.role_off_s, d.role_rec_s, d.role_prm, d.ctl, d.energy,
-                    d.flags_dev, d.bonded_part, d.bbox_red, d.pair_count, d.inner_count, d.pme_force, d.wstep_s, d.path, d.dprune, d.force_b, d.force_c, d.cons_o, d.cons_s, d.cons_tmp, d.cons_mask, d.cons_cnt, d.cons_off, d.cons_vir, d.vsite_o, d.vsite_s, d.gsite_o, d.gsite_s, d.gsite_tmp, d.pme_q, d.pme_f,
+                    d.flags_dev, d.bonded_part, d.bbox_red, d.pair_count, d.inner_count, d.lj_count, d.pme_force, d.wstep_s, d.path, d.dprune, d.force_b, d.force_c, d.cons_o, d.cons_s, d.cons_tmp, d.cons_mask, d.cons_cnt, d.cons_off, d.cons_vir, d.vsite_o, d.vsite_s, d.gsite_o, d.gsite_s, d.gsite_tmp, d.pme_q, d.pme_f,
                     d.pme_theta, d.pme_q2, d.pme_f2, d.scratch4, d.tile_bnd, d.tile_scan, d.tile_order, d.tile_lpt, d.rb_ctl, d.scan_chain, d.grp, d.grp_mat, d.fl_hot, d.fl_slab, d.star_o, d.star_s, d.ewald_tab,
                     d.ps_cls, d.ps_p14, d.ps_stage, d.ps_slab, d.ps_rows, d.ps_fslab, d.ps_fout, d.ps_rigid, d.ps_flex, d.ps_flex_tab, d.ps_search};
     for (void* p : ptrs) if (p) (void)hipFree(p);
@@ -219,6 +219,7 @@
         const char* const e = std::getenv("MDX_KIND_CLUSTERS");
         h->kind_split = e ? e[0] != '0' : (n_lj_only >= N / 20u && n_q_only >= N / 20u && N >= 200000u);
     }
+    mdx_refresh_lj_bit(h);
     mdx_refresh_uni_lj(h);
     h->mol_start.assign(s->mol_start ? s->mol_start : nullptr, s->mol_start ? s->mol_start + s->n_mols : nullptr);
     h->total_charge = 0.0; h->sum_q2 = 0.0;
@@ -1342,6 +1343,23 @@
     return MDX_OK;
 }
 
+extern "C" int mdx_pair_lj_info(const mdx_handle* h, uint64_t out[4]) {
+    if (!h || !out) FAIL(MDX_EPARAM, "null argument");
+    out[0] = h->lj_bit ? 1u : 0u; out[1] = h->lj_bit_step; out[2] = 0; out[3] = 0;
+    if (h->d.lj_count) {
+        unsigned long long c[2 * MDX_LJ_COUNT_WORDS];
+        HIP_TRY(hipSetDevice(h->device));
+        HIP_TRY(hipMemcpyAsync(c, h->d.lj_count, sizeof(c), hipMemcpyDeviceToHost, h->stream));
+        HIP_TRY(hipStreamSynchronize(h->stream));
+        uint32_t last = 0;
+        for (int k = 0; k < MDX_LJ_COUNT_WORDS; ++k) last = std::max(last, (uint32_t)(c[k] >> 32));
+        for (int k = 0; k < MDX_LJ_COUNT_WORDS; ++k) {
+            if (last && (uint32_t)(c[k] >> 32) == last) { out[2] += c[k] & 0xFFFFFFFFull; out[3] += c[MDX_LJ_COUNT_WORDS + k] & 0xFFFFFFFFull; }
+        }
+    }
+    return MDX_OK;
+}
+
 extern "C" int mdx_get_stats(mdx_handle* h, mdx_stats* out) {
     if (!h || !out) FAIL(MDX_EPARAM, "null argument");
     HIP_TRY(hipSetDevice(h->device));
diff --git a/molchanica_amd/csrc/mdx_extras.hip b/molchanica_amd/csrc/mdx_extras.hip
--- a/molchanica_amd/csrc/mdx_extras.hip
+++ b/molchanica_amd/csrc/mdx_extras.hip
@@ -450,6 +450,7 @@
     HIP_TRY(hipStreamSynchronize(h->stream));
     MDX_TRY(mdx_unsort_state(h));
     h->alch_on = on; h->alch_lambda = on ? lambda : 0.0; h->alch_lo = lo; h->alch_hi = hi;
+    mdx_refresh_lj_bit(h);
     mdx_refresh_uni_lj(h);
     h->pme_canvas_clean = false; h->pme_canvas2_clean = false;
     h->list_valid = false; h->forces_valid = false;
diff --git a/molchanica_amd/csrc/mdx_grid.hip b/molchanica_amd/csrc/mdx_grid.hip
--- a/molchanica_amd/csrc/mdx_grid.hip
+++ b/molchanica_amd/csrc/mdx_grid.hip
@@ -912,8 +912,8 @@
 #ifndef PRUNE_TRIES
 #define PRUNE_TRIES 1
 #endif
-struct PruneInner { uint2* entries_in; uint32_t* inner_nch; float rin2; WptRule rule; };
-template <bool INNER>
+struct PruneInner { uint2* entries_in; uint32_t* inner_nch; float rin2; WptRule rule; const float2* lj; unsigned long long* lj_count; uint32_t lj_seq; };
+template <bool INNER, bool LJW = false>
 __global__ __launch_bounds__(256) void prune_list_kernel(uint32_t T, float r2, float shx, float shy, float shz,
                                                          const float4* __restrict__ posq, ListCounts* __restrict__ counts,
                                                          const uint32_t* __restrict__ entry_off, uint2* __restrict__ entries,
@@ -939,6 +939,13 @@
         const float4 p = posq[(size_t)t * MDX_TILE + ci * MDX_CLUSTER + ii];
         xi[ci] = p.x; yi[ci] = p.y; zi[ci] = p.z;
     }
+    static_assert(!LJW || INNER, "the Lennard-Jones bit belongs to the inner list");
+    unsigned long long wells_i = 0ull;
+    if (LJW) {
+#pragma unroll
+        for (int ci = 0; ci < 8; ++ci) wells_i |= (__ballot(pin.lj[(size_t)t * MDX_TILE + ci * MDX_CLUSTER + ii].y != 0.f) & 0xFFull) << (8 * ci);
+    }
+    uint32_t kept_in = 0, kept_lj = 0;
     constexpr int NTRY = INNER ? 0 : PRUNE_TRIES;
     constexpr int TI[6] = {0, 7, 3, 0, 7, 4}, TJ[6] = {0, 7, 4, 7, 0, 3};
     float4 rep[NTRY ? NTRY : 1];
@@ -955,14 +962,20 @@
     uint32_t wcur_in = 0;
     uint2 ent_n = make_uint2(null_cluster, 13u), ent_nn = make_uint2(null_cluster, 13u);
     float4 pj_n = make_float4(0.f, 0.f, 0.f, 0.f);
-    if (nchunks) { ent_n = entries[e0 + (lane >> 3)]; pj_n = posq[(size_t)ent_n.x * MDX_CLUSTER + (lane & 7)]; }
+    float wj_n = 0.f;
+    if (nchunks) {
+        ent_n = entries[e0 + (lane >> 3)]; pj_n = posq[(size_t)ent_n.x * MDX_CLUSTER + (lane & 7)];
+        if (LJW) wj_n = pin.lj[(size_t)ent_n.x * MDX_CLUSTER + (lane & 7)].y;
+    }
     if (nchunks > 1) ent_nn = entries[e0 + 8 + (lane >> 3)];
     for (uint32_t c = 0; c < nchunks; ++c) {
         const uint2 ent = ent_n;
         float4 pj = pj_n;
+        if (LJW) pj.w = wj_n;
         if (c + 1 < nchunks) {
             ent_n = ent_nn;
             pj_n = posq[(size_t)ent_n.x * MDX_CLUSTER + (lane & 7)];
+            if (LJW) wj_n = pin.lj[(size_t)ent_n.x * MDX_CLUSTER + (lane & 7)].y;
             if (c + 2 < nchunks) ent_nn = entries[e0 + (c + 2) * 8 + (lane >> 3)];
         }
         const uint32_t code = ent.y & 31u;
@@ -990,7 +1003,8 @@
             const float4 q = s_j[wave][e * 8 + jj];
             const uint32_t y = __builtin_amdgcn_readlane(y_in, e * 8);
             const uint32_t sure = (uint32_t)(acc >> (e * 8)) & 0xFFu;
-            uint32_t any = sure, anyin = 0u;
+            uint32_t any = sure, anyin = 0u, anylj = 0u;
+            const unsigned long long well_j = LJW ? __ballot(q.w != 0.f) : 0ull;
 #pragma unroll
             for (int ci = 0; ci < 8; ++ci) {
                 if (!(((y >> 8) & ~sure) & (1u << ci))) continue;
@@ -998,12 +1012,17 @@
                 const float d2 = dx * dx + dy * dy + dz * dz;
                 const bool hit = __ballot(d2 < r2) != 0ull;
                 any |= (hit ? 1u : 0u) << ci;
-                if (INNER && hit) anyin |= (__ballot(d2 < pin.rin2) != 0ull ? 1u : 0u) << ci;
+                if (INNER && hit) {
+                    const unsigned long long bin = __ballot(d2 < pin.rin2);
+                    anyin |= (bin != 0ull ? 1u : 0u) << ci;
+                    if (LJW) anylj |= (lj_pair_in_reach(bin, well_j, wells_i, ci) ? 1u : 0u) << ci;
+                }
             }
             const uint32_t im = (y >> 8) & any;
             kept += __popc(im & 0xFFu);
             if ((lane >> 3) == e) newy = (y & 0xFFu) | ((im & 0xFFu) << 8);
-            if (INNER && (lane >> 3) == e) newy_in = (y & 0xFFu) | ((((y >> 8) & anyin) & 0xFFu) << 8);
+            if (INNER && (lane >> 3) == e) newy_in = (y & 0xFFu) | ((((y >> 8) & anyin) & 0xFFu) << 8) | ((((y >> 8) & anylj) & 0xFFu) << 16);
+            if (LJW) { kept_in += __popc((y >> 8) & anyin & 0xFFu); kept_lj += __popc((y >> 8) & anylj & 0xFFu); }
         }
         __builtin_amdgcn_fence(__ATOMIC_SEQ_CST, "workgroup"); __builtin_amdgcn_wave_barrier();
         ghost_hit |= ((newy >> 8) & 0xFFu) != 0u && ent.x >= first_ghost_cluster && ent.x < null_cluster;
@@ -1032,6 +1051,10 @@
         const uint32_t nin_pad = (wcur_in + 7u) & ~7u;
         if (lane < (int)(nin_pad - wcur_in)) pin.entries_in[e0 + cnt.n_masked + wcur_in + lane] = make_uint2(null_cluster, 13u);
         if (lane < 8) pin.inner_nch[(size_t)t * 8 + lane] = nmc + (nin_pad >> 3);
+        if (LJW && lane == 0 && kept_in) {
+            unsigned long long* const w = pin.lj_count + (t & (MDX_LJ_COUNT_WORDS - 1));
+            lj_count_add(w, pin.lj_seq, kept_in); lj_count_add(w + MDX_LJ_COUNT_WORDS, pin.lj_seq, kept_lj);
+        }
     }
     const bool any_ghost = __any(ghost_hit);
     if (lane == 0) {
@@ -1621,7 +1644,7 @@
     return MDX_OK;
 }
 
-struct RebuildResult { uint32_t T = 0, E = 0, MC = 0, n_interior = 0; unsigned long long npairs = 0; bool ordered = false, classified = false, inner_built = false; };
+struct RebuildResult { uint32_t T = 0, E = 0, MC = 0, n_interior = 0; unsigned long long npairs = 0; bool ordered = false, classified = false, inner_built = false, inner_lj = false; };
 
 struct TileOrderPlan { bool lpt, grouped, split; };
 static TileOrderPlan tile_order_plan(const mdx_handle* h, uint32_t T) {
@@ -1724,7 +1747,8 @@
                            (h->n_vsites == 0 || h->vsites_convex);
     const bool inner_here = inner_env && dual_next && exact_prune && !h->dd && h->n_local == h->N && g.npop == 1 && !h->alch_on &&
                             d.entries_in && d.inner_nch;
-    bool inner_launched = false;
+    bool inner_launched = false, inner_lj = false;
+    if (inner_here && h->lj_bit && !d.lj_count) { ALLOC(d.lj_count, 2 * MDX_LJ_COUNT_WORDS); HIP_TRY(hipMemsetAsync(d.lj_count, 0, sizeof(unsigned long long) * 2 * MDX_LJ_COUNT_WORDS, st)); }
     if (prune && exact_prune) {
         const float rb = a.r_build;
         const float shx = h->per[0] ? h->box_hi[0] - h->box_lo[0] : 0.f, shy = h->per[1] ? h->box_hi[1] - h->box_lo[1] : 0.f,
@@ -1741,6 +1765,11 @@
             const float rin = std::max(std::isfinite(h->cfg.lj_cutoff) && h->cfg.lj_cutoff > 0.f ? h->cfg.lj_cutoff : 0.f,
                                        std::isfinite(h->cfg.coulomb_cutoff) && h->cfg.coulomb_cutoff > 0.f ? h->cfg.coulomb_cutoff : 0.f) + inner_skin_next;
             pin.rin2 = rin * rin;
+            if (h->lj_bit && d.lj_count) {
+                pin.lj = d.lj; pin.lj_count = d.lj_count; pin.lj_seq = ++h->lj_seq; inner_lj = true;
+                hipLaunchKernelGGL((prune_list_kernel<true, true>), dim3((div_up(T_bound, 4) + 7u) & ~7u), dim3(256), 0, st, T_bound, rb * rb, shx, shy, shz,
+                                   d.posq, d.list_counts, d.entry_off, d.entries, a.null_cluster, d.pair_count, (const uint32_t*)d.rb_ctl, tint, kinds, pin);
+            } else
             hipLaunchKernelGGL(prune_list_kernel<true>, dim3((div_up(T_bound, 4) + 7u) & ~7u), dim3(256), 0, st, T_bound, rb * rb, shx, shy, shz,
                                d.posq, d.list_counts, d.entry_off, d.entries, a.null_cluster, d.pair_count, (const uint32_t*)d.rb_ctl, tint, kinds, pin);
             inner_launched = true;
@@ -1784,6 +1813,7 @@
     res->npairs = (prune && exact_prune) ? kept : built;
     h->E = res->E; h->MC = res->MC;
     res->ordered = true;
+    res->inner_lj = inner_lj;
     res->inner_built = inner_launched && mdx_wpt_rule(mdx_wpt_rule_of(h), T) == 1;
     h->force_zeroed = true;
     h->tile_lpt_on = plan.lpt; h->tile_lpt_grouped = plan.grouped;
@@ -2033,6 +2063,8 @@
     if (h->inner_from_rebuild) ++h->inner_rebuilds;
     h->tail_w = 0; h->tail_tiles = 0;
     if (h->dual_on && h->tile_lpt_on && h->tile_lpt_grouped && !h->alch_on) mdx_tail_plan(h, T, &h->tail_w, &h->tail_tiles);
+    if (!d.lj_count) { ALLOC(d.lj_count, 2 * MDX_LJ_COUNT_WORDS); HIP_TRY(hipMemsetAsync(d.lj_count, 0, sizeof(unsigned long long) * 2 * MDX_LJ_COUNT_WORDS, st)); }
+    h->lj_bit_list = h->lj_bit && !h->alch_on && (!h->inner_from_rebuild || res.inner_lj);
     if (!d.inner_count) { ALLOC(d.inner_count, MDX_EPART + 8); HIP_TRY(hipMemsetAsync(d.inner_count, 0, sizeof(unsigned long long) * (MDX_EPART + 8), st)); }
     uint64_t nmask = (uint64_t)MC * 8;
     h->stats.n_atoms = N; h->stats.n_slots = S; h->stats.n_tiles = T; h->stats.n_clusters = NC;
diff --git a/molchanica_amd/csrc/mdx_hostutil.cpp b/molchanica_amd/csrc/mdx_hostutil.cpp
--- a/molchanica_amd/csrc/mdx_hostutil.cpp
+++ b/molchanica_amd/csrc/mdx_hostutil.cpp
@@ -70,6 +70,15 @@
     return true;
 }
 
+bool mdx_lj_bit_eligible(const float* lj, size_t n, bool alch_on) {
+    if (!lj || alch_on) return false;
+    bool with = false, without = false;
+    for (size_t i = 0; i < n && !(with && without); ++i) {
+        if (lj[2 * i + 1] == 0.f) without = true; else with = true;
+    }
+    return with && without;
+}
+
 uint64_t mdx_fp_mix(uint64_t h, const void* p, size_t bytes) {
     if (!p) return (h ^ 0x9E3779B97F4A7C15ull) * 0xBF58476D1CE4E5B9ull;
 #ifdef MDX_HOST_X86
diff --git a/molchanica_amd/csrc/mdx_internal.h b/molchanica_amd/csrc/mdx_internal.h
--- a/molchanica_amd/csrc/mdx_internal.h
+++ b/molchanica_amd/csrc/mdx_internal.h
@@ -189,6 +189,7 @@
     double*  bonded_part = nullptr; size_t cap_bonded_part = 0;
     unsigned long long* pair_count = nullptr;
     unsigned long long* inner_count = nullptr;
+    unsigned long long* lj_count = nullptr;
     float*   bbox_red = nullptr;
     uint32_t* tile_bnd = nullptr;
     uint32_t* tile_scan = nullptr;
@@ -336,6 +337,7 @@
     uint32_t pair_info_step[8] = {}, pair_info_any[8] = {};
     bool uni_lj = false; float uni_c = 0.f;
     uint32_t pair_body_step = 0, pair_body_any = 0;
+    bool lj_bit = false, lj_bit_list = false; uint32_t lj_bit_step = 0, lj_seq = 0;
     bool bonded_deferred = false;
     uint64_t rng_state = 0;
     bool zero_com = false;
@@ -479,6 +481,30 @@
     h->uni_lj = ok; h->uni_c = ok ? c : 0.f;
 }
 
+bool mdx_lj_bit_eligible(const float* lj, size_t n, bool alch_on);
+#ifndef MDX_LJ_BIT_DEFAULT
+#define MDX_LJ_BIT_DEFAULT 1
+#endif
+static inline void mdx_refresh_lj_bit(mdx_handle* h) {
+    static const bool off = [] { const char* e = std::getenv("MDX_LJ_BIT"); return (e && e[0]) ? e[0] == '0' : !MDX_LJ_BIT_DEFAULT; }();
+    h->lj_bit = !off && mdx_lj_bit_eligible(reinterpret_cast<const float*>(h->h_lj.data()), h->h_lj.size(), h->alch_on);
+}
+__device__ __forceinline__ void lj_count_add(unsigned long long* w, const uint32_t seq, const uint32_t n) {
+    unsigned long long old = __hip_atomic_load(w, __ATOMIC_RELAXED, __HIP_MEMORY_SCOPE_AGENT), seen;
+    do {
+        seen = old;
+        const unsigned long long want = (uint32_t)(seen >> 32) == seq ? seen + n : (((unsigned long long)seq << 32) | n);
+        old = atomicCAS(w, seen, want);
+    } while (old != seen);
+}
+__device__ __forceinline__ bool lj_pair_in_reach(const unsigned long long bb, const unsigned long long well_j, const unsigned long long wells_i, const int ci) {
+    const unsigned long long t = bb & well_j;
+    const uint32_t m = ((uint32_t)(wells_i >> (8 * ci)) & 0xFFu) * 0x01010101u;
+    return (((uint32_t)t | (uint32_t)(t >> 32)) & m) != 0u;
+}
+#define MDX_LJ_COUNT_WORDS 64
+
+
 int mdx_build_constraints(mdx_handle* h, const mdx_system* s);
 int mdx_remap_constraints(mdx_handle* h);
 int mdx_launch_constrain_positions(mdx_handle* h, float dt, const uint32_t* d_gate, uint32_t* d_disp_out, uint32_t thr,
diff --git a/molchanica_amd/csrc/mdx_nonbonded.hip b/molchanica_amd/csrc/mdx_nonbonded.hip
--- a/molchanica_amd/csrc/mdx_nonbonded.hip
+++ b/molchanica_amd/csrc/mdx_nonbonded.hip
@@ -140,7 +140,7 @@
         a.prune_flag2 = (part == 2 && step_call) ? &h->d.ctl->prune_ghost[h->nb_step + 1] : nullptr;
         const float rin = std::max(cut_on(c.lj_cutoff) ? c.lj_cutoff : 0.f, cut_on(c.coulomb_cutoff) ? c.coulomb_cutoff : 0.f) + h->inner_skin;
         a.rin2 = rin * rin;
-        a.entries_in = h->d.entries_in; a.inner_nch = h->d.inner_nch; a.ref = h->d.ref; a.inner_count = h->d.inner_count;
+        a.entries_in = h->d.entries_in; a.inner_nch = h->d.inner_nch; a.ref = h->d.ref; a.inner_count = h->d.inner_count; a.lj_count = h->d.lj_count;
         a.path = h->path_split ? h->d.path : nullptr; a.dprune = h->path_split ? h->d.dprune : nullptr;
     }
     static const bool fuse_bonded = [] { const char* e = std::getenv("MDX_FUSE_BONDED"); return !(e && e[0] == '0'); }();
diff --git a/molchanica_amd/csrc/mdx_nonbonded_impl.h b/molchanica_amd/csrc/mdx_nonbonded_impl.h
--- a/molchanica_amd/csrc/mdx_nonbonded_impl.h
+++ b/molchanica_amd/csrc/mdx_nonbonded_impl.h
@@ -166,7 +166,7 @@
 }
 
 
-template <bool ENERGY, int COUL, bool GEOM, bool SAMECUT, int WPT, bool HALF, bool ALCH, int DUAL, int BW, bool STEP = false, bool UNI = false>
+template <bool ENERGY, int COUL, bool GEOM, bool SAMECUT, int WPT, bool HALF, bool ALCH, int DUAL, int BW, bool STEP = false, bool UNI = false, bool LJB = false>
 __device__ __forceinline__ void nb_cluster_body(const NbArgs& a, const bool owned_prune, float4 (*s_xyzq)[64], float4 (*s_lj)[64],
                                                 float (*s_red)[3][64], float (*s_ownj)[64], float4 (*s_g)[64],
                                                 unsigned long long (*s_mask)[64], const float4* __restrict__ etab = nullptr) {
@@ -174,6 +174,7 @@
     constexpr int SPLIT = BW < WPT ? WPT / BW : 1;
     static_assert(!UNI || (!ENERGY && !GEOM && !ALCH && !STEP), "the constant-sigma^2 body: force-only, Lorentz-Berthelot, no alchemical window");
     static_assert(SPLIT == 1 || HALF, "a tile split over workgroups returns its i-forces through atomics");
+    static_assert(!LJB || (!ENERGY && !ALCH && !STEP && HALF && WPT == 1 && (DUAL == 1 || DUAL == 2)), "the Lennard-Jones bit: force-only dual-list bodies of the one-wave class");
     constexpr int TPB = SPLIT > 1 ? 1 : BW / WPT;
     const uint32_t ntiles = a.tile_order ? a.t_count : a.T;
     const uint32_t nblocks = SPLIT > 1 ? ntiles * SPLIT : (ntiles + TPB - 1) / TPB;
@@ -325,7 +326,12 @@
     const uint32_t jlane_off = (uint32_t)(jj * 4 + ii) * 4u;
     float4* const sg = s_g[HALF ? wave : 0];
     constexpr bool prune = DUAL == 2;
-    uint32_t kept = 0;
+    uint32_t kept = 0, kept_lj = 0;
+    unsigned long long wells_i = 0ull;
+    if (LJB && prune) {
+#pragma unroll
+        for (int ci = 0; ci < 8; ++ci) wells_i |= (__ballot(epi[ci] != 0.f) & 0xFFull) << (8 * ci);
+    }
 #ifdef NB_HALF_STATS
     uint32_t dbg_jh = 0, dbg_ih = 0, dbg_q = 0, dbg_pairs = 0;
 #endif
@@ -370,9 +376,12 @@
         for (int e = 0; e < 8; ++e) {
             const float4 pj = sx[e * 8 + jj];
             const float2 lj = UNI ? make_float2(0.f, sl[e * 8 + jj].x) : *reinterpret_cast<const float2*>(&sl[e * 8 + jj]);
-            const uint32_t im = (__builtin_amdgcn_readlane(cur_y, e * 8) >> 8) & 0xFFu;
+            const uint32_t ye = __builtin_amdgcn_readlane(cur_y, e * 8);
+            const uint32_t im = (ye >> 8) & 0xFFu;
             if (im == 0) continue;
             uint32_t newm = 0;
+            const unsigned long long well_j = (LJB && prune) ? __ballot(lj.y != 0.f) : 0ull;
+            if (LJB && prune) asm volatile("" : "+s"(wells_i));
             const int x8 = MASKED_CHUNK ? (int)(~(uint32_t)reinterpret_cast<const uint8_t*>(&s_mask[wave][lane])[e]) : 0;
             float g[3] = {-0.f, -0.f, -0.f};
             float wj = 0.f;
@@ -387,7 +396,12 @@
                     if constexpr (ASM_PAIR)
                         pair_eval_asm<MASKED_CHUNK, prune>(xi[ci], yi[ci], zi[ci], qi[ci], sgi[ci], epi[ci], pj, lj, rc2_s, bias, fx[ci], fy[ci], fz[ci],
                                                            g[0], g[1], g[2], r2v);
-                    else
+                    else if (LJB && DUAL == 1 && !(ye & (0x10000u << ci))) {
+                        if constexpr (LJB && DUAL == 1)
+                            pair_eval<false, COUL, GEOM, SAMECUT, true, true, false, MASKED_CHUNK, UNI, true>(xi[ci], yi[ci], zi[ci], qi[ci], sgi[ci], epi[ci],
+                                                                             pj, lj, true, a.p, fx[ci], fy[ci], fz[ci], e1, e2, g, nullptr, nullptr, bias,
+                                                                             nullptr, nullptr, etab);
+                    } else
                     pair_eval<ENERGY, COUL, GEOM, SAMECUT, true, HALF, ALCH, MASKED_CHUNK, UNI>(xi[ci], yi[ci], zi[ci], qi[ci], sgi[ci], epi[ci],
                                                                              pj, lj, true, a.p, fx[ci], fy[ci],
                                                                              fz[ci], e1, e2, g, ENERGY ? &e3 : nullptr,
@@ -396,6 +410,7 @@
                     if (prune) {
                         const unsigned long long bb = __ballot(r2v < a.rin2);
                         if (bb != 0ull) newm |= 1u << ci;
+                        if (LJB && lj_pair_in_reach(bb, well_j, wells_i, ci)) newm |= 0x100u << ci;
 #ifdef NB_HALF_STATS
                         if (bb != 0ull) {
                             const unsigned long long ilo = 0x0F0F0F0F0F0F0F0Full;
@@ -414,7 +429,8 @@
                 }
             }
             if (prune) {
-                kept += __popc(newm);
+                kept += __popc(newm & 0xFFu);
+                if (LJB) kept_lj += __popc(newm >> 8);
                 if (jj == e) newy |= newm << 8;
             }
             if (HALF && NB_HALF_FLUSH) {
@@ -506,6 +522,10 @@
         }
         if (lane == 0 && kept) atomicAdd(a.inner_count + ((blk * BW + wave) & (MDX_EPART - 1)), (unsigned long long)kept);
         if (lane == 0 && blk == 0 && wave == 0) atomicAdd(a.inner_count + MDX_EPART, 1ull);
+        if (LJB && lane == 0 && kept) {
+            unsigned long long* const w = a.lj_count + ((blk * BW + wave) & (MDX_LJ_COUNT_WORDS - 1));
+            lj_count_add(w, a.lj_seq, kept); lj_count_add(w + MDX_LJ_COUNT_WORDS, a.lj_seq, kept_lj);
+        }
 #ifdef NB_HALF_STATS
         if (lane == 0) {
             atomicAdd(a.inner_count + MDX_EPART + 1, (unsigned long long)dbg_jh); atomicAdd(a.inner_count + MDX_EPART + 2, (unsigned long long)dbg_ih);
@@ -585,7 +605,8 @@
     nb_cluster_body<ENERGY, COUL, GEOM, SAMECUT, WPT, HALF, ALCH, DUAL, BW>(a, owned_prune, s_xyzq, s_lj, s_red, s_ownj, s_g, s_mask, etab);
 }
 
-template <bool ENERGY, int COUL, bool GEOM, bool SAMECUT, int WPT, bool HALF, bool ALCH = false, int DUAL = 0, bool FB = false, int SPLIT = 1, bool UNI = false>
+template <bool ENERGY, int COUL, bool GEOM, bool SAMECUT, int WPT, bool HALF, bool ALCH = false, int DUAL = 0, bool FB = false, int SPLIT = 1, bool UNI = false,
+          bool LJB = false>
 __global__ __launch_bounds__((SPLIT > 1 ? WPT / SPLIT : (WPT > NB_WAVES ? WPT : NB_WAVES)) * 64, ((HALF && NB_HALF_FLUSH) || ENERGY || (DUAL == 5 && NB_STEP_WAVES3)) ? 3 : 4) void nb_cluster_kernel(NbArgs a) {
     if (a.gate && *a.gate > a.thr_bits) {
         if ((DUAL == 5 || DUAL == 6) && a.st_disp_out && blockIdx.x == 0 && threadIdx.x == 0) atomicMax(a.st_disp_out, *a.gate);
@@ -595,6 +616,7 @@
     static_assert(DUAL != 6 || (WPT == 8 && !FB), "one launch per step: the eight-waves-per-tile class");
     constexpr bool STEP = DUAL == 5 || DUAL == 6;
     static_assert(!UNI || (!ENERGY && !GEOM && !ALCH && !STEP && !FB && SPLIT == 1 && DUAL <= 3), "the constant-sigma^2 bodies that exist (launch_cluster)");
+    static_assert(!LJB || (!ENERGY && !ALCH && WPT == 1 && HALF && !FB && SPLIT == 1 && DUAL >= 1 && DUAL <= 3), "the bodies with the Lennard-Jones bit that exist (launch_cluster)");
     static_assert(DUAL == 0 || (HALF && !ENERGY), "the dual list exists for the half-list force kernel");
     static_assert(!FB || DUAL != 0, "the bonded workgroups ride with the dual-list launches");
     constexpr int BW = SPLIT > 1 ? WPT / SPLIT : (WPT > NB_WAVES ? WPT : NB_WAVES);
@@ -633,12 +655,12 @@
             if (want_prune) nb_cluster_body_call<ENERGY, COUL, GEOM, SAMECUT, WPT, HALF, ALCH, 2, BW>(a, owned_prune, s_xyzq, s_lj, s_red, s_ownj, s_g, s_mask, etab);
             else nb_cluster_body_call<ENERGY, COUL, GEOM, SAMECUT, WPT, HALF, ALCH, 1, BW>(a, owned_prune, s_xyzq, s_lj, s_red, s_ownj, s_g, s_mask, etab);
 #else
-            if (want_prune) nb_cluster_body<ENERGY, COUL, GEOM, SAMECUT, WPT, HALF, ALCH, 2, BW, STEP, UNI>(a, owned_prune, s_xyzq, s_lj, s_red, s_ownj, s_g, s_mask, etab);
-            else nb_cluster_body<ENERGY, COUL, GEOM, SAMECUT, WPT, HALF, ALCH, 1, BW, STEP, UNI>(a, owned_prune, s_xyzq, s_lj, s_red, s_ownj, s_g, s_mask, etab);
+            if (want_prune) nb_cluster_body<ENERGY, COUL, GEOM, SAMECUT, WPT, HALF, ALCH, 2, BW, STEP, UNI, LJB>(a, owned_prune, s_xyzq, s_lj, s_red, s_ownj, s_g, s_mask, etab);
+            else nb_cluster_body<ENERGY, COUL, GEOM, SAMECUT, WPT, HALF, ALCH, 1, BW, STEP, UNI, LJB>(a, owned_prune, s_xyzq, s_lj, s_red, s_ownj, s_g, s_mask, etab);
 #endif
         } else {
             if (want_prune != (DUAL == 2)) return;
-            nb_cluster_body<ENERGY, COUL, GEOM, SAMECUT, WPT, HALF, ALCH, DUAL == 2 ? 2 : 1, BW, false, UNI>(a, owned_prune, s_xyzq, s_lj, s_red, s_ownj, s_g, s_mask, etab);
+            nb_cluster_body<ENERGY, COUL, GEOM, SAMECUT, WPT, HALF, ALCH, DUAL == 2 ? 2 : 1, BW, false, UNI, LJB>(a, owned_prune, s_xyzq, s_lj, s_red, s_ownj, s_g, s_mask, etab);
         }
 #ifdef NB_DRAIN_TRACE
         if (DUAL == 3 && a.drain) {
@@ -655,7 +677,20 @@
 }
 
 template <bool ENERGY, int COUL, bool G, bool S, int WPT, bool HALF, int DUAL>
-static bool launch_cluster(bool uni, dim3 g, dim3 b, uint32_t lds, hipStream_t st, const NbArgs& a) {
+static bool launch_cluster(bool uni, dim3 g, dim3 b, uint32_t lds, hipStream_t st, const NbArgs& a, bool ljb = false, bool* ljb_used = nullptr) {
+    if constexpr (!ENERGY && WPT == 1 && HALF && DUAL >= 1 && DUAL <= 3 && (S || COUL != CM_EWALD_TAB)) {
+        if (ljb) {
+            if (ljb_used) *ljb_used = true;
+            if constexpr (!G && COUL != CM_SOFT) {
+                if (uni) {
+                    hipLaunchKernelGGL((nb_cluster_kernel<false, COUL, false, S, 1, true, false, DUAL, false, 1, true, true>), g, b, lds, st, a);
+                    return true;
+                }
+            }
+            hipLaunchKernelGGL((nb_cluster_kernel<false, COUL, G, S, 1, true, false, DUAL, false, 1, false, true>), g, b, lds, st, a);
+            return false;
+        }
+    }
     if constexpr (!ENERGY && !G && COUL != CM_SOFT) {
         if (uni) {
             hipLaunchKernelGGL((nb_cluster_kernel<false, COUL, false, S, WPT, HALF, false, DUAL, false, 1, true>), g, b, lds, st, a);
@@ -670,7 +705,9 @@
 void launch_variant(mdx_handle* h, const NbArgs& a_in, bool geom, bool samecut) {
     NbArgs a = a_in;
     const bool uni = h->uni_lj && !h->alch_on && !geom && a.p.uni_c != 0.f;
-    bool uni_used = false;
+    bool uni_used = false, ljb_used = false;
+    const bool ljb = h->lj_bit_list && !h->alch_on && a.inner && a.lj_count != nullptr;
+    if (ljb) a.lj_seq = ++h->lj_seq;
     const int var = mdx_nb_variant(h);
     int wpt = 1;
     const bool half = var == 5;
@@ -757,7 +794,7 @@
         note(D, wpt == 8 || wpt == 2 || wpt == 1 ? wpt : 4, 1, 0);                                                     \
         if (wpt == 8) hipLaunchKernelGGL((nb_cluster_kernel<false, COUL, G, S, 8, true, false, D>), g, b, lds_pad, h->stream, a); \
         else if (wpt == 2) hipLaunchKernelGGL((nb_cluster_kernel<false, COUL, G, S, 2, true, false, D>), g, b, lds_pad, h->stream, a); \
-        else if (wpt == 1) uni_used = launch_cluster<false, COUL, G, S, 1, true, D>(uni, g, b, lds_pad, h->stream, a);                 \
+        else if (wpt == 1) uni_used = launch_cluster<false, COUL, G, S, 1, true, D>(uni, g, b, lds_pad, h->stream, a, ljb, &ljb_used); \
         else hipLaunchKernelGGL((nb_cluster_kernel<false, COUL, G, S, 4, true, false, D>), g, b, lds_pad, h->stream, a);               \
     } while (0)
 #define NB_LAUNCH(G, S)                                                                                    \
@@ -798,4 +835,5 @@
 #undef NB_STEP
     if (a.inner || (h->nb_step >= 0 && a.gate)) h->pair_body_step = uni_used ? 1u : 0u;
     h->pair_body_any = uni_used ? 1u : 0u;
+    if (a.inner) h->lj_bit_step = ljb_used ? 1u : 0u;
 }
diff --git a/molchanica_amd/csrc/mdx_pair_dev.h b/molchanica_amd/csrc/mdx_pair_dev.h
--- a/molchanica_amd/csrc/mdx_pair_dev.h
+++ b/molchanica_amd/csrc/mdx_pair_dev.h
@@ -72,6 +72,7 @@
     uint32_t* st_prune_out;
     uint32_t* st_viol;
     uint32_t tail_w, tail_head, tail_group;
+    uint32_t lj_seq; unsigned long long* lj_count;
 #ifdef NB_DRAIN_TRACE
     uint4* drain;
 #endif
@@ -84,7 +85,8 @@
 #define EWALD_TAB_CBITS 0x40800000u
 #define EWALD_TAB_MAX 1024u
 
-template <bool ENERGY, int COUL, bool GEOM, bool SAMECUT, bool BRANCHY, bool HALF = false, bool ALCH = false, bool NANMASK = false, bool UNI = false>
+template <bool ENERGY, int COUL, bool GEOM, bool SAMECUT, bool BRANCHY, bool HALF = false, bool ALCH = false, bool NANMASK = false, bool UNI = false,
+          bool NOLJ = false>
 __device__ __forceinline__ void pair_eval(float xi, float yi, float zi, float qi, float sgi, float epi,
                                           const float4 pj, const float2 lj, bool allowed, const NbParams& p,
                                           float& fx, float& fy, float& fz, float& elj, float& ecoul,
@@ -93,6 +95,7 @@
                                           const float4* __restrict__ etab = nullptr) {
     static_assert(!NANMASK || BRANCHY, "the NaN-coded exclusion needs the early-out");
     static_assert(!UNI || (!ENERGY && !GEOM && !ALCH), "the constant-sigma^2 body: force-only, Lorentz-Berthelot, no alchemical window");
+    static_assert(!NOLJ || (!ENERGY && !ALCH), "the Coulomb-only body: force-only, no alchemical window");
     const float dx = xi - pj.x, dy = yi - pj.y, dz = zi - pj.z;
     const float r2 = NANMASK ? __builtin_fmaf(dz, dz, __builtin_fmaf(dx, dx, __builtin_fmaf(dy, dy, r2bias)))
                              : dx * dx + dy * dy + dz * dz;
@@ -101,8 +104,8 @@
     const bool in_lj = (r2 < p.rc2_lj) && allowed;
     const bool in_c = SAMECUT ? in_lj : ((r2 < p.rc2_coul) && allowed);
     if (BRANCHY && !(in_lj || in_c)) return;
-    const float sig = UNI ? 0.f : (GEOM ? sgi * lj.x : sgi + lj.x);
-    const float eps_s = epi * lj.y;
+    const float sig = (UNI || NOLJ) ? 0.f : (GEOM ? sgi * lj.x : sgi + lj.x);
+    const float eps_s = NOLJ ? 0.f : epi * lj.y;
     const float eps = ALCH ? fabsf(eps_s) : eps_s;
     const bool cross = ALCH && __float_as_int(eps_s) < 0;
     const float ascale = cross ? p.alch_scale : 1.0f;
@@ -149,7 +152,8 @@
         fc_r2 = qq * (erfc_ar * rinv + 1.1283791671f * p.alpha * ex);
     }
     float fs;
-    if (SAMECUT) fs = (BRANCHY || in_lj) ? (flj_r2 + fc_r2) * rinv2 : 0.0f;
+    if (NOLJ) fs = (SAMECUT ? (BRANCHY || in_lj) : in_c) ? fc_r2 * rinv2 : 0.0f;
+    else if (SAMECUT) fs = (BRANCHY || in_lj) ? (flj_r2 + fc_r2) * rinv2 : 0.0f;
     else fs = (in_lj || in_c) ? ((in_lj ? flj_r2 : 0.0f) + (in_c ? fc_r2 : 0.0f)) * rinv2 : 0.0f;
     const float fsc = fs;
     if (ALCH) {
diff --git a/molchanica_amd/md_state.py b/molchanica_amd/md_state.py
--- a/molchanica_amd/md_state.py
+++ b/molchanica_amd/md_state.py
@@ -68,6 +68,7 @@
     lib.mdx_get_skin.argtypes = [H, _fp, C.POINTER(C.c_int)]
     lib.mdx_pair_launch_info.argtypes = [H, _u32p]
     lib.mdx_pair_body_info.argtypes = [H, _u32p]
+    lib.mdx_pair_lj_info.argtypes = [H, C.POINTER(C.c_uint64)]
     lib.mdx_minimize_energy.argtypes = [H, C.c_uint32, _fp, C.c_float, C.POINTER(CEnergies), _u32p]
     lib.mdx_initialize_velocities.argtypes = [H, C.c_float, C.c_int, C.c_uint64]
     lib.mdx_set_thermostat.argtypes = [H, C.c_int, C.c_float, C.c_float, C.c_uint32, C.c_uint64]
@@ -631,6 +632,11 @@
         return {"eligible": bool(out[0]), "step": bool(out[1]), "any": bool(out[2]), "c_bits": int(out[3]),
                 "c": float(np.array([out[3]], np.uint32).view(np.float32)[0])}
 
+    def pair_lj_info(self) -> dict:
+        out = (C.c_uint64 * 4)()
+        _check(load_library().mdx_pair_lj_info(self._h, out))
+        return {"eligible": bool(out[0]), "step": bool(out[1]), "kept": int(out[2]), "with_bit": int(out[3])}
+
     def skin(self):
         v, t = C.c_float(), C.c_int()
         _check(load_library().mdx_get_skin(self._h, C.byref(v), C.byref(t)))
```

Measured after the change: 1.547 billion. -30.6%, worse.
